# kungyao/vae-play

Measured on AMD Instinct MI355X. Metric: images/sec (train step, 128x128 VAE), higher is better.
Workload: dtype bf16x3; 1 GPU; networks VAE 128x128x3 latent=128 train step (fwd+BCE/KL+bwd+allreduce+Adam), 32 images/GPU, global batch 32; parallelism=dp1, per_gpu_batch=32, global_batch=32, graph=False, precision=bf16x3

## Files before the change

### include/vaeplay_hip.h

```cpp
#ifndef VAEPLAY_HIP_H
#define VAEPLAY_HIP_H
#include <stddef.h>
#include <stdint.h>

#ifdef __cplusplus
extern "C" {
#endif

typedef void* vp_stream;

enum vp_status { VP_OK = 0, VP_ERR_ARG = -1, VP_ERR_LAUNCH = -2, VP_ERR_WORKSPACE = -3, VP_ERR_STATE = -4 };
enum vp_act { VP_ACT_NONE = 0, VP_ACT_RELU = 1, VP_ACT_LRELU = 2, VP_ACT_TANH = 3, VP_ACT_SIGMOID = 4 };

int vp_abi_version(void);
const char* vp_last_error(void);

int vp_nchw_to_nhwc_f32(const float* in, float* out, int B, int C, int H, int W, vp_stream stream);
int vp_nhwc_to_nchw_f32(const float* in, float* out, int B, int C, int H, int W, vp_stream stream);

int vp_pack_w5_f32(const float* w_ref, float* p0, float* p1, int Csmall, int Cbig, vp_stream stream);

int vp_conv5_gather_f32(const float* big, const float* w_p0, const float* bias, float* small_out,
                        int B, int Hs, int Ws, int Cbig, int Csmall, int stride, int act, vp_stream stream);
int vp_conv5_scatter_f32(const float* small, const float* w_p1, float* big_out,
                         int B, int Hs, int Ws, int Csmall, int Cbig, int stride, vp_stream stream);
size_t vp_conv5_wgrad_workspace_bytes(int B, int Hs, int Ws, int Cbig, int Csmall, int stride);
int vp_conv5_wgrad_f32(const float* big, const float* small, float* dw_ref,
                       int B, int Hs, int Ws, int Cbig, int Csmall, int stride,
                       void* ws, size_t ws_bytes, vp_stream stream);
int vp_conv5_wgrad_f32_cus(const float* big, const float* small, float* dw_ref, int B, int Hs, int Ws, int Cbig, int Csmall,
                           int stride, int max_cus, void* ws, size_t ws_bytes, vp_stream stream);
size_t vp_conv5_stats_f32_workspace_bytes(int family, int B, int Hs, int Ws, int Cbig, int Csmall, int stride);
int vp_conv5_gather_stats_f32(const float* big, const float* w_p0, float* small_out, int B, int Hs, int Ws, int Cbig, int Csmall, int stride,
                              float eps, float momentum, float* mean, float* rstd, float* running_mean, float* running_var, void* ws,
                              size_t ws_bytes, vp_stream stream);
int vp_conv5_scatter_stats_f32(const float* small, const float* w_p1, float* big_out, int B, int Hs, int Ws, int Csmall, int Cbig, int stride,
                               float eps, float momentum, float* mean, float* rstd, float* running_mean, float* running_var, void* ws,
                               size_t ws_bytes, vp_stream stream);

int vp_pack_w_f32(const float* w_ref, float* p0, float* p1, int Csmall, int Cbig, int ks, vp_stream stream);
int vp_conv_gather_f32(const float* big, const float* w_p0, const float* bias, float* small_out,
                       int B, int Hs, int Ws, int Hb, int Wb, int Cbig, int Csmall, int ks, int stride, int act, vp_stream stream);
int vp_conv_scatter_f32(const float* small, const float* w_p1, float* big_out,
                        int B, int Hs, int Ws, int Hb, int Wb, int Csmall, int Cbig, int ks, int stride, vp_stream stream);
size_t vp_conv_wgrad_workspace_bytes(int B, int Hs, int Ws, int Hb, int Wb, int Cbig, int Csmall, int ks, int stride);
int vp_conv_wgrad_f32(const float* big, const float* small, float* dw_ref,
                      int B, int Hs, int Ws, int Hb, int Wb, int Cbig, int Csmall, int ks, int stride,
                      void* ws, size_t ws_bytes, vp_stream stream);

int vp_pack_w_split(const float* w_ref, void* p0_split, void* p1_split, int Csmall, int Cbig, int ks, vp_stream stream);
int vp_conv_gather_bf16x3(const void* big_split, const void* w_p0_split, const float* bias, float* small_out, int B, int Hs, int Ws,
                          int Hb, int Wb, int Cbig, int Csmall, int ks, int stride, int act, vp_stream stream);
int vp_conv_scatter_bf16x3(const void* small_split, const void* w_p1_split, float* big_out, int B, int Hs, int Ws, int Hb, int Wb,
                           int Csmall, int Cbig, int ks, int stride, vp_stream stream);
size_t vp_conv_wgrad_bf16x3_workspace_bytes(int B, int Hs, int Ws, int Hb, int Wb, int Cbig, int Csmall, int ks, int stride);
int vp_conv_wgrad_bf16x3(const void* big_split, const void* small_split, float* dw_ref, int B, int Hs, int Ws, int Hb, int Wb, int Cbig,
                         int Csmall, int ks, int stride, void* ws, size_t ws_bytes, vp_stream stream);
int vp_split_f32(const float* x, void* out_split, size_t n, vp_stream stream);
int vp_split_pad_f32(const float* x, void* out_split, size_t npix, int C, int Cpad, vp_stream stream);
int vp_pack_w5_split(const float* w_ref, void* p0_split, void* p1_split, int Csmall, int Cbig, vp_stream stream);
int vp_conv5_gather_bf16x3(const void* big_split, const void* w_p0_split, const float* bias, float* small_out,
                           int B, int Hs, int Ws, int Cbig, int Csmall, int stride, int act, vp_stream stream);
int vp_conv5_scatter_bf16x3(const void* small_split, const void* w_p1_split, float* big_out,
                            int B, int Hs, int Ws, int Csmall, int Cbig, int stride, vp_stream stream);
int vp_conv5_smallout_bf16x3(const float* big, const float* w_p0, const float* bias, float* small_out, int B, int H, int W,
                             int Cbig, int Csmall, int act, vp_stream stream);
size_t vp_conv5_smallout_wgrad_bf16x3_workspace_bytes(int B, int H, int W, int Cbig, int Csmall);
int vp_conv5_smallout_wgrad_bf16x3(const float* big, const float* small, float* dw_ref, int B, int H, int W, int Cbig, int Csmall,
                                   void* ws, size_t ws_bytes, vp_stream stream);
size_t vp_conv5_smallout_wgrad_f32_workspace_bytes(int B, int H, int W, int Cbig, int Csmall);
int vp_conv5_smallout_wgrad_f32(const float* big, const float* small, float* dw_ref, int B, int H, int W, int Cbig, int Csmall,
                                void* ws, size_t ws_bytes, vp_stream stream);
int vp_im2col5s2_cols(int C);
int vp_im2col5s2_split_f32(const float* x, void* out_split, int B, int C, int Hb, int Wb, int nchw, vp_stream stream);
int vp_pack_w_im2col5_split(const float* w_ref, void* out_split, int Cout, int C, vp_stream stream);
int vp_unpack_dw_im2col5_f32(const float* dw_cols, float* dw_ref, int Cout, int C, vp_stream stream);
int vp_im2col5s2_f32(const float* x, float* out, int B, int C, int Hb, int Wb, int nchw, vp_stream stream);
int vp_pack_w_im2col5_f32(const float* w_ref, float* out, int Cout, int C, vp_stream stream);
size_t vp_conv5_stats_workspace_bytes(int family, int B, int Hs, int Ws, int Cbig, int Csmall, int stride);
int vp_conv5_gather_stats_bf16x3(const void* big_split, const void* w_p0_split, float* small_out,
                                 int B, int Hs, int Ws, int Cbig, int Csmall, int stride, float eps, float momentum,
                                 float* mean, float* rstd, float* running_mean, float* running_var,
                                 void* ws, size_t ws_bytes, vp_stream stream);
int vp_conv5_scatter_stats_bf16x3(const void* small_split, const void* w_p1_split, float* big_out,
                                  int B, int Hs, int Ws, int Csmall, int Cbig, int stride, float eps, float momentum,
                                  float* mean, float* rstd, float* running_mean, float* running_var,
                                  void* ws, size_t ws_bytes, vp_stream stream);
int vp_conv5_smallin_dgrad_bf16x3(const float* small, const float* w_ref, float* big_out, int B, int H, int W, int Csmall, int Cbig,
                                  vp_stream stream);
int vp_conv5_smallin_dgrad_f32(const float* small, const float* w_ref, float* big_out, int B, int H, int W, int Csmall, int Cbig,
                               vp_stream stream);
int vp_conv5_smallin_fwd_bf16x3(const float* small, const float* w_ref, const float* bias, float* big_out, int B, int H, int W, int Csmall,
                                int Cbig, int act, vp_stream stream);
size_t vp_conv5_wgrad_bf16x3_workspace_bytes(int B, int Hs, int Ws, int Cbig, int Csmall, int stride);
int vp_conv5_wgrad_bf16x3(const void* big_split, const void* small_split, float* dw_ref,
                          int B, int Hs, int Ws, int Cbig, int Csmall, int stride,
                          void* ws, size_t ws_bytes, vp_stream stream);
int vp_conv5_wgrad_bf16x3_cus(const void* big_split, const void* small_split, float* dw_ref,
                              int B, int Hs, int Ws, int Cbig, int Csmall, int stride, int max_cus,
                              void* ws, size_t ws_bytes, vp_stream stream);
size_t vp_conv3_small_wgrad_workspace_bytes(int B, int H, int W, int Cin, int Cout);
int vp_conv3_small_wgrad_f32(const float* x, const float* dy, float* dw_ref, int B, int H, int W, int Cin, int Cout,
                             void* ws, size_t ws_bytes, vp_stream stream);
int vp_conv3_small_fwd_f32(const float* x, const float* w_ref, const float* bias, float* y, int B, int H, int W, int Cin, int Cout,
                           vp_stream stream);
int vp_conv3_small_dgrad_f32(const float* dy, const float* w_ref, float* dx, int B, int H, int W, int Cin, int Cout, vp_stream stream);
int vp_wgrad_slab_reduce_f32(const float* slab, float* dw_ref, int Csmall, int Cbig, int nsplit, int ntaps, int variant,
                             vp_stream stream);
int vp_bn_small_fwd_f32(const float* x, int R, int C, float eps, float momentum, const float* gamma, const float* beta, float* mean,
                        float* rstd, float* running_mean, float* running_var, float* y, int act, float slope, vp_stream stream);
int vp_bn_small_bwd_f32(const float* x, const float* dy, const float* mean, const float* rstd, const float* gamma, const float* beta,
                        float* dx, float* dgamma, float* dbeta, int R, int C, int act, float slope, int batch_stats, vp_stream stream);
int vp_bn_act_fwd_split_f32(const float* x, const float* mean, const float* rstd, const float* gamma, const float* beta,
                            float* y, void* y_split, int R, int C, int act, float slope, vp_stream stream);
int vp_bn_act_bwd_split_f32(const float* x, const float* dy, const float* mean, const float* rstd,
                            const float* gamma, const float* beta, float* dx, void* dx_split, float* dgamma, float* dbeta,
                            int R, int C, int act, float slope, int batch_stats,
                            void* ws, size_t ws_bytes, vp_stream stream);
int vp_nchw_to_nhwc_split_f32(const float* in, float* out, void* out_split, int B, int C, int H, int W, vp_stream stream);
typedef struct vp_pack_job {
  const float* w;
  void* p0;
  void* p1;
  int Csmall, Cbig, Csmall_pad, split;
} vp_pack_job;
int vp_pack_w5_batch(const vp_pack_job* jobs, int njobs, vp_stream stream);
int vp_pack_w5_p1_split_padded(const float* w_ref, void* p1_split, int Csmall, int Cbig, int Csmall_pad, vp_stream stream);
int vp_bce_sigmoid_bwd_pad_split_f32(const float* p, const float* t, float gscale, float* dlogit, void* dlogit_split,
                                     size_t npix, int C, int Cpad, vp_stream stream);

size_t vp_gemm_workspace_bytes(int M, int N, int K);
int vp_gemm_f32(const float* A, long sam, long sak, const float* B, long sbn, long sbk,
                float* C, int ldc, const float* bias, int M, int N, int K, int mode,
                void* ws, size_t ws_bytes, vp_stream stream);
size_t vp_colsum_workspace_bytes(int R, int C);
int vp_colsum_f32(const float* x, float* out, int R, int C, void* ws, size_t ws_bytes, vp_stream stream);

size_t vp_bn_workspace_bytes(int R, int C);
int vp_bn_stats_f32(const float* x, int R, int C, float eps, float momentum,
                    float* mean, float* rstd, float* running_mean, float* running_var,
                    void* ws, size_t ws_bytes, vp_stream stream);
int vp_bn_act_fwd_f32(const float* x, const float* mean, const float* rstd, const float* gamma, const float* beta,
                      float* y, int R, int C, int act, float slope, vp_stream stream);
int vp_bn_act_bwd_f32(const float* x, const float* dy, const float* mean, const float* rstd,
                      const float* gamma, const float* beta, float* dx, float* dgamma, float* dbeta,
                      int R, int C, int act, float slope, int batch_stats,
                      void* ws, size_t ws_bytes, vp_stream stream);
size_t vp_instnorm_workspace_bytes(int B, int R, int C);
int vp_instnorm_act_fwd_f32(const float* x, float* y, float* mean, float* rstd, int B, int R, int C, float eps, int act,
                            float slope, void* ws, size_t ws_bytes, vp_stream stream);
int vp_instnorm_act_bwd_f32(const float* x, const float* dy, const float* mean, const float* rstd, float* dx, int B, int R, int C,
                            int act, float slope, void* ws, size_t ws_bytes, vp_stream stream);
int vp_instnorm_act_fwd_split_f32(const float* x, float* y, void* y_split, float* mean, float* rstd, int B, int R, int C, float eps,
                                  int act, float slope, void* ws, size_t ws_bytes, vp_stream stream);
int vp_instnorm_act_bwd_split_f32(const float* x, const float* dy, const float* mean, const float* rstd, float* dx, void* dx_split, int B,
                                  int R, int C, int act, float slope, void* ws, size_t ws_bytes, vp_stream stream);
int vp_act_fwd_f32(const float* x, float* y, size_t n, int act, float slope, vp_stream stream);
int vp_act_bwd_from_y_f32(const float* y, const float* dy, float* dx, size_t n, int act, float slope, vp_stream stream);

int vp_upsample2x_bilinear_fwd_f32(const float* x, float* y, int B, int H, int W, int C, vp_stream stream);
int vp_upsample2x_bilinear_bwd_f32(const float* dy, float* dx, int B, int H, int W, int C, vp_stream stream);
int vp_add_coords_f32(const float* x, float* out, int B, int H, int W, int C, int normalize, vp_stream stream);
int vp_slice_channels_f32(const float* in, float* out, size_t npix, int Cin, int Cout, vp_stream stream);

int vp_latent_fwd_f32(const float* mu, const float* logvar, const float* eps, float* z, float* kl,
                      int B, int Z, vp_stream stream);
int vp_latent_bwd_f32(const float* mu, const float* logvar, const float* eps, const float* dz, const float* gkl,
                      float gkl_scalar, float* dmu, float* dlogvar, int B, int Z, vp_stream stream);

size_t vp_reduce_workspace_bytes(size_t n);
int vp_bce_sum_f32(const float* p, const float* t, size_t n, float* out, void* ws, size_t ws_bytes, vp_stream stream);
int vp_bce_bwd_f32(const float* p, const float* t, const float* gptr, float gscale, float* dp, size_t n, vp_stream stream);
int vp_bce_sigmoid_bwd_f32(const float* p, const float* t, float gscale, float* dlogit, size_t n, vp_stream stream);
int vp_global_avgpool_fwd_f32(const float* x_nhwc, float* out, int B, int HW, int C, vp_stream stream);
int vp_global_avgpool_bwd_f32(const float* dy, float* dx_nhwc, int B, int HW, int C, vp_stream stream);
int vp_softmax_rows_fwd_f32(const float* x, float* y, int R, int n, vp_stream stream);
int vp_softmax_rows_bwd_f32(const float* y, const float* dy, float* dx, int R, int n, vp_stream stream);
int vp_cross_entropy_fwd_f32(const float* logits, const long long* labels, float* loss, float* prob, int R, int n, vp_stream stream);
int vp_cross_entropy_bwd_f32(const float* prob, const long long* labels, const float* gptr, float* dlogits, int R, int n, vp_stream stream);
int vp_l1_mean_f32(const float* a, const float* b, size_t n, float* out, void* ws, size_t ws_bytes, vp_stream stream);
int vp_l1_mean_bwd_f32(const float* a, const float* b, const float* gptr, float* da, float* db, size_t n, vp_stream stream);

size_t vp_be_loss_workspace_bytes(int B, int n);
int vp_be_loss_fwd_f32(const float* logits, const float* targets, float* loss, float* sums, int B, int n, float bce_weight,
                       float smooth, void* ws, size_t ws_bytes, vp_stream stream);
int vp_be_loss_bwd_f32(const float* logits, const float* targets, const float* sums, const float* gptr, float* dlogits, int B,
                       int n, float bce_weight, float smooth, vp_stream stream);

int vp_dice_loss_fwd_f32(const float* probs, const float* targets, float* loss, float* sums, int B, int n, float smooth, void* ws,
                         size_t ws_bytes, vp_stream stream);
int vp_dice_loss_bwd_f32(const float* probs, const float* targets, const float* sums, const float* gptr, float* dprobs, int B, int n,
                         float smooth, vp_stream stream);

int vp_half_sqdiff_f32(const float* a, const float* b, float* out, size_t n, vp_stream stream);
int vp_half_sqdiff_rowsum_f32(const float* a, const float* b, float* out, int R, int n_per_row, vp_stream stream);
int vp_half_sqdiff_bwd_f32(const float* a, const float* b, const float* g, float* da, float* db, int R, int n_per_row,
                           int g_per_row, vp_stream stream);
int vp_gan_head_f32(const float* logit, int B, float coef, float* p_out, float* sums, float* dlogit, vp_stream stream);
int vp_smooth_l1_cat_f32(const float* targets, const float* a, const float* b, int B, int n1, int n2, float scale, float* loss,
                         float* da, float* db, vp_stream stream);
int vp_sum_f32(const float* x, size_t n, float* out, void* ws, size_t ws_bytes, vp_stream stream);
int vp_vae_loss_f32(const float* x_tilde, const float* x, size_t n, const float* kl, int B, float* recon, float* kl_sum,
                    float* loss, float loss_scale, void* ws, size_t ws_bytes, vp_stream stream);
int vp_add_f32(const float* a, const float* b, float* out, size_t n, vp_stream stream);

#define VP_SPLIT_BF16 0
#define VP_SPLIT_F16 1
int vp_split_fmt_f32(const float* x, void* out_split, size_t n, int fmt, float scale, vp_stream stream);
int vp_nchw_to_nhwc_split_fmt_f32(const float* in, float* out, void* out_split, int B, int C, int H, int W, int fmt, vp_stream stream);
int vp_bn_act_fwd_split_fmt_f32(const float* x, const float* mean, const float* rstd, const float* gamma, const float* beta,
                                float* y, void* y_split, int R, int C, int act, float slope, int fmt, vp_stream stream);
int vp_bn_act_bwd_split_fmt_f32(const float* x, const float* dy, const float* mean, const float* rstd,
                                const float* gamma, const float* beta, float* dx, void* dx_split, float* dgamma, float* dbeta,
                                int R, int C, int act, float slope, int batch_stats, int fmt, float scale,
                                void* ws, size_t ws_bytes, vp_stream stream);
int vp_bn_act_bwd_split_fmt_sat_f32(const float* x, const float* dy, const float* mean, const float* rstd,
                                    const float* gamma, const float* beta, float* dx, void* dx_split, float* dgamma, float* dbeta,
                                    int R, int C, int act, float slope, int batch_stats, int fmt, float scale, int* saturated,
                                    void* ws, size_t ws_bytes, vp_stream stream);
int vp_im2col5s2_split_fmt_f32(const float* x, void* out_split, int B, int C, int Hb, int Wb, int nchw, int fmt, vp_stream stream);
int vp_pack_w_im2col5_split_fmt(const float* w_ref, void* out_split, int Cout, int C, int fmt, vp_stream stream);
int vp_conv5_gather_f16(const void* big_split, const void* w_p0_split, const float* bias, float* small_out,
// ... 48 lines not shown
```

### vae_play_amd/_lib.py

```python
from __future__ import annotations

import ctypes
import os
from ctypes import c_char_p, c_float, c_int, c_long, c_size_t, c_void_p

_HERE = os.path.dirname(os.path.abspath(__file__))
LIB_PATH = os.environ.get("VAEPLAY_HIP_LIB", os.path.join(_HERE, "libvaeplay_hip.so"))

P = c_void_p


class PackJob(ctypes.Structure):
    _fields_ = [("w", c_void_p), ("p0", c_void_p), ("p1", c_void_p), ("Csmall", c_int), ("Cbig", c_int),
                ("Csmall_pad", c_int), ("split", c_int)]


SIGNATURES = {
    "vp_abi_version": (c_int, []),
    "vp_last_error": (c_char_p, []),
    "vp_nchw_to_nhwc_f32": (c_int, [P, P, c_int, c_int, c_int, c_int, P]),
    "vp_nhwc_to_nchw_f32": (c_int, [P, P, c_int, c_int, c_int, c_int, P]),
    "vp_pack_w5_f32": (c_int, [P, P, P, c_int, c_int, P]),
    "vp_conv5_gather_f32": (c_int, [P, P, P, P, c_int, c_int, c_int, c_int, c_int, c_int, c_int, P]),
    "vp_conv5_scatter_f32": (c_int, [P, P, P, c_int, c_int, c_int, c_int, c_int, c_int, P]),
    "vp_conv5_wgrad_workspace_bytes": (c_size_t, [c_int, c_int, c_int, c_int, c_int, c_int]),
    "vp_conv5_wgrad_f32": (c_int, [P, P, P, c_int, c_int, c_int, c_int, c_int, c_int, P, c_size_t, P]),
    "vp_conv5_wgrad_f32_cus": (c_int, [P, P, P, c_int, c_int, c_int, c_int, c_int, c_int, c_int, P, c_size_t, P]),
    "vp_pack_w_f32": (c_int, [P, P, P, c_int, c_int, c_int, P]),
    "vp_conv_gather_f32": (c_int, [P, P, P, P] + [c_int] * 10 + [P]),
    "vp_conv_scatter_f32": (c_int, [P, P, P] + [c_int] * 9 + [P]),
    "vp_conv_wgrad_workspace_bytes": (c_size_t, [c_int] * 9),
    "vp_conv_wgrad_f32": (c_int, [P, P, P] + [c_int] * 9 + [P, c_size_t, P]),
    "vp_split_f32": (c_int, [P, P, c_size_t, P]),
    "vp_split_pad_f32": (c_int, [P, P, c_size_t, c_int, c_int, P]),
    "vp_pack_w5_split": (c_int, [P, P, P, c_int, c_int, P]),
    "vp_pack_w_split": (c_int, [P, P, P, c_int, c_int, c_int, P]),
    "vp_conv_gather_bf16x3": (c_int, [P, P, P, P] + [c_int] * 10 + [P]),
    "vp_conv_scatter_bf16x3": (c_int, [P, P, P] + [c_int] * 9 + [P]),
    "vp_conv_wgrad_bf16x3_workspace_bytes": (c_size_t, [c_int] * 9),
    "vp_conv_wgrad_bf16x3": (c_int, [P, P, P] + [c_int] * 9 + [P, c_size_t, P]),
    "vp_conv5_gather_bf16x3": (c_int, [P, P, P, P, c_int, c_int, c_int, c_int, c_int, c_int, c_int, P]),
    "vp_conv5_scatter_bf16x3": (c_int, [P, P, P, c_int, c_int, c_int, c_int, c_int, c_int, P]),
    "vp_conv5_smallout_bf16x3": (c_int, [P, P, P, P] + [c_int] * 6 + [P]),
    "vp_conv5_smallout_wgrad_bf16x3_workspace_bytes": (c_size_t, [c_int] * 5),
    "vp_conv5_smallout_wgrad_bf16x3": (c_int, [P, P, P] + [c_int] * 5 + [P, c_size_t, P]),
    "vp_conv5_smallout_wgrad_f32_workspace_bytes": (c_size_t, [c_int] * 5),
    "vp_conv5_smallout_wgrad_f32": (c_int, [P, P, P] + [c_int] * 5 + [P, c_size_t, P]),
    "vp_im2col5s2_cols": (c_int, [c_int]),
    "vp_im2col5s2_split_f32": (c_int, [P, P, c_int, c_int, c_int, c_int, c_int, P]),
    "vp_pack_w_im2col5_split": (c_int, [P, P, c_int, c_int, P]),
    "vp_unpack_dw_im2col5_f32": (c_int, [P, P, c_int, c_int, P]),
    "vp_im2col5s2_f32": (c_int, [P, P, c_int, c_int, c_int, c_int, c_int, P]),
    "vp_pack_w_im2col5_f32": (c_int, [P, P, c_int, c_int, P]),
    "vp_conv5_stats_workspace_bytes": (c_size_t, [c_int] * 7),
    "vp_conv5_gather_stats_bf16x3": (c_int, [P, P, P] + [c_int] * 6 + [c_float, c_float, P, P, P, P, P, c_size_t, P]),
    "vp_conv5_gather_stats_f32": (c_int, [P, P, P] + [c_int] * 6 + [c_float, c_float, P, P, P, P, P, c_size_t, P]),
    "vp_conv5_scatter_stats_f32": (c_int, [P, P, P] + [c_int] * 6 + [c_float, c_float, P, P, P, P, P, c_size_t, P]),
    "vp_conv5_stats_f32_workspace_bytes": (c_size_t, [c_int] * 7),
    "vp_conv5_scatter_stats_bf16x3": (c_int, [P, P, P] + [c_int] * 6 + [c_float, c_float, P, P, P, P, P, c_size_t, P]),
    "vp_split_fmt_f32": (c_int, [P, P, c_size_t, c_int, c_float, P]),
    "vp_nchw_to_nhwc_split_fmt_f32": (c_int, [P, P, P, c_int, c_int, c_int, c_int, c_int, P]),
    "vp_bn_act_fwd_split_fmt_f32": (c_int, [P] * 7 + [c_int, c_int, c_int, c_float, c_int, P]),
    "vp_bn_act_bwd_split_fmt_f32": (c_int, [P] * 10 + [c_int, c_int, c_int, c_float, c_int, c_int, c_float, P, c_size_t, P]),
    "vp_bn_act_bwd_split_fmt_sat_f32": (c_int, [P] * 10 + [c_int, c_int, c_int, c_float, c_int, c_int, c_float, P, P, c_size_t, P]),
    "vp_im2col5s2_split_fmt_f32": (c_int, [P, P] + [c_int] * 6 + [P]),
    "vp_pack_w_im2col5_split_fmt": (c_int, [P, P, c_int, c_int, c_int, P]),
    "vp_conv5_gather_f16": (c_int, [P, P, P, P] + [c_int] * 8 + [c_float, P]),
    "vp_conv_gather_f16": (c_int, [P, P, P, P] + [c_int] * 11 + [c_float, P]),
    "vp_conv5_scatter_f16": (c_int, [P, P, P] + [c_int] * 7 + [c_float, P]),
    "vp_conv_scatter_f16": (c_int, [P, P, P] + [c_int] * 10 + [c_float, P]),
    "vp_conv5_wgrad_f16x2": (c_int, [P, P, P] + [c_int] * 6 + [c_float, P, c_size_t, P]),
    "vp_conv5_wgrad_f16x2_cus": (c_int, [P, P, P] + [c_int] * 6 + [c_float, c_int, P, c_size_t, P]),
    "vp_conv_wgrad_f16x2": (c_int, [P, P, P] + [c_int] * 9 + [c_float, P, c_size_t, P]),
    "vp_conv5_stats_f16_workspace_bytes": (c_size_t, [c_int] * 7),
    "vp_conv5_gather_stats_f16": (c_int, [P, P, P] + [c_int] * 7 + [c_float, c_float, P, P, P, P, P, c_size_t, P]),
    "vp_conv5_scatter_stats_f16": (c_int, [P, P, P] + [c_int] * 7 + [c_float, c_float, P, P, P, P, P, c_size_t, P]),
    "vp_conv5_smallin_fwd_bf16x3": (c_int, [P, P, P, P, c_int, c_int, c_int, c_int, c_int, c_int, P]),
    "vp_conv5_smallin_dgrad_bf16x3": (c_int, [P, P, P, c_int, c_int, c_int, c_int, c_int, P]),
    "vp_conv5_smallin_dgrad_f32": (c_int, [P, P, P, c_int, c_int, c_int, c_int, c_int, P]),
    "vp_conv5_wgrad_bf16x3_workspace_bytes": (c_size_t, [c_int, c_int, c_int, c_int, c_int, c_int]),
    "vp_conv5_wgrad_bf16x3": (c_int, [P, P, P, c_int, c_int, c_int, c_int, c_int, c_int, P, c_size_t, P]),
    "vp_conv5_wgrad_bf16x3_cus": (c_int, [P, P, P, c_int, c_int, c_int, c_int, c_int, c_int, c_int, P, c_size_t, P]),
    "vp_wgrad_slab_reduce_f32": (c_int, [P, P, c_int, c_int, c_int, c_int, c_int, P]),
    "vp_conv3_small_wgrad_workspace_bytes": (c_size_t, [c_int] * 5),
    "vp_conv3_small_wgrad_f32": (c_int, [P, P, P, c_int, c_int, c_int, c_int, c_int, P, c_size_t, P]),
    "vp_conv3_small_fwd_f32": (c_int, [P, P, P, P, c_int, c_int, c_int, c_int, c_int, P]),
    "vp_conv3_small_dgrad_f32": (c_int, [P, P, P, c_int, c_int, c_int, c_int, c_int, P]),
    "vp_bn_small_fwd_f32": (c_int, [P, c_int, c_int, c_float, c_float, P, P, P, P, P, P, P, c_int, c_float, P]),
    "vp_bn_small_bwd_f32": (c_int, [P] * 9 + [c_int, c_int, c_int, c_float, c_int, P]),
    "vp_bn_act_fwd_split_f32": (c_int, [P, P, P, P, P, P, P, c_int, c_int, c_int, c_float, P]),
    "vp_bn_act_bwd_split_f32": (c_int, [P, P, P, P, P, P, P, P, P, P, c_int, c_int, c_int, c_float, c_int, P, c_size_t, P]),
    "vp_nchw_to_nhwc_split_f32": (c_int, [P, P, P, c_int, c_int, c_int, c_int, P]),
    "vp_pack_w5_p1_split_padded": (c_int, [P, P, c_int, c_int, c_int, P]),
    "vp_pack_w5_batch": (c_int, [ctypes.POINTER(PackJob), c_int, P]),
    "vp_bce_sigmoid_bwd_pad_split_f32": (c_int, [P, P, c_float, P, P, c_size_t, c_int, c_int, P]),
    "vp_gemm_workspace_bytes": (c_size_t, [c_int, c_int, c_int]),
    "vp_gemm_f32": (c_int, [P, c_long, c_long, P, c_long, c_long, P, c_int, P, c_int, c_int, c_int, c_int, P, c_size_t, P]),
    "vp_colsum_workspace_bytes": (c_size_t, [c_int, c_int]),
    "vp_colsum_f32": (c_int, [P, P, c_int, c_int, P, c_size_t, P]),
    "vp_bn_workspace_bytes": (c_size_t, [c_int, c_int]),
    "vp_bn_stats_f32": (c_int, [P, c_int, c_int, c_float, c_float, P, P, P, P, P, c_size_t, P]),
    "vp_bn_act_fwd_f32": (c_int, [P, P, P, P, P, P, c_int, c_int, c_int, c_float, P]),
    "vp_bn_act_bwd_f32": (c_int, [P, P, P, P, P, P, P, P, P, c_int, c_int, c_int, c_float, c_int, P, c_size_t, P]),
    "vp_instnorm_workspace_bytes": (c_size_t, [c_int, c_int, c_int]),
    "vp_instnorm_act_fwd_f32": (c_int, [P, P, P, P, c_int, c_int, c_int, c_float, c_int, c_float, P, c_size_t, P]),
    "vp_instnorm_act_bwd_f32": (c_int, [P, P, P, P, P, c_int, c_int, c_int, c_int, c_float, P, c_size_t, P]),
    "vp_instnorm_act_fwd_split_f32": (c_int, [P, P, P, P, P, c_int, c_int, c_int, c_float, c_int, c_float, P, c_size_t, P]),
    "vp_instnorm_act_bwd_split_f32": (c_int, [P, P, P, P, P, P, c_int, c_int, c_int, c_int, c_float, P, c_size_t, P]),
    "vp_act_fwd_f32": (c_int, [P, P, c_size_t, c_int, c_float, P]),
    "vp_act_bwd_from_y_f32": (c_int, [P, P, P, c_size_t, c_int, c_float, P]),
    "vp_upsample2x_bilinear_fwd_f32": (c_int, [P, P, c_int, c_int, c_int, c_int, P]),
    "vp_upsample2x_bilinear_bwd_f32": (c_int, [P, P, c_int, c_int, c_int, c_int, P]),
    "vp_add_coords_f32": (c_int, [P, P, c_int, c_int, c_int, c_int, c_int, P]),
    "vp_slice_channels_f32": (c_int, [P, P, c_size_t, c_int, c_int, P]),
    "vp_latent_fwd_f32": (c_int, [P, P, P, P, P, c_int, c_int, P]),
    "vp_latent_bwd_f32": (c_int, [P, P, P, P, P, c_float, P, P, c_int, c_int, P]),
    "vp_reduce_workspace_bytes": (c_size_t, [c_size_t]),
    "vp_bce_sum_f32": (c_int, [P, P, c_size_t, P, P, c_size_t, P]),
    "vp_bce_bwd_f32": (c_int, [P, P, P, c_float, P, c_size_t, P]),
    "vp_bce_sigmoid_bwd_f32": (c_int, [P, P, c_float, P, c_size_t, P]),
    "vp_sum_f32": (c_int, [P, c_size_t, P, P, c_size_t, P]),
    "vp_vae_loss_f32": (c_int, [P, P, c_size_t, P, c_int, P, P, P, c_float, P, c_size_t, P]),
    "vp_add_f32": (c_int, [P, P, P, c_size_t, P]),
    "vp_global_avgpool_fwd_f32": (c_int, [P, P, c_int, c_int, c_int, P]),
    "vp_global_avgpool_bwd_f32": (c_int, [P, P, c_int, c_int, c_int, P]),
    "vp_softmax_rows_fwd_f32": (c_int, [P, P, c_int, c_int, P]),
    "vp_softmax_rows_bwd_f32": (c_int, [P, P, P, c_int, c_int, P]),
    "vp_cross_entropy_fwd_f32": (c_int, [P, P, P, P, c_int, c_int, P]),
    "vp_cross_entropy_bwd_f32": (c_int, [P, P, P, P, c_int, c_int, P]),
    "vp_l1_mean_f32": (c_int, [P, P, c_size_t, P, P, c_size_t, P]),
    "vp_l1_mean_bwd_f32": (c_int, [P, P, P, P, P, c_size_t, P]),
    "vp_be_loss_workspace_bytes": (c_size_t, [c_int, c_int]),
    "vp_be_loss_fwd_f32": (c_int, [P, P, P, P, c_int, c_int, c_float, c_float, P, c_size_t, P]),
    "vp_be_loss_bwd_f32": (c_int, [P, P, P, P, P, c_int, c_int, c_float, c_float, P]),
    "vp_dice_loss_fwd_f32": (c_int, [P, P, P, P, c_int, c_int, c_float, P, c_size_t, P]),
    "vp_dice_loss_bwd_f32": (c_int, [P, P, P, P, P, c_int, c_int, c_float, P]),
    "vp_half_sqdiff_f32": (c_int, [P, P, P, c_size_t, P]),
    "vp_half_sqdiff_rowsum_f32": (c_int, [P, P, P, c_int, c_int, P]),
    "vp_half_sqdiff_bwd_f32": (c_int, [P, P, P, P, P, c_int, c_int, c_int, P]),
    "vp_gan_head_f32": (c_int, [P, c_int, c_float, P, P, P, P]),
    "vp_smooth_l1_cat_f32": (c_int, [P, P, P, c_int, c_int, c_int, c_float, P, P, P, P]),
    "vp_bn_fold_f32": (c_int, [P, P, P, P, c_float, P, P, P, c_int, P]),
    "vp_conv5_affine_supported": (c_int, [c_int] * 8),
    "vp_conv5_gather_affine_bf16x3": (c_int, [P] * 6 + [c_int] * 7 + [P]),
    "vp_conv5_scatter_affine_bf16x3": (c_int, [P] * 6 + [c_int] * 7 + [P]),
    "vp_conv5_gather_affine_f32": (c_int, [P] * 6 + [c_int] * 7 + [P]),
    "vp_conv5_scatter_affine_f32": (c_int, [P] * 6 + [c_int] * 7 + [P]),
    "vp_adam_f32": (c_int, [P, P, P, P, c_size_t, c_float, c_float, c_float, c_float, c_int, c_float, P]),
    "vp_adam_outer_f32": (c_int, [P, P, P, P, P, c_int, c_int, c_int, c_float, c_float, c_float, c_float, c_int, c_float, P]),
    "vp_rmsprop_f32": (c_int, [P, P, P, c_size_t, c_float, c_float, c_float, c_float, P]),
}

_lib = None


class VaePlayHipError(RuntimeError):
    pass


def load() -> ctypes.CDLL:
    global _lib
    if _lib is not None:
        return _lib
    if not os.path.exists(LIB_PATH):
        raise VaePlayHipError(
            f"{LIB_PATH} not found: build it with `python -c 'import __graft_entry__ as g; g.build()'` "
            "or `make -C vae_play_amd/csrc`. There is no CPU fallback.")
    lib = ctypes.CDLL(LIB_PATH)
    for name, (res, args) in SIGNATURES.items():
        fn = getattr(lib, name)
        fn.restype = res
        fn.argtypes = args
    _lib = lib
    return lib


def check(rc: int, what: str = "") -> None:
    if rc != 0:
        msg = load().vp_last_error()
        raise VaePlayHipError(f"{what or 'vaeplay_hip'} failed (status {rc}): {msg.decode() if msg else ''}")


TRACE = None


def call(name: str, *args):
    tr = TRACE
    if tr is None:
        check(getattr(load(), name)(*args), name)
        return
    import torch
    e0, e1 = torch.cuda.Event(enable_timing=True), torch.cuda.Event(enable_timing=True)
    e0.record()
    rc = getattr(load(), name)(*args)
    e1.record()
    tr["events"].append((name, args, e0, e1))
    check(rc, name)
```

### vae_play_amd/csrc/bn.hip

```cpp
#include <stdlib.h>
#include "common.h"
#include "problems.h"
#include "split.h"

namespace vp {

constexpr int BN_TX = 16;
constexpr int BN_TY = 16;
constexpr int BN_CH = BN_TX * 4;

struct BnGrid { int chunks_r, chunks_c, rows_per_chunk; };

inline BnGrid bn_grid(int R, int C) {
  BnGrid g;
  g.chunks_c = (C + BN_CH - 1) / BN_CH;
  int total = 1024;
  int want = total / g.chunks_c;
  if (want < 1) want = 1;
  int maxr = (R + 63) / 64;
  if (maxr < 1) maxr = 1;
  g.chunks_r = want < maxr ? want : maxr;
  g.rows_per_chunk = (R + g.chunks_r - 1) / g.chunks_r;
  g.chunks_r = (R + g.rows_per_chunk - 1) / g.rows_per_chunk;
  return g;
}

__device__ __forceinline__ float act_apply(float v, int act, float slope) {
  switch (act) {
    case ACT_RELU: return v > 0.f ? v : 0.f;
    case ACT_LRELU: return v > 0.f ? v : v * slope;
    case ACT_TANH: return tanhf(v);
    case ACT_SIGMOID: return 1.f / (1.f + __expf(-v));
    default: return v;
  }
}
__device__ __forceinline__ float bn_pre(float x, float mu, float rs, float ga, float be) {
  return fmaf(ga, (x - mu) * rs, be);
}
__device__ __forceinline__ float act_grad_pre(float u, int act, float slope) {
  switch (act) {
    case ACT_RELU: return u > 0.f ? 1.f : 0.f;
    case ACT_LRELU: return u > 0.f ? 1.f : slope;
    case ACT_TANH: { float t = tanhf(u); return 1.f - t * t; }
    case ACT_SIGMOID: { float s = 1.f / (1.f + __expf(-u)); return s * (1.f - s); }
    default: return 1.f;
  }
}

template <int MODE>
__global__ void __launch_bounds__(256) bn_partial_kernel(const float* __restrict__ x, const float* __restrict__ dy,
                                                         const float* __restrict__ mean, const float* __restrict__ rstd,
                                                         const float* __restrict__ gamma, const float* __restrict__ beta,
                                                         float* __restrict__ part, int R, int C, int rows_per_chunk,
                                                         int act, float slope, size_t bxs = 0, size_t bps = 0) {
  x += blockIdx.z * bxs; part += blockIdx.z * bps;
  if (MODE == 1) { dy += blockIdx.z * bxs; mean += blockIdx.z * (size_t)C; rstd += blockIdx.z * (size_t)C; }
  __shared__ float sh[2][BN_TY][BN_CH + 4];
  const int tx = threadIdx.x % BN_TX, ty = threadIdx.x / BN_TX;
  const int c = blockIdx.y * BN_CH + tx * 4;
  const int r0 = blockIdx.x * rows_per_chunk;
  const int r1 = min(R, r0 + rows_per_chunk);
  float s0[4] = {0.f, 0.f, 0.f, 0.f}, s1[4] = {0.f, 0.f, 0.f, 0.f};
  const bool vec = (C % 4 == 0);
  float mu[4], rs[4], ga[4], be[4];
#pragma unroll
  for (int j = 0; j < 4; ++j) {
    const bool ok = c + j < C;
    mu[j] = (MODE == 1 && ok) ? mean[c + j] : 0.f;
    rs[j] = (MODE == 1 && ok) ? rstd[c + j] : 0.f;
    ga[j] = (MODE == 1 && ok && gamma) ? gamma[c + j] : 1.f;
    be[j] = (MODE == 1 && ok && beta) ? beta[c + j] : 0.f;
    if (MODE == 0) mu[j] = ok ? x[c + j] : 0.f;
  }
  if (c < C) {
    auto accum = [&](const float (&xv)[4], const float (&gv)[4]) {
#pragma unroll
      for (int j = 0; j < 4; ++j) {
        if (MODE == 0) {
          const float d = xv[j] - mu[j];
          s0[j] += d;
          s1[j] = fmaf(d, d, s1[j]);
        } else {
          const float xh = (xv[j] - mu[j]) * rs[j];
          const float g = gv[j] * act_grad_pre(fmaf(ga[j], xh, be[j]), act, slope);
          s0[j] += g;
          s1[j] = fmaf(g, xh, s1[j]);
        }
      }
    };
    int r = r0 + ty;
    if (vec) {
      for (; r + 3 * BN_TY < r1; r += 4 * BN_TY) {
        vp_f32x4 tx4[4], td4[4];
#pragma unroll
        for (int u = 0; u < 4; ++u) {
          const size_t off = (size_t)(r + u * BN_TY) * C + c;
          tx4[u] = *reinterpret_cast<const vp_f32x4*>(x + off);
          if (MODE == 1) td4[u] = *reinterpret_cast<const vp_f32x4*>(dy + off);
        }
#pragma unroll
        for (int u = 0; u < 4; ++u) {
          float xv[4] = {tx4[u][0], tx4[u][1], tx4[u][2], tx4[u][3]}, gv[4] = {0.f, 0.f, 0.f, 0.f};
          if (MODE == 1) { gv[0] = td4[u][0]; gv[1] = td4[u][1]; gv[2] = td4[u][2]; gv[3] = td4[u][3]; }
          accum(xv, gv);
        }
      }
    }
    for (; r < r1; r += BN_TY) {
      float xv[4], gv[4] = {0.f, 0.f, 0.f, 0.f};
      const size_t off = (size_t)r * C + c;
      if (vec) {
        vp_f32x4 t = *reinterpret_cast<const vp_f32x4*>(x + off);
        xv[0] = t[0]; xv[1] = t[1]; xv[2] = t[2]; xv[3] = t[3];
        if (MODE == 1) {
          vp_f32x4 d = *reinterpret_cast<const vp_f32x4*>(dy + off);
          gv[0] = d[0]; gv[1] = d[1]; gv[2] = d[2]; gv[3] = d[3];
        }
      } else {
#pragma unroll
        for (int j = 0; j < 4; ++j) {
          xv[j] = (c + j < C) ? x[off + j] : 0.f;
          if (MODE == 1) gv[j] = (c + j < C) ? dy[off + j] : 0.f;
        }
      }
      accum(xv, gv);
    }
  }
#pragma unroll
  for (int j = 0; j < 4; ++j) {
    sh[0][ty][tx * 4 + j] = s0[j];
    sh[1][ty][tx * 4 + j] = s1[j];
  }
  __syncthreads();
  if (threadIdx.x < 2 * BN_CH) {
    const int which = threadIdx.x / BN_CH, cc = threadIdx.x % BN_CH;
    float s = 0.f;
#pragma unroll
    for (int k = 0; k < BN_TY; ++k) s += sh[which][k][cc];
    const int cg = blockIdx.y * BN_CH + cc;
    if (cg < C) part[((size_t)which * gridDim.x + blockIdx.x) * C + cg] = s;
  }
}

constexpr int FIN_C = 4;

__device__ __forceinline__ void bn_final_reduce(const float* __restrict__ part, int nchunk, int C, int c, int lane,
                                                double& s, double& q) {
  double s0 = 0.0, s1 = 0.0, q0 = 0.0, q1 = 0.0;
  if (c < C) {
    int k = lane;
    for (; k + 64 < nchunk; k += 128) {
      s0 += (double)part[(size_t)k * C + c];
      s1 += (double)part[(size_t)(k + 64) * C + c];
      q0 += (double)part[((size_t)nchunk + k) * C + c];
      q1 += (double)part[((size_t)nchunk + k + 64) * C + c];
    }
    if (k < nchunk) {
      s0 += (double)part[(size_t)k * C + c];
      q0 += (double)part[((size_t)nchunk + k) * C + c];
    }
  }
  s = wave_sum_d(s0 + s1);
  q = wave_sum_d(q0 + q1);
}

__global__ void __launch_bounds__(256) bn_stats_final_kernel(const float* __restrict__ part, int nchunk, int R, int C, float eps,
                                                             float momentum, float* __restrict__ mean, float* __restrict__ rstd,
                                                             float* __restrict__ rm, float* __restrict__ rv, const float* __restrict__ x,
                                                             size_t bps = 0, size_t bxs = 0) {
  part += blockIdx.z * bps; mean += blockIdx.z * (size_t)C; rstd += blockIdx.z * (size_t)C; x += blockIdx.z * bxs;
  const int c = blockIdx.x * FIN_C + (threadIdx.x >> 6), lane = threadIdx.x & 63;
  double s, q;
  bn_final_reduce(part, nchunk, C, c, lane, s, q);
  if (lane != 0 || c >= C) return;
  const double ms = s / R;
  double var = q / R - ms * ms;
  if (var < 0.0) var = 0.0;
  const double m = (double)x[c] + ms;
  mean[c] = (float)m;
  rstd[c] = (float)(1.0 / sqrt(var + (double)eps));
  if (rm) rm[c] = (1.f - momentum) * rm[c] + momentum * (float)m;
  if (rv) {
    const double unb = R > 1 ? var * (double)R / (double)(R - 1) : var;
    rv[c] = (1.f - momentum) * rv[c] + momentum * (float)unb;
  }
}

__global__ void __launch_bounds__(256) bn_bwd_final_kernel(const float* __restrict__ part, int nchunk, int C,
                                                           float* __restrict__ sum_g, float* __restrict__ sum_gx,
                                                           float* __restrict__ dgamma, float* __restrict__ dbeta, size_t bps = 0) {
  part += blockIdx.z * bps; sum_g += blockIdx.z * (size_t)C; sum_gx += blockIdx.z * (size_t)C;
// ... 595 lines not shown
```

### vae_play_amd/csrc/conv16.hip

```cpp
#define VP_PCFG_LIBRARY 1
#define VP_IGEMM16_M16_ON 1
#include "conv16_impl.h"

namespace vp {

__global__ void split_kernel(const float* __restrict__ x, u16_t* __restrict__ out, size_t n, int fmt, float scale) {
  const size_t n4 = n / 4;
  for (size_t i = (size_t)blockIdx.x * blockDim.x + threadIdx.x; i < n4; i += (size_t)gridDim.x * blockDim.x) {
    const vp_f32x4 v = *reinterpret_cast<const vp_f32x4*>(x + i * 4);
    store_split4(out, n, i * 4, v[0] * scale, v[1] * scale, v[2] * scale, v[3] * scale, fmt);
  }
  if (blockIdx.x == 0 && threadIdx.x < (n & 3)) {
    const size_t i = n4 * 4 + threadIdx.x;
    u16_t h, l;
    split_f32(x[i] * scale, h, l, fmt);
    out[i] = h;
    out[n + i] = l;
  }
}

__global__ void split_pad_kernel(const float* __restrict__ x, u16_t* __restrict__ out, size_t npix, int C, int Cpad) {
  const size_t n = npix * (size_t)Cpad, n4 = n / 4;
  for (size_t i = (size_t)blockIdx.x * blockDim.x + threadIdx.x; i < n4; i += (size_t)gridDim.x * blockDim.x) {
    const size_t e = i * 4, pix = e / Cpad;
// ... 323 lines not shown
  const float* pv = slab + ((size_t)0 * C + c) * G;
  const float* sv = slab + ((size_t)1 * C + c) * G;
  const float* qv = slab + ((size_t)2 * C + c) * G;
  const double P = (double)pv[0];
  double S = 0.0, Q = 0.0;
  for (int g = threadIdx.x; g < G; g += 256) {
    const int tile = g % tiles_m;
    const long left = M - (long)tile * BM;
    const double n = (double)(left < BM ? left : BM);
    const double d = (double)pv[g] - P, s = (double)sv[g], q = (double)qv[g];
    S += s + n * d;
    Q += q + 2.0 * d * s + n * d * d;
  }
  S = wave_sum_d(S);
  Q = wave_sum_d(Q);
  if ((threadIdx.x & 63) == 0) { shs[threadIdx.x >> 6] = S; shq[threadIdx.x >> 6] = Q; }
  __syncthreads();
  if (threadIdx.x != 0) return;
  S = (shs[0] + shs[1]) + (shs[2] + shs[3]);
  Q = (shq[0] + shq[1]) + (shq[2] + shq[3]);
  const double ms = S / (double)R;
  double var = Q / (double)R - ms * ms;
  if (var < 0.0) var = 0.0;
  const double m = P + ms;
  mean[c] = (float)m;
  rstd[c] = (float)(1.0 / sqrt(var + (double)eps));
  if (rm) rm[c] = (1.f - momentum) * rm[c] + momentum * (float)m;
  if (rv) {
    const double unb = R > 1 ? var * (double)R / (double)(R - 1) : var;
    rv[c] = (1.f - momentum) * rv[c] + momentum * (float)unb;
  }
}
}

extern "C" {

size_t vp_conv5_stats_workspace_bytes(int family, int B, int Hs, int Ws, int Cbig, int Csmall, int stride) {
  const StatPlan sp = stat_plan(family, B, Hs, Ws, Cbig, Csmall, stride);
  return sp.ok ? (size_t)3 * sp.N * sp.tiles_m * sp.gz * sizeof(float) : 0;
}

}
namespace vp {
int stats_slab_finish(const float* slab, int groups, int tiles_m, int bm, long M, long R, int N, float eps, float momentum, float* mean,
                      float* rstd, float* rm, float* rv, hipStream_t stream) {
  hipLaunchKernelGGL(bn_stats_slab_final_kernel, dim3(N), dim3(256), 0, stream, slab, groups, tiles_m, bm, M, R, N, eps, momentum, mean, rstd, rm, rv);
  return check_launch("vp_conv5_*_stats_f32(final)");
}
}
int vp16_stats_finish(const StatPlan& sp, const float* slab, float eps, float momentum, float* mean, float* rstd, float* rm, float* rv,
                        vp_stream stream) {
  hipLaunchKernelGGL(bn_stats_slab_final_kernel, dim3(sp.N), dim3(256), 0, (hipStream_t)stream, slab, sp.tiles_m * sp.gz, sp.tiles_m, sp.bm,
                     sp.M, sp.R, sp.N, eps, momentum, mean, rstd, rm, rv);
  return check_launch("vp_conv5_*_stats_bf16x3(final)");
}
extern "C" {

int vp_conv5_gather_stats_bf16x3(const void* big_split, const void* w_p0_split, float* small_out, int B, int Hs, int Ws, int Cbig,
                                 int Csmall, int stride, float eps, float momentum, float* mean, float* rstd, float* running_mean,
                                 float* running_var, void* ws, size_t ws_bytes, vp_stream stream) {
  VP_REQUIRE(big_split && w_p0_split && small_out && mean && rstd && ws, "vp_conv5_gather_stats_bf16x3: null pointer");
  const StatPlan sp = stat_plan(0, B, Hs, Ws, Cbig, Csmall, stride);
  VP_REQUIRE(sp.ok, "vp_conv5_gather_stats_bf16x3: this shape cannot emit statistics (vp_conv5_stats_workspace_bytes() == 0)");
  if (ws_bytes < (size_t)3 * sp.N * sp.tiles_m * sp.gz * sizeof(float)) return fail(VP_ERR_WORKSPACE, "vp_conv5_gather_stats_bf16x3: workspace too small");
  int rc = gather16_t<ProbF16>(big_split, w_p0_split, nullptr, small_out, B, Hs, Ws, Hs * stride, Ws * stride, Cbig, Csmall, 5, stride,
                               VP_ACT_NONE, true, stream, (float*)ws);
  if (rc) return rc;
  return vp16_stats_finish(sp, (const float*)ws, eps, momentum, mean, rstd, running_mean, running_var, stream);
}

int vp_conv5_scatter_stats_bf16x3(const void* small_split, const void* w_p1_split, float* big_out, int B, int Hs, int Ws, int Csmall,
                                  int Cbig, int stride, float eps, float momentum, float* mean, float* rstd, float* running_mean,
                                  float* running_var, void* ws, size_t ws_bytes, vp_stream stream) {
  VP_REQUIRE(small_split && w_p1_split && big_out && mean && rstd && ws, "vp_conv5_scatter_stats_bf16x3: null pointer");
  const StatPlan sp = stat_plan(1, B, Hs, Ws, Cbig, Csmall, stride);
  VP_REQUIRE(sp.ok, "vp_conv5_scatter_stats_bf16x3: this shape cannot emit statistics (vp_conv5_stats_workspace_bytes() == 0)");
  if (ws_bytes < (size_t)3 * sp.N * sp.tiles_m * sp.gz * sizeof(float)) return fail(VP_ERR_WORKSPACE, "vp_conv5_scatter_stats_bf16x3: workspace too small");
  int rc = scatter16_t<ProbT16>(small_split, w_p1_split, big_out, B, Hs, Ws, Hs * stride, Ws * stride, Csmall, Cbig, 5, stride, true, stream,
                                (float*)ws);
  if (rc) return rc;
  return vp16_stats_finish(sp, (const float*)ws, eps, momentum, mean, rstd, running_mean, running_var, stream);
}


}

extern "C" {

int vp_im2col5s2_cols(int C) { return im2col5_kc(C); }

int vp_im2col5s2_split_fmt_f32(const float* x, void* out_split, int B, int C, int Hb, int Wb, int nchw, int fmt, vp_stream stream) {
  VP_REQUIRE(x && out_split && B > 0 && Hb > 0 && Wb > 0 && Hb % 2 == 0 && Wb % 2 == 0, "vp_im2col5s2_split_f32: bad arguments");
  VP_REQUIRE(C == 1 || C == 3, "vp_im2col5s2_split_f32: 1 or 3 image channels");
  VP_REQUIRE(split_fmt_ok(fmt, 1.f), "vp_im2col5s2_split_fmt_f32: format 0 (bf16 pair) or 1 (fp16 pair)");
  const dim3 grid((unsigned)(B * (Hb / 2)));
  if (C == 3) hipLaunchKernelGGL((im2col5s2_split_kernel<3>), grid, dim3(256), 0, (hipStream_t)stream, x, (u16_t*)out_split, B, Hb, Wb, Hb / 2, Wb / 2, nchw, fmt);
  else hipLaunchKernelGGL((im2col5s2_split_kernel<1>), grid, dim3(256), 0, (hipStream_t)stream, x, (u16_t*)out_split, B, Hb, Wb, Hb / 2, Wb / 2, nchw, fmt);
  return check_launch("vp_im2col5s2_split_f32");
}

int vp_im2col5s2_split_f32(const float* x, void* out_split, int B, int C, int Hb, int Wb, int nchw, vp_stream stream) {
  return vp_im2col5s2_split_fmt_f32(x, out_split, B, C, Hb, Wb, nchw, SPLIT_BF16, stream);
}

int vp_im2col5s2_f32(const float* x, float* out, int B, int C, int Hb, int Wb, int nchw, vp_stream stream) {
  VP_REQUIRE(x && out && B > 0 && Hb > 0 && Wb > 0 && Hb % 2 == 0 && Wb % 2 == 0, "vp_im2col5s2_f32: bad arguments");
  VP_REQUIRE(C == 1 || C == 3, "vp_im2col5s2_f32: 1 or 3 image channels");
  VP_REQUIRE(((uintptr_t)out & 15) == 0, "vp_im2col5s2_f32: the output must be 16-byte aligned");
  const dim3 grid((unsigned)(B * (Hb / 2)));
  if (C == 3) hipLaunchKernelGGL((im2col5s2_f32_kernel<3>), grid, dim3(256), 0, (hipStream_t)stream, x, out, B, Hb, Wb, Hb / 2, Wb / 2, nchw);
  else hipLaunchKernelGGL((im2col5s2_f32_kernel<1>), grid, dim3(256), 0, (hipStream_t)stream, x, out, B, Hb, Wb, Hb / 2, Wb / 2, nchw);
  return check_launch("vp_im2col5s2_f32");
}

int vp_pack_w_im2col5_f32(const float* w_ref, float* out, int Cout, int C, vp_stream stream) {
  VP_REQUIRE(w_ref && out && Cout > 0 && (C == 1 || C == 3), "vp_pack_w_im2col5_f32: bad arguments");
  const int KC = im2col5_kc(C), GW = im2col5_gw(C);
  hipLaunchKernelGGL(pack_w_im2col5_f32_kernel, dim3(grid_for((size_t)Cout * KC, 256)), dim3(256), 0, (hipStream_t)stream, w_ref, out, Cout, C,
                     GW, KC);
  return check_launch("vp_pack_w_im2col5_f32");
}

int vp_pack_w_im2col5_split_fmt(const float* w_ref, void* out_split, int Cout, int C, int fmt, vp_stream stream) {
  VP_REQUIRE(w_ref && out_split && Cout > 0 && (C == 1 || C == 3), "vp_pack_w_im2col5_split: bad arguments");
  VP_REQUIRE(split_fmt_ok(fmt, 1.f), "vp_pack_w_im2col5_split_fmt: format 0 (bf16 pair) or 1 (fp16 pair)");
  const int KC = im2col5_kc(C), GW = im2col5_gw(C);
  hipLaunchKernelGGL(pack_w_im2col5_split_kernel, dim3(grid_for((size_t)Cout * KC, 256)), dim3(256), 0, (hipStream_t)stream, w_ref,
                     (u16_t*)out_split, Cout, C, GW, KC, fmt);
  return check_launch("vp_pack_w_im2col5_split");
}

int vp_pack_w_im2col5_split(const float* w_ref, void* out_split, int Cout, int C, vp_stream stream) {
  return vp_pack_w_im2col5_split_fmt(w_ref, out_split, Cout, C, SPLIT_BF16, stream);
}

int vp_unpack_dw_im2col5_f32(const float* dw_cols, float* dw_ref, int Cout, int C, vp_stream stream) {
  VP_REQUIRE(dw_cols && dw_ref && Cout > 0 && (C == 1 || C == 3), "vp_unpack_dw_im2col5_f32: bad arguments");
  const int KC = im2col5_kc(C), GW = im2col5_gw(C);
  hipLaunchKernelGGL(unpack_dw_im2col5_kernel, dim3(grid_for((size_t)Cout * C * 25, 256)), dim3(256), 0, (hipStream_t)stream, dw_cols, dw_ref,
                     Cout, C, GW, KC);
  return check_launch("vp_unpack_dw_im2col5_f32");
}


int vp_conv5_smallout_bf16x3(const float* big, const float* w_p0, const float* bias, float* small_out, int B, int H, int W, int Cbig,
                             int Csmall, int act, vp_stream stream) {
  VP_REQUIRE(big && w_p0 && small_out && B > 0 && H > 0 && W > 0, "vp_conv5_smallout_bf16x3: bad arguments");
  VP_REQUIRE(((uintptr_t)big & 15) == 0 && ((uintptr_t)w_p0 & 15) == 0, "vp_conv5_smallout_bf16x3: operands must be 16-byte aligned");
  const ConvGeom g = make_geom(B, H, W, Csmall, Cbig, 1);
  VP_REQUIRE(tapn_gather_applicable(g, act), "vp_conv5_smallout_bf16x3: needs 64 or 32 input channels, 1 or 3 outputs, act none|sigmoid");
  return tapn_gather_launch(big, w_p0, bias, small_out, g, act, (hipStream_t)stream);
}

}
```

### vae_play_amd/csrc/edge.hip

```cpp
#include <stdlib.h>
#include <stdint.h>
#include "common.h"
#include "igemm16.h"
#include "narrow.h"
#include "split.h"

namespace vp {

template <int NOUT, int TH>
__global__ void __launch_bounds__(256, 2) wgrad_tapm_kernel(const float* __restrict__ u, const float* __restrict__ dlogit,
                                                            float* __restrict__ slab, int H, int W, int bands_per_img) {
  constexpr int C = 64, NCOL = 25 * NOUT, MT = (NCOL + 31) / 32;
  constexpr int SS = 64;
  constexpr int US = KmStride<64>::bytes;
  constexpr int UPLANE = ((SS * US + 127) / 128) * 128 + 64;
  constexpr int UBUF = 2 * UPLANE;
  extern __shared__ __attribute__((aligned(16))) unsigned char smem[];
  const int PC = ((W + 4 + 7) / 8) * 8;
  const int PLANE_E = (TH + 4) * PC;
  u16* const dhi = reinterpret_cast<u16*>(smem + 2 * UBUF);
  u16* const dlo = dhi + NOUT * PLANE_E;
  u16* const zeros = dlo + NOUT * PLANE_E;
  const int tid = threadIdx.x, lane = tid & 63;
  const int wave = __builtin_amdgcn_readfirstlane(tid >> 6);
  const int li = lane & 31, lh = lane >> 5;
  const int b = blockIdx.x / bands_per_img, h0 = (blockIdx.x - b * bands_per_img) * TH;

  for (int i = tid; i < NOUT * PLANE_E; i += 256) {
    const int n = i / PLANE_E, rem = i - n * PLANE_E;
    const int pr = rem / PC, pc = rem - pr * PC;
    const int h = h0 - 2 + pr, w = pc - 2;
    float v = 0.f;
    if (h >= 0 && h < H && w >= 0 && w < W) v = dlogit[((size_t)(b * H + h) * W + w) * NOUT + n];
    u16_t hh, ll;
    split_f32(v, hh, ll);
    dhi[i] = hh;
    dlo[i] = ll;
  }
  if (tid < 32) zeros[tid] = 0;

  const int m = 32 * wave + li;
  const bool mrow = wave < MT && m < NCOL;
  const int tap = mrow ? m / NOUT : 0, n_ = mrow ? m - tap * NOUT : 0;
  const int r_ = tap / 5, q_ = tap - 5 * r_;
  const int a_off = n_ * PLANE_E + (4 - r_) * PC + (4 - q_) + 8 * lh;

  const int spx = tid >> 2, sch = (tid & 3) * 16;
  vp_f32x4 st[4];
  const int nss = TH * W / SS;
  auto load_ss = [&](int ss) {
    const int p0 = ss * SS + spx;
    const int hr = p0 / W, w = p0 - hr * W;
    const float* src = u + ((size_t)(b * H + h0 + hr) * W + w) * C + sch;
#pragma unroll
    for (int v = 0; v < 4; ++v) st[v] = ld4(src + 4 * v);
  };
  auto write_ss = [&](int buf) {
    unsigned char* base = smem + buf * UBUF + spx * US + sch * 2;
#pragma unroll
    for (int v = 0; v < 4; ++v) {
      u16x4_t h, l;
#pragma unroll
      for (int j = 0; j < 4; ++j) { u16_t a, c; split_f32(st[v][j], a, c); h[j] = a; l[j] = c; }
      *reinterpret_cast<u16x4_t*>(base + 8 * v) = h;
      *reinterpret_cast<u16x4_t*>(base + UPLANE + 8 * v) = l;
    }
  };

  f32x16_t acc[2];
#pragma unroll
  for (int j = 0; j < 2; ++j)
#pragma unroll
    for (int r = 0; r < 16; ++r) acc[j][r] = 0.f;

  load_ss(0);
  write_ss(0);
  __syncthreads();
  for (int ss = 0; ss < nss; ++ss) {
    const bool more = ss + 1 < nss;
    if (more) load_ss(ss + 1);
    if (wave < MT) {
      const unsigned char* ub = smem + (ss & 1) * UBUF;
      const int pbase = ss * SS;
      const int hr = pbase / W, w0 = pbase - hr * W;
#pragma unroll
      for (int s = 0; s < 4; ++s) {
        const int e = mrow ? a_off + hr * PC + w0 + 16 * s : 0;
        const u16* ph = mrow ? dhi + e : zeros;
        const u16* pl = mrow ? dlo + e : zeros;
        bf16x8_t ah, al;
#pragma unroll
        for (int j = 0; j < 8; ++j) {
          ah[j] = __builtin_bit_cast(__bf16, ph[j]);
          al[j] = __builtin_bit_cast(__bf16, pl[j]);
        }
#pragma unroll
        for (int j = 0; j < 2; ++j) {
          const bf16x8_t bh = frag16<64, true, 64>(ub, 32 * j + li, s, li, lh, lane);
          const bf16x8_t bl = frag16<64, true, 64>(ub + UPLANE, 32 * j + li, s, li, lh, lane);
          acc[j] = __builtin_amdgcn_mfma_f32_32x32x16_bf16(al, bh, acc[j], 0, 0, 0);
          acc[j] = __builtin_amdgcn_mfma_f32_32x32x16_bf16(ah, bl, acc[j], 0, 0, 0);
          acc[j] = __builtin_amdgcn_mfma_f32_32x32x16_bf16(ah, bh, acc[j], 0, 0, 0);
        }
      }
    }
    if (more) write_ss((ss + 1) & 1);
    __syncthreads();
  }
  if (wave < MT) {
    float* out = slab + (size_t)blockIdx.x * NCOL * C;
#pragma unroll
    for (int j = 0; j < 2; ++j)
#pragma unroll
      for (int r = 0; r < 16; ++r) {
        const int row = 32 * wave + (r & 3) + 8 * (r >> 2) + 4 * lh;
        if (row < NCOL) out[(size_t)row * C + 32 * j + li] = acc[j][r];
      }
  }
}

template <int NOUT, int TH>
__global__ void __launch_bounds__(256, 2) wgrad_tapm_f32_kernel(const float* __restrict__ u, const float* __restrict__ dlogit,
                                                                float* __restrict__ slab, int H, int W, int bands_per_img) {
  constexpr int C = 64, NCOL = 25 * NOUT, MT = (NCOL + 31) / 32;
  constexpr int SS = 64, UP = 96;
  constexpr int UBUF = SS * UP;
  static_assert(MT <= 3, "row blocks");
  extern __shared__ __attribute__((aligned(16))) unsigned char smem[];
  float* const ubuf = reinterpret_cast<float*>(smem);
  float* const patch = ubuf + 2 * UBUF;
  const int PC = ((W + 4 + 7) / 8) * 8;
  const int PLANE_E = (TH + 4) * PC;
  const int tid = threadIdx.x, lane = tid & 63;
  const int wave = __builtin_amdgcn_readfirstlane(tid >> 6);
  const int li = lane & 31, lh = lane >> 5;
  const int b = blockIdx.x / bands_per_img, h0 = (blockIdx.x - b * bands_per_img) * TH;

  for (int i = tid; i < NOUT * PLANE_E; i += 256) {
    const int n = i / PLANE_E, rem = i - n * PLANE_E;
    const int pr = rem / PC, pc = rem - pr * PC;
    const int h = h0 - 2 + pr, w = pc - 2;
    patch[i] = (h >= 0 && h < H && w >= 0 && w < W) ? dlogit[((size_t)(b * H + h) * W + w) * NOUT + n] : 0.f;
  }

  int a_off[MT];
  bool mrow[MT];
#pragma unroll
  for (int rb = 0; rb < MT; ++rb) {
    const int m = 32 * rb + li;
    mrow[rb] = m < NCOL;
    const int tap = mrow[rb] ? m / NOUT : 0, n_ = mrow[rb] ? m - tap * NOUT : 0;
    const int r_ = tap / 5, q_ = tap - 5 * r_;
    a_off[rb] = n_ * PLANE_E + (4 - r_) * PC + (4 - q_) + 16 * wave + lh;
  }

  const int spx = tid >> 2, sch = (tid & 3) * 16;
  vp_f32x4 st[4];
  const int nss = TH * W / SS;
  auto load_ss = [&](int ss) {
    const int p0 = ss * SS + spx;
    const int hr = p0 / W, w = p0 - hr * W;
    const float* src = u + ((size_t)(b * H + h0 + hr) * W + w) * C + sch;
#pragma unroll
    for (int v = 0; v < 4; ++v) st[v] = ld4(src + 4 * v);
  };
  auto write_ss = [&](int buf) {
    float* base = ubuf + buf * UBUF + spx * UP + sch;
#pragma unroll
    for (int v = 0; v < 4; ++v) *reinterpret_cast<vp_f32x4*>(base + 4 * v) = st[v];
  };

  f32x16_t acc[MT][2];
#pragma unroll
  for (int rb = 0; rb < MT; ++rb)
#pragma unroll
    for (int j = 0; j < 2; ++j)
#pragma unroll
      for (int r = 0; r < 16; ++r) acc[rb][j][r] = 0.f;

  load_ss(0);
  write_ss(0);
  __syncthreads();
  for (int ss = 0; ss < nss; ++ss) {
    const bool more = ss + 1 < nss;
    if (more) load_ss(ss + 1);
    {
      const float* ub = ubuf + (ss & 1) * UBUF + (16 * wave + lh) * UP + li;
      const int pbase = ss * SS;
      const int hr = pbase / W, w0 = pbase - hr * W;
      const float* pa = patch + hr * PC + w0;
#pragma unroll
      for (int j = 0; j < 8; ++j) {
        const float b0 = ub[2 * j * UP], b1 = ub[2 * j * UP + 32];
#pragma unroll
        for (int rb = 0; rb < MT; ++rb) {
          float a = pa[a_off[rb] + 2 * j];
          a = mrow[rb] ? a : 0.f;
          acc[rb][0] = __builtin_amdgcn_mfma_f32_32x32x2f32(a, b0, acc[rb][0], 0, 0, 0);
          acc[rb][1] = __builtin_amdgcn_mfma_f32_32x32x2f32(a, b1, acc[rb][1], 0, 0, 0);
        }
      }
    }
    if (more) write_ss((ss + 1) & 1);
    __syncthreads();
  }
  constexpr int WREGS = MT * 2 * 16;
  float* const red = ubuf;
  static_assert(2 * WREGS * 64 <= 2 * UBUF, "reduction scratch");
  auto park = [&](int slot) {
#pragma unroll
    for (int rb = 0; rb < MT; ++rb)
#pragma unroll
      for (int j = 0; j < 2; ++j)
#pragma unroll
        for (int r = 0; r < 16; ++r) red[((slot * WREGS) + (rb * 2 + j) * 16 + r) * 64 + lane] = acc[rb][j][r];
  };
  auto take = [&](int slot) {
#pragma unroll
    for (int rb = 0; rb < MT; ++rb)
#pragma unroll
      for (int j = 0; j < 2; ++j)
#pragma unroll
        for (int r = 0; r < 16; ++r) acc[rb][j][r] += red[((slot * WREGS) + (rb * 2 + j) * 16 + r) * 64 + lane];
  };
  if (wave >= 2) park(wave - 2);
  __syncthreads();
  if (wave < 2) take(wave);
  __syncthreads();
  if (wave == 1) park(0);
  __syncthreads();
  if (wave == 0) {
    take(0);
    float* out = slab + (size_t)blockIdx.x * NCOL * C;
#pragma unroll
    for (int rb = 0; rb < MT; ++rb)
#pragma unroll
      for (int j = 0; j < 2; ++j)
#pragma unroll
        for (int r = 0; r < 16; ++r) {
          const int row = 32 * rb + (r & 3) + 8 * (r >> 2) + 4 * lh;
          if (row < NCOL) out[(size_t)row * C + 32 * j + li] = acc[rb][j][r];
        }
  }
}

constexpr int TAPM_TH = 8;

bool tapm_wgrad_applicable(const ConvGeom& g) {
  const bool on = true;
  return on && g.ks == 5 && g.stride == 1 && g.Hb == g.Hs && g.Wb == g.Ws && (g.Cs == 1 || g.Cs == 3) && g.Cb == 64 &&
         g.Ws % 64 == 0 && g.Hs % TAPM_TH == 0 && g.Ws <= 512;
}

size_t tapm_wgrad_ws_floats(const ConvGeom& g) { return (size_t)g.B * (g.Hs / TAPM_TH) * kTaps * g.Cs * g.Cb; }

static size_t tapm_lds_bytes(const ConvGeom& g) {
  constexpr int US = KmStride<64>::bytes, UPLANE = ((64 * US + 127) / 128) * 128 + 64;
  const int PC = ((g.Ws + 4 + 7) / 8) * 8;
  return (size_t)2 * 2 * UPLANE + (size_t)2 * g.Cs * (TAPM_TH + 4) * PC * 2 + 64;
}

int tapm_wgrad_launch(const float* big_f32, const float* small_f32, float* dw_ref, const ConvGeom& g, float* ws, hipStream_t s) {
  const int bands = g.Hs / TAPM_TH, nblk = g.B * bands;
  const size_t lds = tapm_lds_bytes(g);
  if (lds > 160 * 1024) return fail(VP_ERR_ARG, "wgrad_tapm: image too wide for the LDS patch");
  if (g.Cs == 3) {
    static bool attr3 = false;
    if (!attr3) { (void)hipFuncSetAttribute((const void*)wgrad_tapm_kernel<3, TAPM_TH>, hipFuncAttributeMaxDynamicSharedMemorySize, 160 * 1024); attr3 = true; }
    hipLaunchKernelGGL((wgrad_tapm_kernel<3, TAPM_TH>), dim3(nblk), dim3(256), lds, s, big_f32, small_f32, ws, g.Hs, g.Ws, bands);
  } else {
    static bool attr1 = false;
    if (!attr1) { (void)hipFuncSetAttribute((const void*)wgrad_tapm_kernel<1, TAPM_TH>, hipFuncAttributeMaxDynamicSharedMemorySize, 160 * 1024); attr1 = true; }
    hipLaunchKernelGGL((wgrad_tapm_kernel<1, TAPM_TH>), dim3(nblk), dim3(256), lds, s, big_f32, small_f32, ws, g.Hs, g.Ws, bands);
  }
  int rc = check_launch("wgrad_tapm");
  if (rc) return rc;
  return slab_reduce_launch(ws, dw_ref, g.Cs, g.Cb, nblk, s, kTaps);
}

static size_t tapm_f32_lds_bytes(const ConvGeom& g) {
  const int PC = ((g.Ws + 4 + 7) / 8) * 8;
  return (size_t)2 * 64 * 96 * 4 + (size_t)g.Cs * (TAPM_TH + 4) * PC * 4;
}

int tapm_wgrad_f32_launch(const float* big_f32, const float* small_f32, float* dw_ref, const ConvGeom& g, float* ws, hipStream_t s) {
  const int bands = g.Hs / TAPM_TH, nblk = g.B * bands;
  const size_t lds = tapm_f32_lds_bytes(g);
  if (lds > 160 * 1024) return fail(VP_ERR_ARG, "wgrad_tapm_f32: image too wide for the LDS patch");
  if (g.Cs == 3) {
    static bool attr3 = false;
    if (!attr3) { (void)hipFuncSetAttribute((const void*)wgrad_tapm_f32_kernel<3, TAPM_TH>, hipFuncAttributeMaxDynamicSharedMemorySize, 160 * 1024); attr3 = true; }
    hipLaunchKernelGGL((wgrad_tapm_f32_kernel<3, TAPM_TH>), dim3(nblk), dim3(256), lds, s, big_f32, small_f32, ws, g.Hs, g.Ws, bands);
  } else {
    static bool attr1 = false;
    if (!attr1) { (void)hipFuncSetAttribute((const void*)wgrad_tapm_f32_kernel<1, TAPM_TH>, hipFuncAttributeMaxDynamicSharedMemorySize, 160 * 1024); attr1 = true; }
    hipLaunchKernelGGL((wgrad_tapm_f32_kernel<1, TAPM_TH>), dim3(nblk), dim3(256), lds, s, big_f32, small_f32, ws, g.Hs, g.Ws, bands);
  }
  int rc = check_launch("wgrad_tapm_f32");
  if (rc) return rc;
  return slab_reduce_launch(ws, dw_ref, g.Cs, g.Cb, nblk, s, kTaps);
}


template <int NIN, int CF, bool FWD>
__global__ void __launch_bounds__(512, 2) dgrad_rowk_kernel(const float* __restrict__ dlogit, const float* __restrict__ w,
                                                            float* __restrict__ out, int H, int W, int tiles_x, int tiles_per_img,
                                                            int ntiles, const float* __restrict__ bias = nullptr, int act = ACT_NONE) {
  static_assert(CF == 64 || CF == 32, "wide channel count");
  constexpr int NJT = CF / 32;
  constexpr int TR = 8, TC = 32, PR = TR + 4, PC = (TC + 4) * NIN + 8;
  constexpr int KROW = 5 * NIN;
  __shared__ float patch[PR * PC];
  const int tid = threadIdx.x, lane = tid & 63, wave = tid >> 6;
  const int li = lane & 31, lh = lane >> 5;
  typedef __bf16 bf16x8_l __attribute__((ext_vector_type(8)));
  typedef float f32x16_l __attribute__((ext_vector_type(16)));
  __shared__ __attribute__((aligned(16))) bf16x8_l bfr[5 * NJT * 2 * 64];
  auto split8 = [](const float (&x)[8], bf16x8_l& h, bf16x8_l& l) {
#pragma unroll
    for (int j = 0; j < 8; ++j) {
      const __bf16 hh = (__bf16)x[j];
      h[j] = hh;
      l[j] = (__bf16)(x[j] - (float)hh);
    }
  };
  if (wave < 5) {
    const int r = wave;
#pragma unroll
    for (int jt = 0; jt < NJT; ++jt) {
      float x[8];
#pragma unroll
      for (int j = 0; j < 8; ++j) {
        const int k = 8 * lh + j, d = k / NIN, n = k - d * NIN, cf = 32 * jt + li;
        const size_t wi = FWD ? (((size_t)cf * NIN + n) * 5 + r) * 5 + d : (((size_t)n * CF + cf) * 5 + r) * 5 + (4 - d);
        x[j] = k < KROW ? w[wi] : 0.f;
      }
      bf16x8_l h8, l8;
      split8(x, h8, l8);
      bfr[((r * NJT + jt) * 2 + 0) * 64 + lane] = h8;
      bfr[((r * NJT + jt) * 2 + 1) * 64 + lane] = l8;
    }
  }
  constexpr int NPE = PR * (TC + 4) * NIN, NPV = (NPE + 511) / 512;
  float pv[NPV];
  auto load_patch = [&](int tile) {
    const int b = tile / tiles_per_img, rem = tile - b * tiles_per_img;
    const int h0 = (rem / tiles_x) * TR, w0 = (rem % tiles_x) * TC;
#pragma unroll
    for (int u = 0; u < NPV; ++u) {
      const int i = tid + 512 * u;
      const int pr = i / ((TC + 4) * NIN), e = i - pr * ((TC + 4) * NIN);
      const int px = e / NIN, n = e - px * NIN;
      const int h = h0 - 2 + pr, ww = w0 - 2 + px;
      pv[u] = (i < NPE && h >= 0 && h < H && ww >= 0 && ww < W) ? dlogit[((size_t)(b * H + h) * W + ww) * NIN + n] : 0.f;
    }
  };
  if ((int)blockIdx.x < ntiles) load_patch(blockIdx.x);
  for (int tile = blockIdx.x; tile < ntiles; tile += gridDim.x) {
    const int b = tile / tiles_per_img, rem = tile - b * tiles_per_img;
    const int h0 = (rem / tiles_x) * TR, w0 = (rem % tiles_x) * TC;
    __syncthreads();
#pragma unroll
    for (int u = 0; u < NPV; ++u) {
      const int i = tid + 512 * u;
      if (i < NPE) { const int pr = i / ((TC + 4) * NIN); patch[pr * PC + (i - pr * ((TC + 4) * NIN))] = pv[u]; }
    }
    if (tid < PR * 8) patch[(tid >> 3) * PC + (TC + 4) * NIN + (tid & 7)] = 0.f;
    __syncthreads();
    if (tile + (int)gridDim.x < ntiles) load_patch(tile + (int)gridDim.x);
    f32x16_l acc[NJT];
#pragma unroll
    for (int jt = 0; jt < NJT; ++jt)
#pragma unroll
      for (int e = 0; e < 16; ++e) acc[jt][e] = 0.f;
#pragma unroll
    for (int r = 0; r < 5; ++r) {
      const float* q = &patch[(FWD ? wave + r : wave + 4 - r) * PC + li * NIN + 8 * lh];
      float x[8];
#pragma unroll
      for (int j = 0; j < 8; ++j) x[j] = (8 * lh + j < KROW) ? q[j] : 0.f;
      bf16x8_l ah, al;
      split8(x, ah, al);
#pragma unroll
      for (int jt = 0; jt < NJT; ++jt) {
        const bf16x8_l bh = bfr[((r * NJT + jt) * 2 + 0) * 64 + lane], bl = bfr[((r * NJT + jt) * 2 + 1) * 64 + lane];
        acc[jt] = __builtin_amdgcn_mfma_f32_32x32x16_bf16(al, bh, acc[jt], 0, 0, 0);
        acc[jt] = __builtin_amdgcn_mfma_f32_32x32x16_bf16(ah, bl, acc[jt], 0, 0, 0);
        acc[jt] = __builtin_amdgcn_mfma_f32_32x32x16_bf16(ah, bh, acc[jt], 0, 0, 0);
      }
    }
    const int h = h0 + wave;
    if (h < H) {
#pragma unroll
      for (int jt = 0; jt < NJT; ++jt) {
        const float bv = (FWD && bias) ? bias[32 * jt + li] : 0.f;
#pragma unroll
        for (int e = 0; e < 16; ++e) {
          const int ww = w0 + (e & 3) + 8 * (e >> 2) + 4 * lh;
          float v = acc[jt][e] + bv;
          if (FWD && act == ACT_RELU) v = v > 0.f ? v : 0.f;
          if (ww < W) out[((size_t)(b * H + h) * W + ww) * CF + 32 * jt + li] = v;
        }
      }
    }
  }
}

template <int NIN, int CF>
__global__ void __launch_bounds__(512, 2) dgrad_rowk_f32_kernel(const float* __restrict__ dlogit, const float* __restrict__ w,
                                                                float* __restrict__ out, int H, int W, int tiles_x, int tiles_per_img,
                                                                int ntiles) {
  static_assert(CF == 64 || CF == 32, "wide channel count");
  constexpr int NJT = CF / 32;
  constexpr int TR = 8, TC = 32, PR = TR + 4, PC = (TC + 4) * NIN + 8;
  constexpr int KROW = 5 * NIN;
  __shared__ float patch[PR * PC];
  typedef float f32x4_l __attribute__((ext_vector_type(4)));
  typedef float f32x16_l __attribute__((ext_vector_type(16)));
  __shared__ __attribute__((aligned(16))) f32x4_l bfr[5 * NJT * 2 * 64];
  const int tid = threadIdx.x, lane = tid & 63, wave = tid >> 6;
  const int li = lane & 31, lh = lane >> 5;
  if (wave < 5) {
    const int r = wave;
#pragma unroll
    for (int jt = 0; jt < NJT; ++jt)
#pragma unroll
      for (int jh = 0; jh < 2; ++jh) {
        f32x4_l x;
#pragma unroll
        for (int jj = 0; jj < 4; ++jj) {
          const int k = 8 * lh + 4 * jh + jj, d = k / NIN, n = k - d * NIN, cf = 32 * jt + li;
          x[jj] = k < KROW ? w[(((size_t)n * CF + cf) * 5 + r) * 5 + (4 - d)] : 0.f;
        }
        bfr[((r * NJT + jt) * 2 + jh) * 64 + lane] = x;
      }
  }
  constexpr int NPE = PR * (TC + 4) * NIN, NPV = (NPE + 511) / 512;
  float pv[NPV];
  auto load_patch = [&](int tile) {
    const int b = tile / tiles_per_img, rem = tile - b * tiles_per_img;
    const int h0 = (rem / tiles_x) * TR, w0 = (rem % tiles_x) * TC;
#pragma unroll
    for (int u = 0; u < NPV; ++u) {
      const int i = tid + 512 * u;
      const int pr = i / ((TC + 4) * NIN), e = i - pr * ((TC + 4) * NIN);
      const int px = e / NIN, n = e - px * NIN;
      const int h = h0 - 2 + pr, ww = w0 - 2 + px;
      pv[u] = (i < NPE && h >= 0 && h < H && ww >= 0 && ww < W) ? dlogit[((size_t)(b * H + h) * W + ww) * NIN + n] : 0.f;
    }
  };
  if ((int)blockIdx.x < ntiles) load_patch(blockIdx.x);
  for (int tile = blockIdx.x; tile < ntiles; tile += gridDim.x) {
    const int b = tile / tiles_per_img, rem = tile - b * tiles_per_img;
    const int h0 = (rem / tiles_x) * TR, w0 = (rem % tiles_x) * TC;
    __syncthreads();
#pragma unroll
    for (int u = 0; u < NPV; ++u) {
      const int i = tid + 512 * u;
      if (i < NPE) { const int pr = i / ((TC + 4) * NIN); patch[pr * PC + (i - pr * ((TC + 4) * NIN))] = pv[u]; }
    }
    if (tid < PR * 8) patch[(tid >> 3) * PC + (TC + 4) * NIN + (tid & 7)] = 0.f;
    __syncthreads();
    if (tile + (int)gridDim.x < ntiles) load_patch(tile + (int)gridDim.x);
    f32x16_l acc[NJT];
#pragma unroll
    for (int jt = 0; jt < NJT; ++jt)
#pragma unroll
      for (int e = 0; e < 16; ++e) acc[jt][e] = 0.f;
#pragma unroll
    for (int r = 0; r < 5; ++r) {
      const float* q = &patch[(wave + 4 - r) * PC + li * NIN + 8 * lh];
      float x[8];
#pragma unroll
      for (int j = 0; j < 8; ++j) x[j] = (8 * lh + j < KROW) ? q[j] : 0.f;
#pragma unroll
      for (int jt = 0; jt < NJT; ++jt) {
        const f32x4_l b0 = bfr[((r * NJT + jt) * 2 + 0) * 64 + lane], b1 = bfr[((r * NJT + jt) * 2 + 1) * 64 + lane];
#pragma unroll
        for (int j = 0; j < 4; ++j) acc[jt] = __builtin_amdgcn_mfma_f32_32x32x2f32(x[j], b0[j], acc[jt], 0, 0, 0);
#pragma unroll
        for (int j = 0; j < 4; ++j) acc[jt] = __builtin_amdgcn_mfma_f32_32x32x2f32(x[4 + j], b1[j], acc[jt], 0, 0, 0);
      }
    }
    const int h = h0 + wave;
    if (h < H) {
#pragma unroll
      for (int jt = 0; jt < NJT; ++jt)
#pragma unroll
        for (int e = 0; e < 16; ++e) {
          const int ww = w0 + (e & 3) + 8 * (e >> 2) + 4 * lh;
          if (ww < W) out[((size_t)(b * H + h) * W + ww) * CF + 32 * jt + li] = acc[jt][e];
        }
    }
  }
}

bool rowk_dgrad_applicable(int B, int H, int W, int Cbig, int Csmall) {
  const bool on = true;
  return on && B > 0 && H > 0 && W > 0 && Cbig == 64 && (Csmall == 1 || Csmall == 3);
}

}

using namespace vp;

extern "C" {

size_t vp_conv5_smallout_wgrad_bf16x3_workspace_bytes(int B, int H, int W, int Cbig, int Csmall) {
  const ConvGeom g = make_geom(B, H, W, Csmall, Cbig, 1);
  return tapm_wgrad_applicable(g) ? tapm_wgrad_ws_floats(g) * sizeof(float) : 0;
}

int vp_conv5_smallout_wgrad_bf16x3(const float* big, const float* small, float* dw_ref, int B, int H, int W, int Cbig, int Csmall,
                                   void* ws, size_t ws_bytes, vp_stream stream) {
  VP_REQUIRE(big && small && dw_ref && ws && B > 0 && H > 0 && W > 0, "vp_conv5_smallout_wgrad_bf16x3: bad arguments");
  VP_REQUIRE(((uintptr_t)big & 15) == 0, "vp_conv5_smallout_wgrad_bf16x3: the activation must be 16-byte aligned");
  const ConvGeom g = make_geom(B, H, W, Csmall, Cbig, 1);
  VP_REQUIRE(tapm_wgrad_applicable(g), "vp_conv5_smallout_wgrad_bf16x3: needs 64 input channels, 1 or 3 outputs, width a multiple of 64, height of 8");
  if (ws_bytes < tapm_wgrad_ws_floats(g) * sizeof(float)) return fail(VP_ERR_WORKSPACE, "vp_conv5_smallout_wgrad_bf16x3: workspace too small");
  return tapm_wgrad_launch(big, small, dw_ref, g, (float*)ws, (hipStream_t)stream);
}

size_t vp_conv5_smallout_wgrad_f32_workspace_bytes(int B, int H, int W, int Cbig, int Csmall) {
  return vp_conv5_smallout_wgrad_bf16x3_workspace_bytes(B, H, W, Cbig, Csmall);
}

int vp_conv5_smallout_wgrad_f32(const float* big, const float* small, float* dw_ref, int B, int H, int W, int Cbig, int Csmall,
                                void* ws, size_t ws_bytes, vp_stream stream) {
  VP_REQUIRE(big && small && dw_ref && ws && B > 0 && H > 0 && W > 0, "vp_conv5_smallout_wgrad_f32: bad arguments");
  VP_REQUIRE(((uintptr_t)big & 15) == 0, "vp_conv5_smallout_wgrad_f32: the activation must be 16-byte aligned");
  const ConvGeom g = make_geom(B, H, W, Csmall, Cbig, 1);
  VP_REQUIRE(tapm_wgrad_applicable(g), "vp_conv5_smallout_wgrad_f32: needs 64 input channels, 1 or 3 outputs, width a multiple of 64, height of 8");
  if (ws_bytes < tapm_wgrad_ws_floats(g) * sizeof(float)) return fail(VP_ERR_WORKSPACE, "vp_conv5_smallout_wgrad_f32: workspace too small");
  return tapm_wgrad_f32_launch(big, small, dw_ref, g, (float*)ws, (hipStream_t)stream);
}

int vp_conv5_smallin_dgrad_bf16x3(const float* small, const float* w_ref, float* big_out, int B, int H, int W, int Csmall, int Cbig,
                                  vp_stream stream) {
  VP_REQUIRE(small && w_ref && big_out, "vp_conv5_smallin_dgrad_bf16x3: null pointer");
  VP_REQUIRE(rowk_dgrad_applicable(B, H, W, Cbig, Csmall), "vp_conv5_smallin_dgrad_bf16x3: needs 64 big channels and 1 or 3 small channels");
  const int tiles_x = (W + 31) / 32, tiles_y = (H + 7) / 8, ntiles = B * tiles_x * tiles_y;
  const int grid = ntiles < 512 ? ntiles : 512;
  if (Csmall == 3)
    hipLaunchKernelGGL((dgrad_rowk_kernel<3, 64, false>), dim3(grid), dim3(512), 0, (hipStream_t)stream, small, w_ref, big_out, H, W, tiles_x,
                       tiles_x * tiles_y, ntiles, (const float*)nullptr, 0);
  else
    hipLaunchKernelGGL((dgrad_rowk_kernel<1, 64, false>), dim3(grid), dim3(512), 0, (hipStream_t)stream, small, w_ref, big_out, H, W, tiles_x,
                       tiles_x * tiles_y, ntiles, (const float*)nullptr, 0);
  return check_launch("vp_conv5_smallin_dgrad_bf16x3");
}

int vp_conv5_smallin_dgrad_f32(const float* small, const float* w_ref, float* big_out, int B, int H, int W, int Csmall, int Cbig,
                               vp_stream stream) {
  VP_REQUIRE(small && w_ref && big_out, "vp_conv5_smallin_dgrad_f32: null pointer");
  VP_REQUIRE(rowk_dgrad_applicable(B, H, W, Cbig, Csmall), "vp_conv5_smallin_dgrad_f32: needs 64 big channels and 1 or 3 small channels");
  const int tiles_x = (W + 31) / 32, tiles_y = (H + 7) / 8, ntiles = B * tiles_x * tiles_y;
  const int grid = ntiles < 512 ? ntiles : 512;
  if (Csmall == 3)
    hipLaunchKernelGGL((dgrad_rowk_f32_kernel<3, 64>), dim3(grid), dim3(512), 0, (hipStream_t)stream, small, w_ref, big_out, H, W, tiles_x,
                       tiles_x * tiles_y, ntiles);
  else
    hipLaunchKernelGGL((dgrad_rowk_f32_kernel<1, 64>), dim3(grid), dim3(512), 0, (hipStream_t)stream, small, w_ref, big_out, H, W, tiles_x,
                       tiles_x * tiles_y, ntiles);
  return check_launch("vp_conv5_smallin_dgrad_f32");
}

int vp_conv5_smallin_fwd_bf16x3(const float* small, const float* w_ref, const float* bias, float* big_out, int B, int H, int W, int Csmall,
                                int Cbig, int act, vp_stream stream) {
  VP_REQUIRE(small && w_ref && big_out && B > 0 && H > 0 && W > 0, "vp_conv5_smallin_fwd_bf16x3: bad arguments");
  VP_REQUIRE((Cbig == 32 || Cbig == 64) && (Csmall == 1 || Csmall == 3), "vp_conv5_smallin_fwd_bf16x3: needs 1 or 3 input and 32 or 64 output channels");
  VP_REQUIRE(act == VP_ACT_NONE || act == VP_ACT_RELU, "vp_conv5_smallin_fwd_bf16x3: activation none|relu");
  const int tiles_x = (W + 31) / 32, tiles_y = (H + 7) / 8, ntiles = B * tiles_x * tiles_y;
  const int grid = ntiles < 512 ? ntiles : 512;
#define VP_ROWK_FWD(NI, CFF) hipLaunchKernelGGL((dgrad_rowk_kernel<NI, CFF, true>), dim3(grid), dim3(512), 0, (hipStream_t)stream, small, w_ref, big_out, \
                                                H, W, tiles_x, tiles_x * tiles_y, ntiles, bias, act)
  if (Cbig == 64) { if (Csmall == 3) VP_ROWK_FWD(3, 64); else VP_ROWK_FWD(1, 64); }
  else { if (Csmall == 3) VP_ROWK_FWD(3, 32); else VP_ROWK_FWD(1, 32); }
#undef VP_ROWK_FWD
  return check_launch("vp_conv5_smallin_fwd_bf16x3");
}

}
```

### vae_play_amd/csrc/narrow.h

```cpp
#pragma once
#include <hip/hip_runtime.h>
#include "problems.h"

namespace vp {
bool narrow_gather_applicable(const ConvGeom& g, int act);
int narrow_gather_launch(const float* big, const float* w_p0, const float* bias, float* out, const ConvGeom& g, int act, hipStream_t s);
bool tapn_gather_applicable(const ConvGeom& g, int act);
int tapn_gather_launch(const float* big, const float* w_p0, const float* bias, float* out, const ConvGeom& g, int act, hipStream_t s);
int narrow_wgrad_kind(const ConvGeom& g);
size_t narrow_wgrad_ws_floats(const ConvGeom& g);
int narrow_wgrad_launch(const float* big, const float* small, float* dw_ref, const ConvGeom& g, float* ws, hipStream_t s);
int pack_w5_f32_launch(const float* w, float* p0, float* p1, int Cs, int Cb, hipStream_t s, int nt = kTaps);
int slab_reduce_launch(const float* slab, float* dw_ref, int Cs, int Cb, int nsplit, hipStream_t s, int nt = kTaps);
}
```

### vae_play_amd/csrc/narrow.hip

```cpp
#include <stdlib.h>
#include <stdint.h>
#include "common.h"
#include "problems.h"
#include "narrow.h"

namespace vp {

template <int NOUT>
__global__ void __launch_bounds__(256) conv5s1_smallout_kernel(const float* __restrict__ in, const float* __restrict__ w,
                                                               const float* __restrict__ bias, float* __restrict__ out,
                                                               int H, int W, int C, int act) {
  constexpr int T = 16, HALO = T + 4, CC = 16, PS = 20, ROW = 448;
  typedef float f32x2 __attribute__((ext_vector_type(2)));
  __shared__ __attribute__((aligned(16))) float tile[HALO * ROW];
  const int b = blockIdx.z, h0 = blockIdx.y * T, w0 = blockIdx.x * T;
  const int tx = threadIdx.x % T, ty = threadIdx.x / T;
  f32x2 acc[NOUT];
#pragma unroll
  for (int n = 0; n < NOUT; ++n) acc[n] = f32x2{0.f, 0.f};
  for (int c0 = 0; c0 < C; c0 += CC) {
    __syncthreads();
    for (int i = threadIdx.x; i < HALO * HALO * 4; i += 256) {
      const int pix = i >> 2, v = i & 3;
      const int py = pix / HALO, px = pix - py * HALO;
      const int h = h0 + py - 2, ww = w0 + px - 2;
      vp_f32x4 val = zero4();
      if (h >= 0 && h < H && ww >= 0 && ww < W) val = ld4(in + ((size_t)(b * H + h) * W + ww) * C + c0 + v * 4);
      *reinterpret_cast<vp_f32x4*>(&tile[py * ROW + px * PS + v * 4]) = val;
    }
    __syncthreads();
#pragma unroll 1
    for (int r = 0; r < 5; ++r) {
#pragma unroll
      for (int q = 0; q < 5; ++q) {
        const float* tp = &tile[(ty + r) * ROW + (tx + q) * PS];
        const float* wp = w + (size_t)(r * 5 + q) * C + c0;
#pragma unroll
        for (int v = 0; v < 4; ++v) {
          const vp_f32x4 xv = *reinterpret_cast<const vp_f32x4*>(tp + v * 4);
          const f32x2 x01 = {xv[0], xv[1]}, x23 = {xv[2], xv[3]};
#pragma unroll
          for (int n = 0; n < NOUT; ++n) {
            const float* wn = wp + (size_t)n * kTaps * C + v * 4;
            const f32x2 w01 = {wn[0], wn[1]}, w23 = {wn[2], wn[3]};
            acc[n] = __builtin_elementwise_fma(x01, w01, acc[n]);
            acc[n] = __builtin_elementwise_fma(x23, w23, acc[n]);
          }
        }
      }
    }
  }
  const int h = h0 + ty, ww = w0 + tx;
  if (h < H && ww < W) {
    float* o = out + ((size_t)(b * H + h) * W + ww) * NOUT;
#pragma unroll
    for (int n = 0; n < NOUT; ++n) {
      float v = (acc[n][0] + acc[n][1]) + (bias ? bias[n] : 0.f);
      if (act == ACT_SIGMOID) v = 1.f / (1.f + __builtin_expf(-v));
      o[n] = v;
    }
  }
}

constexpr int NS_ROWS = 4;

template <int NS>
__global__ void __launch_bounds__(256) wgrad_narrow_small_kernel(const float* __restrict__ big, const float* __restrict__ small,
                                                                 float* __restrict__ slab, int B, int H, int W, int Cb,
                                                                 int nunits) {
  __shared__ float red[4][5 * NS][64];
  const int lane = threadIdx.x & 63;
  const int g = __builtin_amdgcn_readfirstlane(threadIdx.x >> 6);
  const int c = blockIdx.y * 64 + lane;
  typedef float f32x2 __attribute__((ext_vector_type(2)));
  f32x2 accp[5][2][NS];
  float acc4[5][NS];
#pragma unroll
  for (int r = 0; r < 5; ++r)
#pragma unroll
    for (int n = 0; n < NS; ++n) { accp[r][0][n] = f32x2{0.f, 0.f}; accp[r][1][n] = f32x2{0.f, 0.f}; acc4[r][n] = 0.f; }
  const int unit = blockIdx.x * 4 + g;
  if (unit < nunits) {
    const int strips = (H + NS_ROWS - 1) / NS_ROWS;
    const int half = unit & 1, su = unit >> 1;
    const int b = su / strips, h0 = (su - b * strips) * NS_ROWS;
    const int h1 = min(H, h0 + NS_ROWS);
    const int wh = (W + 1) / 2;
    const int xa = half * wh, xb = min(W, xa + wh);
    for (int hb = max(0, h0 - 2); hb < min(H, h1 + 2) && xa < xb; ++hb) {
      const float* bp = big + ((size_t)(b * H + hb) * W) * Cb + c;
      const float* sp[5];
      bool on[5];
#pragma unroll
      for (int r = 0; r < 5; ++r) {
        const int h = hb + 2 - r;
        on[r] = h >= h0 && h < h1;
        sp[r] = small + ((size_t)(b * H + (on[r] ? h : h0)) * W) * NS;
      }
      float win[8], nxt[4];
      win[0] = xa - 2 >= 0 ? bp[(size_t)(xa - 2) * Cb] : 0.f;
      win[1] = xa - 1 >= 0 ? bp[(size_t)(xa - 1) * Cb] : 0.f;
      win[2] = bp[(size_t)xa * Cb];
      win[3] = xa + 1 < W ? bp[(size_t)(xa + 1) * Cb] : 0.f;
#pragma unroll
      for (int j = 0; j < 4; ++j) nxt[j] = (xa + 2 + j < W) ? bp[(size_t)(xa + 2 + j) * Cb] : 0.f;
      for (int x0 = xa; x0 < xb; x0 += 4) {
#pragma unroll
        for (int j = 0; j < 4; ++j) win[4 + j] = nxt[j];
        if (x0 + 4 < xb) {
#pragma unroll
          for (int j = 0; j < 4; ++j) nxt[j] = (x0 + 6 + j < W) ? bp[(size_t)(x0 + 6 + j) * Cb] : 0.f;
        }
        const bool full = x0 + 4 <= xb;
#pragma unroll
        for (int r = 0; r < 5; ++r) {
          if (!on[r]) continue;
          if (full) {
            float sv[4 * NS];
            const float* s4 = sp[r] + (size_t)x0 * NS;
#pragma unroll
            for (int i = 0; i < 4 * NS; ++i) sv[i] = s4[i];
#pragma unroll
            for (int j = 0; j < 4; ++j)
#pragma unroll
              for (int n = 0; n < NS; ++n) {
                const f32x2 s2 = {sv[j * NS + n], sv[j * NS + n]};
                accp[r][0][n] = __builtin_elementwise_fma(f32x2{win[j + 0], win[j + 1]}, s2, accp[r][0][n]);
                accp[r][1][n] = __builtin_elementwise_fma(f32x2{win[j + 2], win[j + 3]}, s2, accp[r][1][n]);
                acc4[r][n] = fmaf(win[j + 4], sv[j * NS + n], acc4[r][n]);
              }
          } else {
#pragma unroll
            for (int j = 0; j < 4; ++j) {
              if (x0 + j < xb) {
#pragma unroll
                for (int n = 0; n < NS; ++n) {
                  const float v = sp[r][(x0 + j) * NS + n];
                  const f32x2 s2 = {v, v};
                  accp[r][0][n] = __builtin_elementwise_fma(f32x2{win[j + 0], win[j + 1]}, s2, accp[r][0][n]);
                  accp[r][1][n] = __builtin_elementwise_fma(f32x2{win[j + 2], win[j + 3]}, s2, accp[r][1][n]);
                  acc4[r][n] = fmaf(win[j + 4], v, acc4[r][n]);
                }
              }
            }
          }
        }
#pragma unroll
        for (int j = 0; j < 4; ++j) win[j] = win[4 + j];
      }
    }
  }
  float* dst = slab + (size_t)blockIdx.x * kTaps * NS * Cb;
#pragma unroll
  for (int r = 0; r < 5; ++r) {
    __syncthreads();
#pragma unroll
    for (int q = 0; q < 5; ++q)
// ... 32 lines not shown
  const int nrows = B * H;
  const int row0 = blockIdx.x * rows_per_block;
  const int row1 = min(nrows, row0 + rows_per_block);
  for (int row = row0 + g; row < row1; row += 4) {
    const int b = row / H, h = row - b * H;
    const float* sp = small + (size_t)row * W * Cs + (c_ok ? c : 0);
    const int hb0 = stride * h - 2 + r0, hb1 = stride * h - 2 + r1;
    const bool rok0 = has0 && hb0 >= 0 && hb0 < Hb, rok1 = has1 && hb1 >= 0 && hb1 < Hb;
    const float* base0 = big + ((size_t)(b * Hb + (rok0 ? hb0 : 0)) * Wb) * NB;
    const float* base1 = big + ((size_t)(b * Hb + (rok1 ? hb1 : 0)) * Wb) * NB;
    auto win = [&](int x, float& v0, float& v1, float& dyv) {
      const int col0 = stride * x - 2 + e0 / NB, col1 = stride * x - 2 + e1 / NB;
      v0 = (rok0 && col0 >= 0 && col0 < Wb) ? base0[(size_t)col0 * NB + e0 % NB] : 0.f;
      v1 = (rok1 && col1 >= 0 && col1 < Wb) ? base1[(size_t)col1 * NB + e1 % NB] : 0.f;
      dyv = c_ok ? sp[(size_t)x * Cs] : 0.f;
    };
    float v0, v1, dyv;
    win(0, v0, v1, dyv);
    for (int x = 0; x < W; ++x) {
      float n0 = 0.f, n1 = 0.f, ndy = 0.f;
      if (x + 1 < W) win(x + 1, n0, n1, ndy);
#pragma unroll
      for (int t = 0; t < kTaps; ++t)
#pragma unroll
        for (int n = 0; n < NB; ++n) {
          const int idx = (t / 5) * NE + (t % 5) * NB + n;
          const float src = idx < 64 ? v0 : v1;
          const float sv = __builtin_bit_cast(float, __builtin_amdgcn_readlane(__builtin_bit_cast(int, src), idx & 63));
          acc[t][n] = fmaf(dyv, sv, acc[t][n]);
        }
      v0 = n0; v1 = n1; dyv = ndy;
    }
  }
  float* dst = slab + (size_t)blockIdx.x * kTaps * Cs * NB;
#pragma unroll
  for (int r = 0; r < 5; ++r) {
    __syncthreads();
#pragma unroll
    for (int q = 0; q < 5; ++q)
#pragma unroll
      for (int n = 0; n < NB; ++n) red[g][q * NB + n][lane] = acc[r * 5 + q][n];
    __syncthreads();
    for (int i = g; i < 5 * NB; i += 4) {
      const float v = (red[0][i][lane] + red[1][i][lane]) + (red[2][i][lane] + red[3][i][lane]);
      const int q = i / NB, n = i - q * NB;
      if (c_ok) dst[((size_t)(r * 5 + q) * Cs + c) * NB + n] = v;
    }
  }
}

__global__ void __launch_bounds__(256) slab_reduce_kernel(const float* __restrict__ slab, float* __restrict__ dw, int Cs, int Cb,
                                                          int nsplit, int nt) {
  __shared__ float tile[64 * 25];
  const size_t cc = (size_t)Cs * Cb, per = cc * nt;
  const size_t j0 = (size_t)blockIdx.x * 64;
  const int lane = threadIdx.x & 63, tg = threadIdx.x >> 6;
  const bool ok = j0 + lane < cc;
  for (int t = tg; t < nt; t += 4) {
    const float* src = slab + (size_t)t * cc + j0 + lane;
    float s0 = 0.f, s1 = 0.f;
    int sp = 0;
    if (ok) {
      for (; sp + 1 < nsplit; sp += 2) {
        s0 += src[(size_t)sp * per];
        s1 += src[(size_t)(sp + 1) * per];
      }
      if (sp < nsplit) s0 += src[(size_t)sp * per];
    }
    tile[lane * nt + t] = s0 + s1;
  }
  __syncthreads();
  const size_t base = j0 * nt;
  for (int i = threadIdx.x; i < 64 * nt; i += 256)
    if (base + i < per) dw[base + i] = tile[i];
}

__global__ void __launch_bounds__(256) slab_reduce_v4_kernel(const float* __restrict__ slab, float* __restrict__ dw, int Cs, int Cb,
                                                             int nsplit, int nt) {
  __shared__ __attribute__((aligned(16))) float tile[64 * 25];
  const size_t cc = (size_t)Cs * Cb, per = cc * nt;
  const size_t j0 = (size_t)blockIdx.x * 64;
  const int q = threadIdx.x & 15, tg = threadIdx.x >> 4;
  for (int t = tg; t < nt; t += 16) {
    const float* src = slab + (size_t)t * cc + j0 + 4 * q;
    vp_f32x4 s0 = {0.f, 0.f, 0.f, 0.f}, s1 = {0.f, 0.f, 0.f, 0.f};
    int sp = 0;
    for (; sp + 3 < nsplit; sp += 4) {
      const vp_f32x4 a = *reinterpret_cast<const vp_f32x4*>(src + (size_t)sp * per);
      const vp_f32x4 b = *reinterpret_cast<const vp_f32x4*>(src + (size_t)(sp + 1) * per);
      const vp_f32x4 c = *reinterpret_cast<const vp_f32x4*>(src + (size_t)(sp + 2) * per);
      const vp_f32x4 d = *reinterpret_cast<const vp_f32x4*>(src + (size_t)(sp + 3) * per);
      s0 += a; s1 += b; s0 += c; s1 += d;
    }
    for (; sp + 1 < nsplit; sp += 2) {
      const vp_f32x4 a = *reinterpret_cast<const vp_f32x4*>(src + (size_t)sp * per);
      const vp_f32x4 b = *reinterpret_cast<const vp_f32x4*>(src + (size_t)(sp + 1) * per);
      s0 += a; s1 += b;
    }
    if (sp < nsplit) s0 += *reinterpret_cast<const vp_f32x4*>(src + (size_t)sp * per);
    const vp_f32x4 v = s0 + s1;
#pragma unroll
    for (int e = 0; e < 4; ++e) tile[(4 * q + e) * nt + t] = v[e];
  }
  __syncthreads();
  const size_t base = j0 * nt;
  for (int i = threadIdx.x * 4; i < 64 * nt; i += 1024)
    *reinterpret_cast<vp_f32x4*>(dw + base + i) = *reinterpret_cast<const vp_f32x4*>(tile + i);
}

__global__ void __launch_bounds__(256) slab_reduce_deep_kernel(const float* __restrict__ slab, float* __restrict__ dw, int Cs, int Cb,
                                                               int nsplit, int nt) {
  __shared__ float red[16][17];
  const size_t per = (size_t)nt * Cs * Cb;
  const int o = threadIdx.x & 15, sl = threadIdx.x >> 4;
  const size_t i = (size_t)blockIdx.x * 16 + o;
  float s0 = 0.f, s1 = 0.f, s2 = 0.f, s3 = 0.f;
  if (i < per) {
    int sp = sl;
    for (; sp + 48 < nsplit; sp += 64) {
      s0 += slab[(size_t)sp * per + i];
      s1 += slab[(size_t)(sp + 16) * per + i];
      s2 += slab[(size_t)(sp + 32) * per + i];
      s3 += slab[(size_t)(sp + 48) * per + i];
    }
    for (; sp < nsplit; sp += 16) s0 += slab[(size_t)sp * per + i];
  }
  red[sl][o] = (s0 + s1) + (s2 + s3);
  __syncthreads();
  if (sl == 0 && i < per) {
    float v = 0.f;
#pragma unroll
    for (int k = 0; k < 16; ++k) v += red[k][o];
    const int cb = (int)(i % Cb);
    const size_t r = i / Cb;
    const int cs = (int)(r % Cs), t = (int)(r / Cs);
    dw[((size_t)cs * Cb + cb) * nt + t] = v;
  }
}


typedef float f32x16_e __attribute__((ext_vector_type(16)));
typedef __bf16 bf16x8_e __attribute__((ext_vector_type(8)));

__device__ __forceinline__ void split8(const vp_f32x4& a, const vp_f32x4& b, bf16x8_e& h, bf16x8_e& l) {
#pragma unroll
  for (int j = 0; j < 8; ++j) {
    const float x = j < 4 ? a[j] : b[j - 4];
    const __bf16 hh = (__bf16)x;
    h[j] = hh;
    l[j] = (__bf16)(x - (float)hh);
  }
}

template <int NOUT, int C>
__global__ void __launch_bounds__(512, 2) conv5s1_tapn_kernel(const float* __restrict__ in, const float* __restrict__ w,
                                                              const float* __restrict__ bias, float* __restrict__ out,
                                                              int H, int W, int tiles_x, int tiles_per_img, int ntiles, int act) {
  static_assert(C == 64 || C == 32, "64 input channels (the VAE's final conv) or 32 (input gradient of a 1|3 -> 32 first conv)");
  constexpr int T = 16, HALO = T + 4, NPIX = HALO * HALO;
  constexpr int NS = C / 16, NRAW = C / 8, HC = C / 2;
  constexpr int NCOL = 25 * NOUT, NT = (NCOL + 31) / 32;
  constexpr int PITCH = 32 * NT + 1;
  constexpr int MT = (NPIX + 31) / 32;
  constexpr int NWAVE = 8;
  __shared__ float P[NPIX * PITCH];
  const int tid = threadIdx.x, lane = tid & 63, wave = tid >> 6;
  const int li = lane & 31, lh = lane >> 5;

  bf16x8_e bh[NT][NS], bl[NT][NS];
#pragma unroll
  for (int jt = 0; jt < NT; ++jt) {
    const int row = 32 * jt + li;
#pragma unroll
    for (int s = 0; s < NS; ++s) {
      vp_f32x4 a = zero4(), c = zero4();
      if (row < NCOL) {
        const float* q = w + (size_t)row * C + HC * lh + 8 * s;
        a = ld4(q);
        c = ld4(q + 4);
      }
      split8(a, c, bh[jt][s], bl[jt][s]);
    }
  }

  auto load_tile = [&](int tile, int t, vp_f32x4 (&raw)[NRAW]) {
    const int b = tile / tiles_per_img, rem = tile - b * tiles_per_img;
    const int h0 = (rem / tiles_x) * T, w0 = (rem % tiles_x) * T;
    const int pi = 32 * t + li;
    const int py = pi / HALO, px = pi - py * HALO;
    const int gh = h0 + py - 2, gw = w0 + px - 2;
    const bool ok = pi < NPIX && gh >= 0 && gh < H && gw >= 0 && gw < W;
    const float* q = in + ((size_t)(b * H + (ok ? gh : 0)) * W + (ok ? gw : 0)) * C + HC * lh;
#pragma unroll
    for (int v = 0; v < NRAW; ++v) raw[v] = ok ? ld4(q + 4 * v) : zero4();
  };
  vp_f32x4 cur[NRAW], nxt[NRAW];
  if ((int)blockIdx.x < ntiles && wave < MT) load_tile(blockIdx.x, wave, cur);
  for (int tile = blockIdx.x; tile < ntiles; tile += gridDim.x) {
    const int b = tile / tiles_per_img, rem = tile - b * tiles_per_img;
    const int h0 = (rem / tiles_x) * T, w0 = (rem % tiles_x) * T;
    for (int t = wave; t < MT; t += NWAVE) {
      const bool more = t + NWAVE < MT;
      if (more) load_tile(tile, t + NWAVE, nxt);
      f32x16_e acc[NT];
#pragma unroll
      for (int jt = 0; jt < NT; ++jt)
#pragma unroll
        for (int r = 0; r < 16; ++r) acc[jt][r] = 0.f;
#pragma unroll
      for (int s = 0; s < NS; ++s) {
        bf16x8_e ah, al;
        split8(cur[2 * s], cur[2 * s + 1], ah, al);
#pragma unroll
        for (int jt = 0; jt < NT; ++jt) {
          acc[jt] = __builtin_amdgcn_mfma_f32_32x32x16_bf16(al, bh[jt][s], acc[jt], 0, 0, 0);
          acc[jt] = __builtin_amdgcn_mfma_f32_32x32x16_bf16(ah, bl[jt][s], acc[jt], 0, 0, 0);
          acc[jt] = __builtin_amdgcn_mfma_f32_32x32x16_bf16(ah, bh[jt][s], acc[jt], 0, 0, 0);
        }
      }
#pragma unroll
      for (int jt = 0; jt < NT; ++jt)
#pragma unroll
        for (int r = 0; r < 16; ++r) {
          const int row = 32 * t + (r & 3) + 8 * (r >> 2) + 4 * lh;
          if (row < NPIX) P[row * PITCH + 32 * jt + li] = acc[jt][r];
        }
      if (more) {
#pragma unroll
        for (int v = 0; v < NRAW; ++v) cur[v] = nxt[v];
      }
    }
    const int ntile = tile + (int)gridDim.x;
    if (ntile < ntiles && wave < MT) load_tile(ntile, wave, cur);
    __syncthreads();
    if (tid < T * T) {
      const int tx = tid % T, ty = tid / T;
      const int h = h0 + ty, ww = w0 + tx;
      float sum[NOUT];
#pragma unroll
      for (int n = 0; n < NOUT; ++n) sum[n] = bias ? bias[n] : 0.f;
#pragma unroll
      for (int r = 0; r < 5; ++r)
#pragma unroll
        for (int q = 0; q < 5; ++q) {
          const float* pp = &P[((ty + r) * HALO + tx + q) * PITCH + r * 5 + q];
#pragma unroll
          for (int n = 0; n < NOUT; ++n) sum[n] += pp[n * 25];
        }
      if (h < H && ww < W) {
        float* o = out + ((size_t)(b * H + h) * W + ww) * NOUT;
#pragma unroll
        for (int n = 0; n < NOUT; ++n) {
          float v = sum[n];
          if (act == ACT_SIGMOID) v = 1.f / (1.f + __builtin_expf(-v));
          o[n] = v;
        }
      }
    }
    __syncthreads();
  }
}

bool narrow_gather_applicable(const ConvGeom& g, int act) {
  return g.ks == 5 && g.Hb == g.Hs && g.Wb == g.Ws && g.stride == 1 && (g.Cs == 1 || g.Cs == 3) && g.Cb % 16 == 0 && (act == ACT_NONE || act == ACT_SIGMOID);
}

bool tapn_gather_applicable(const ConvGeom& g, int act) {
  return narrow_gather_applicable(g, act) && (g.Cb == 64 || g.Cb == 32);
}
int tapn_gather_launch(const float* big, const float* w_p0, const float* bias, float* out, const ConvGeom& g, int act, hipStream_t s) {
  const int tiles_x = (g.Ws + 15) / 16, tiles_per_img = tiles_x * ((g.Hs + 15) / 16), ntiles = tiles_per_img * g.B;
  const dim3 pgrid((unsigned)(ntiles < 256 ? ntiles : 256));
#define VP_TAPN(NO, CC) hipLaunchKernelGGL((conv5s1_tapn_kernel<NO, CC>), pgrid, dim3(512), 0, s, big, w_p0, bias, out, g.Hs, g.Ws, tiles_x, tiles_per_img, ntiles, act)
  if (g.Cb == 64) { if (g.Cs == 3) VP_TAPN(3, 64); else VP_TAPN(1, 64); }
  else { if (g.Cs == 3) VP_TAPN(3, 32); else VP_TAPN(1, 32); }
#undef VP_TAPN
  return check_launch("conv5s1_tapn");
}

int narrow_gather_launch(const float* big, const float* w_p0, const float* bias, float* out, const ConvGeom& g, int act,
                         hipStream_t s) {
  dim3 grid((g.Ws + 15) / 16, (g.Hs + 15) / 16, g.B);
  if (g.Cs == 3)
    hipLaunchKernelGGL((conv5s1_smallout_kernel<3>), grid, dim3(256), 0, s, big, w_p0, bias, out, g.Hs, g.Ws, g.Cb, act);
  else
    hipLaunchKernelGGL((conv5s1_smallout_kernel<1>), grid, dim3(256), 0, s, big, w_p0, bias, out, g.Hs, g.Ws, g.Cb, act);
  return check_launch("conv5s1_smallout");
}

static int narrow_rows_per_block(const ConvGeom& g) {
  const int rows = g.B * g.Hs;
  int blocks = 1024;
  int rpb = (rows + blocks - 1) / blocks;
  if (rpb < 4) rpb = 4;
  return rpb;
}

int narrow_wgrad_kind(const ConvGeom& g) {
  if (g.ks != 5 || g.Hb != g.Hs * g.stride || g.Wb != g.Ws * g.stride) return 0;
  if (g.stride == 1 && (g.Cs == 1 || g.Cs == 3) && g.Cb % 64 == 0) return 1;
  if ((g.Cb == 1 || g.Cb == 3) && g.Cs % 32 == 0) return 2;
  return 0;
}

static int narrow_small_units(const ConvGeom& g) { return g.B * ((g.Hs + NS_ROWS - 1) / NS_ROWS) * 2; }

static int narrow_wgrad_nblk(const ConvGeom& g) {
  if (narrow_wgrad_kind(g) == 1) return (narrow_small_units(g) + 3) / 4;
  const int rpb = narrow_rows_per_block(g);
  return (g.B * g.Hs + rpb - 1) / rpb;
}

size_t narrow_wgrad_ws_floats(const ConvGeom& g) { return (size_t)narrow_wgrad_nblk(g) * kTaps * g.Cs * g.Cb; }

int narrow_wgrad_launch(const float* big, const float* small, float* dw_ref, const ConvGeom& g, float* ws, hipStream_t s) {
  const int kind = narrow_wgrad_kind(g);
  const int rpb = narrow_rows_per_block(g);
  const int nblk = narrow_wgrad_nblk(g);
  if (kind == 1) {
    dim3 grid(nblk, g.Cb / 64);
    const int nunits = narrow_small_units(g);
    if (g.Cs == 3)
      hipLaunchKernelGGL((wgrad_narrow_small_kernel<3>), grid, dim3(256), 0, s, big, small, ws, g.B, g.Hs, g.Ws, g.Cb, nunits);
    else
      hipLaunchKernelGGL((wgrad_narrow_small_kernel<1>), grid, dim3(256), 0, s, big, small, ws, g.B, g.Hs, g.Ws, g.Cb, nunits);
  } else {
    dim3 grid(nblk, (g.Cs + 63) / 64);
    if (g.Cb == 3)
      hipLaunchKernelGGL((wgrad_narrow_big_kernel<3>), grid, dim3(256), 0, s, big, small, ws, g.B, g.Hs, g.Ws, g.Cs, g.stride, rpb);
    else
      hipLaunchKernelGGL((wgrad_narrow_big_kernel<1>), grid, dim3(256), 0, s, big, small, ws, g.B, g.Hs, g.Ws, g.Cs, g.stride, rpb);
  }
  int rc = check_launch("wgrad_narrow");
  if (rc) return rc;
  const size_t per = (size_t)kTaps * g.Cs * g.Cb;
  hipLaunchKernelGGL(slab_reduce_deep_kernel, dim3((unsigned)((per + 15) / 16)), dim3(256), 0, s, (const float*)ws, dw_ref, g.Cs, g.Cb, nblk, kTaps);
  return check_launch("slab_reduce");
}

static bool slab_v4_ok(const float* slab, const float* dw_ref, size_t cc, int nsplit, int nt) {
  return cc >= 4096 && nt <= 25 && !(nt == 1 && nsplit > 16) && cc % 64 == 0 && ((uintptr_t)slab & 15) == 0 && ((uintptr_t)dw_ref & 15) == 0;
}

int slab_reduce_variant_launch(const float* slab, float* dw_ref, int Cs, int Cb, int nsplit, hipStream_t s, int nt, int variant) {
  const size_t cc = (size_t)Cs * Cb, per = cc * nt;
  const bool v4_default = true;
  const bool v4 = variant < 0 ? v4_default : variant == 1;
  if (v4 && slab_v4_ok(slab, dw_ref, cc, nsplit, nt))
    hipLaunchKernelGGL(slab_reduce_v4_kernel, dim3((unsigned)(cc / 64)), dim3(256), 0, s, slab, dw_ref, Cs, Cb, nsplit, nt);
  else if (cc >= 4096 && nt <= 25 && !(nt == 1 && nsplit > 16))
    hipLaunchKernelGGL(slab_reduce_kernel, dim3((unsigned)((cc + 63) / 64)), dim3(256), 0, s, slab, dw_ref, Cs, Cb, nsplit, nt);
  else
    hipLaunchKernelGGL(slab_reduce_deep_kernel, dim3((unsigned)((per + 15) / 16)), dim3(256), 0, s, slab, dw_ref, Cs, Cb, nsplit, nt);
  return check_launch("slab_reduce");
}

int slab_reduce_launch(const float* slab, float* dw_ref, int Cs, int Cb, int nsplit, hipStream_t s, int nt) {
  return slab_reduce_variant_launch(slab, dw_ref, Cs, Cb, nsplit, s, nt, -1);
}

}

extern "C" int vp_wgrad_slab_reduce_f32(const float* slab, float* dw_ref, int Csmall, int Cbig, int nsplit, int ntaps, int variant,
                                        vp_stream stream) {
  using namespace vp;
  VP_REQUIRE(slab && dw_ref && Csmall > 0 && Cbig > 0 && nsplit > 0 && ntaps > 0, "vp_wgrad_slab_reduce_f32: bad arguments");
  VP_REQUIRE(variant >= -1 && variant <= 1, "vp_wgrad_slab_reduce_f32: variant must be -1, 0 or 1");
  return slab_reduce_variant_launch(slab, dw_ref, Csmall, Cbig, nsplit, (hipStream_t)stream, ntaps, variant);
}
```

### vae_play_amd/engine.py

```python
from __future__ import annotations

import math
import os
from ctypes import c_void_p
from typing import Dict, Optional

import torch

from . import _lib, ops, parallel
from .networks import VAE
from .plan import FWD_PRODUCTS, PlanBuilder, _Plan, _ptr, grad_of, plan_device, side_ctx, sync_counters_on_state_dict

_ACT_NONE, _ACT_SIGMOID = ops.ACT_NONE, ops.ACT_SIGMOID


class FusedVAEStep:

    def __init__(self, vae: VAE, optimizer, batch_size: int, img_size: int, channels: int, group=None,
                 precision: str = "bf16x3", grad_scale16: float = 4096.0, _plan_only: bool = False):
        if precision not in ("f32", "bf16x3", "f16x2"):
            raise ValueError("precision must be 'f32', 'bf16x3' or 'f16x2'")
        if precision == "f16x2" and not (grad_scale16 > 0 and math.log2(grad_scale16).is_integer()):
            raise ValueError("grad_scale16 must be a positive power of two")
        self.precision = precision
        self.grad_scale16 = float(grad_scale16)
        self.vae, self.opt, self.B, self.S, self.C = vae, optimizer, batch_size, img_size, channels
        self.Z, self.L = vae.z_size, vae.iter_level
        self.group = group
        self.world = torch.distributed.get_world_size(group) if torch.distributed.is_initialized() else 1
        self.opt.grad_scale = 1.0 / self.world
        self.dev = plan_device(vae, "FusedVAEStep", _plan_only)
        self._bufs: Dict[str, torch.Tensor] = {}
        self._graph = None
        self.reload_switches()
        self._build()
        self._sd_hook = sync_counters_on_state_dict(self, vae)

    def reload_switches(self) -> None:
        env = os.environ.get
        self._side_wgrad = env("VP_SIDE_WGRAD", "1") != "0"
        self._adam_outer = env("VP_ADAM_OUTER", "1") != "0"
        self._adam_outer_early = int(env("VP_ADAM_OUTER_EARLY", "2"))
        self._dp_factored = env("VP_DP_FACTORED", "1") != "0"
        self._dp_enc_tail = env("VP_DP_ENC_TAIL", "1") != "0"

    def _build(self):
        B, S, C, Z, L = self.B, self.S, self.C, self.Z, self.L
        enc, dec = self.vae.encoder, self.vae.decoder
        env = os.environ.get
        fwd, bwd = _Plan(), _Plan()
        P = _ptr
        self._f16_sat = torch.zeros(1, dtype=torch.int32, device=self.dev)
        x3 = self.precision in ("bf16x3", "f16x2")
        b = PlanBuilder(self, self.dev, self.precision, side_on=x3,
                        wgrad_cus=(int(env("VP_WGRAD_MAIN_CUS", "0")), int(env("VP_WGRAD_SIDE_CUS", "160"))),
                        grad_scale16=self.grad_scale16, sat=self._f16_sat, fuse_stats=env("VP_FUSE_BN_STATS", "1") != "0")
        lib = b.lib
        x2 = b.x2
        FMT = 1 if x2 else 0
        GS = b.GS
        a16 = self.precision if x3 else "f32"

        def use16(cin, cout):
            return x3 and cin % 8 == 0 and cout % 8 == 0

        self.x_nchw = b.buf("x_nchw", B, C, S, S)
        self.eps = b.buf("eps", B, Z)
        x_nhwc = b.buf("x_nhwc", B * S * S * C)
        if C > 1:
            fwd.add("vp_nchw_to_nhwc_f32", P(self.x_nchw), P(x_nhwc), B, C, S, S)
        else:
            x_nhwc = self.x_nchw

        enc_ch = [C] + [blk.conv.weight.shape[0] for blk in enc.conv]
        sp = [S // (2 ** i) for i in range(L + 1)]
        enc16 = [use16(enc_ch[i], enc_ch[i + 1]) for i in range(L)]
        enc0_cols = x3 and C in (1, 3) and enc_ch[1] % 8 == 0
        enc0_cols32 = (not x3) and C in (1, 3) and enc_ch[1] % 16 == 0
        enc_in = [x_nhwc]
        enc_in_s = [None]
        enc_rec = []
        for i, blk in enumerate(enc.conv):
            if i == 1 and b.k_pack is not None:
                fwd.wait_side(b.k_pack)
            Cin, Cout, Hs = enc_ch[i], enc_ch[i + 1], sp[i + 1]
            n_out = B * Hs * Hs * Cout
            c = b.buf(f"enc{i}.c", n_out)
            fl = 50.0 * B * Hs * Hs * Cin * Cout
            geom = (B, Hs, Hs, Cin, Cout, 2)
            conv = None
            if i == 0 and enc0_cols:
                KC = lib.vp_im2col5s2_cols(Cin)
                xcol = b.sbuf("enc0.xcol", B * Hs * Hs * KC)
                w0s = b.sbuf("enc0.w0s", Cout * KC)
                if x2:
                    fwd.add("vp_im2col5s2_split_fmt_f32", P(self.x_nchw), P(xcol), B, Cin, S, S, 1, FMT)
                    fwd.add("vp_pack_w_im2col5_split_fmt", P(blk.conv.weight), P(w0s), Cout, Cin, FMT)
                    fwd.add("vp_conv_gather_f16", P(xcol), P(w0s), None, P(c), B, Hs, Hs, Hs, Hs, KC, Cout, 1, 1, _ACT_NONE, FWD_PRODUCTS, 1.0,
                            flops=fl, tag="enc0.fwd")
                else:
                    fwd.add("vp_im2col5s2_split_f32", P(self.x_nchw), P(xcol), B, Cin, S, S, 1)
                    fwd.add("vp_pack_w_im2col5_split", P(blk.conv.weight), P(w0s), Cout, Cin)
                    fwd.add("vp_conv_gather_bf16x3", P(xcol), P(w0s), None, P(c), B, Hs, Hs, Hs, Hs, KC, Cout, 1, 1, _ACT_NONE,
                            flops=fl, tag="enc0.fwd")
                p1, enc0 = None, (xcol, KC)
            elif i == 0 and enc0_cols32:
                KC = lib.vp_im2col5s2_cols(Cin)
                xcol = b.buf("enc0.xcol32", B * Hs * Hs * KC)
                w0 = b.buf("enc0.w0", Cout * KC)
                fwd.add("vp_im2col5s2_f32", P(self.x_nchw), P(xcol), B, Cin, S, S, 1)
                fwd.add("vp_pack_w_im2col5_f32", P(blk.conv.weight), P(w0), Cout, Cin)
                fwd.add("vp_conv_gather_f32", P(xcol), P(w0), None, P(c), B, Hs, Hs, Hs, Hs, KC, Cout, 1, 1, _ACT_NONE, flops=fl, tag="enc0.fwd")
                p1, enc0 = None, (xcol, KC)
            elif enc16[i]:
                p0 = b.sbuf(f"enc{i}.p0s", Cout * 25 * Cin)
                p1 = b.sbuf(f"enc{i}.p1s", Cin * 25 * Cout)
                b.pack(blk.conv.weight, p0, p1, Cout, Cin, True, first=(i == 0))
                conv = (0, a16, enc_in_s[-1], p0, geom, fl)
            else:
                p0 = b.buf(f"enc{i}.p0", Cout * 25 * Cin)
                p1 = b.buf(f"enc{i}.p1", Cin * 25 * Cout) if i > 0 else None
                b.pack(blk.conv.weight, p0, p1, Cout, Cin, False, first=(i == 0))
                conv = (0, "f32", enc_in[-1], p0, geom, fl)
            nxt16 = i + 1 < L and enc16[i + 1]
            a = None if nxt16 else b.buf(f"enc{i}.a", n_out)
            a_s = b.sbuf(f"enc{i}.as", n_out) if nxt16 else None
            saved = b.bn_fwd(fwd, f"enc{i}", c, B * Hs * Hs, Cout, blk.bn, a, a_s, conv=conv)
            enc_rec.append((blk, Cin, Cout, Hs, p1, c, saved))
            enc_in.append(a)
            enc_in_s.append(a_s)
        if L == 1 and b.k_pack is not None:
            fwd.wait_side(b.k_pack)
        size = enc_ch[-1]
        F0 = 64 * size
        flat = b.buf("enc.flat", B * F0)
        fwd.add("vp_nhwc_to_nchw_f32", P(enc_in[-1]), P(flat), B, size, 8, 8)
        fc_lin, fc_bn = enc.fc[0], enc.fc[1]
        h = b.buf("enc.h", B * 1024)
        hb = b.buf("enc.hb", B * 1024)
        b.lin_fwd(fwd, flat, fc_lin.weight, None, h, B, 1024, F0)
        h_saved = b.bn_fwd(fwd, "enc.fc", h, B, 1024, fc_bn, hb)
        self.mu, self.logvar = b.buf("mu", B, Z), b.buf("logvar", B, Z)
        for lin, out in ((enc.l_mu, self.mu), (enc.l_var, self.logvar)):
            b.lin_fwd(fwd, hb, lin.weight, lin.bias, out, B, Z, 1024)
        self.z, self.kl = b.buf("z", B, Z), b.buf("kl", B)
        fwd.add("vp_latent_fwd_f32", P(self.mu), P(self.logvar), P(self.eps), P(self.z), P(self.kl), B, Z)

        dfc_lin, dfc_bn = dec.fc[0], dec.fc[1]
        dsize = dec._c0
        F1 = 64 * dsize
        d = b.buf("dec.d", B * F1)
        db = b.buf("dec.db", B * F1)
        b.lin_fwd(fwd, self.z, dfc_lin.weight, None, d, B, F1, Z)
        d_saved = b.bn_fwd(fwd, "dec.fc", d, B, F1, dfc_bn, db)
        dec_ch = [dsize] + [blk.conv.weight.shape[1] for blk in list(dec.conv)[:L]]
        dec16 = [use16(dec_ch[i], dec_ch[i + 1]) for i in range(L)]
        dn = None if dec16[0] else b.buf("dec.in", B * F1)
        dn_s = b.sbuf("dec.in_s", B * F1) if dec16[0] else None
        if x2:
            fwd.add("vp_nchw_to_nhwc_split_fmt_f32", P(db), P(dn), P(dn_s), B, dsize, 8, 8, FMT)
        else:
            fwd.add("vp_nchw_to_nhwc_split_f32", P(db), P(dn), P(dn_s), B, dsize, 8, 8)

        dec_in = [dn]
        dec_in_s = [dn_s]
        dec_rec = []
        for i in range(L):
            blk = dec.conv[i]
            Cin, Cout, Hs = dec_ch[i], dec_ch[i + 1], 8 * (2 ** i)
            n_out = B * 4 * Hs * Hs * Cout
            tbuf = b.buf(f"dec{i}.t", n_out)
            fl = 50.0 * B * Hs * Hs * Cin * Cout
            geom = (B, Hs, Hs, Cin, Cout, 2)
            if dec16[i]:
                p1 = b.sbuf(f"dec{i}.p1s", Cout * 25 * Cin)
                p0 = b.sbuf(f"dec{i}.p0s", Cin * 25 * Cout)
                b.pack(blk.conv.weight, p0, p1, Cin, Cout, True)
                conv = (1, a16, dec_in_s[-1], p1, geom, fl)
            else:
                p1 = b.buf(f"dec{i}.p1", Cout * 25 * Cin)
                p0 = b.buf(f"dec{i}.p0", Cin * 25 * Cout)
                b.pack(blk.conv.weight, p0, p1, Cin, Cout, False)
                conv = (1, "f32", dec_in[-1], p1, geom, fl)
            nxt16 = i + 1 < L and dec16[i + 1]
            u = None if nxt16 else b.buf(f"dec{i}.u", n_out)
            u_s = b.sbuf(f"dec{i}.us", n_out) if nxt16 else None
            saved = b.bn_fwd(fwd, f"dec{i}", tbuf, B * 4 * Hs * Hs, Cout, blk.bn, u, u_s, conv=conv)
            dec_rec.append((blk, Cin, Cout, Hs, p0, tbuf, saved))
            dec_in.append(u)
            dec_in_s.append(u_s)
        fin = dec.conv[L][0]
        Cf = dec_ch[-1]
        fl_fin = 50.0 * B * S * S * Cf * C
        fp0 = b.buf("fin.p0", C * 25 * Cf)
        fp1 = b.buf("fin.p1", Cf * 25 * C)
        b.pack(fin.weight, fp0, fp1, C, Cf, False)
        xt_nhwc = b.buf("xt_nhwc", B * S * S * C)
        if x3 and Cf == 64 and C in (1, 3):
            fwd.add("vp_conv5_smallout_bf16x3", P(dec_in[-1]), P(fp0), P(fin.bias), P(xt_nhwc), B, S, S, Cf, C, _ACT_SIGMOID,
                    flops=fl_fin, tag="fin.fwd")
        else:
            b.conv5(fwd, 0, "f32", dec_in[-1], fp0, xt_nhwc, (B, S, S, Cf, C, 1), bias=fin.bias, act=_ACT_SIGMOID,
                    flops=fl_fin, tag="fin.fwd")
        self.recon = b.buf("recon", 1)
        self.kl_sum = b.buf("kl_sum", 1)
        n_pix = B * S * S * C
        ws_red = b.ws("red.ws", lib.vp_reduce_workspace_bytes(n_pix))
        self._loss_num = b.buf("loss_num", 1)
        fwd.add("vp_vae_loss_f32", P(xt_nhwc), P(x_nhwc), n_pix, P(self.kl), B, P(self.recon), P(self.kl_sum), P(self._loss_num),
                1.0 / B, P(ws_red), ws_red.numel() * 4)
        self.xt_nhwc = xt_nhwc
        self.x_tilde = xt_nhwc.view(B, S, S, C).permute(0, 3, 1, 2)
        fwd.hook("fwd_done")

        inv_b = 1.0 / B
        dlogit = b.buf("g.dlogit", n_pix)
        fin_rowk = x3 and Cf == 64 and C in (1, 3)
        fin16 = x3 and Cf % 8 == 0 and C < 8 and not fin_rowk
        if fin16:
            dlogit_s = b.sbuf("g.dlogit_s", B * S * S * 8)
            fp1s = b.sbuf("fin.p1s", Cf * 25 * 8)
            b.pack(fin.weight, None, fp1s, C, Cf, True, 8, bf16=True)
            bwd.add("vp_bce_sigmoid_bwd_pad_split_f32", P(xt_nhwc), P(x_nhwc), inv_b, P(dlogit), P(dlogit_s), B * S * S, C, 8)
        else:
            bwd.add("vp_bce_sigmoid_bwd_f32", P(xt_nhwc), P(x_nhwc), inv_b, P(dlogit), n_pix)
        b.colsum(bwd, "g.fin", dlogit, grad_of(fin.bias), B * S * S, C, side=b.side_slot())
        ws_wg = b.wgrad_workspace([(B, r[3], r[1], r[2]) for r in enc_rec] + [(B, r[3], r[2], r[1]) for r in dec_rec],
                                  at_least=lib.vp_conv5_wgrad_workspace_bytes(B, S, S, Cf, C, 1))
        n_tapm = lib.vp_conv5_smallout_wgrad_bf16x3_workspace_bytes(B, S, S, Cf, C)
        if n_tapm:
            ws_fw = b.ws("g.finwgrad.ws", n_tapm)
            bwd.add("vp_conv5_smallout_wgrad_bf16x3" if x3 else "vp_conv5_smallout_wgrad_f32", P(dec_in[-1]), P(dlogit), P(grad_of(fin.weight)),
                    B, S, S, Cf, C, P(ws_fw), ws_fw.numel() * 4, flops=fl_fin, tag="fin.wgrad", side=b.side_slot())
        else:
            bwd.add("vp_conv5_wgrad_f32", P(dec_in[-1]), P(dlogit), P(grad_of(fin.weight)), B, S, S, Cf, C, 1, P(ws_wg), ws_wg.numel() * 4,
                    flops=fl_fin, tag="fin.wgrad", side=b.side_slot())
        big = max([B * F0, B * F1, n_pix] + [B * 4 * r[3] * r[3] * r[2] for r in dec_rec] + [B * r[3] * r[3] * r[2] for r in enc_rec]
                  + [B * S * S * Cf])
        gA, gB = b.buf("g.A", big), b.buf("g.B", big)
        if fin_rowk:
            bwd.add("vp_conv5_smallin_dgrad_bf16x3", P(dlogit), P(fin.weight), P(gA), B, S, S, C, Cf, flops=fl_fin, tag="fin.dgrad")
        elif fin16:
            b.conv5(bwd, 1, "bf16x3", dlogit_s, fp1s, gA, (B, S, S, 8, Cf, 1), flops=fl_fin, tag="fin.dgrad")
        elif Cf == 64 and C in (1, 3):
            bwd.add("vp_conv5_smallin_dgrad_f32", P(dlogit), P(fin.weight), P(gA), B, S, S, C, Cf, flops=fl_fin, tag="fin.dgrad")
        else:
            b.conv5(bwd, 1, "f32", dlogit, fp1, gA, (B, S, S, C, Cf, 1), flops=fl_fin, tag="fin.dgrad")
        cur, other = gA, gB
        gS2 = b.grad_planes(big)
        self._grad_planes = gS2 if x2 else []
        for i in range(L - 1, -1, -1):
            blk, Cin, Cout, Hs, p0, tbuf, saved = dec_rec[i]
            R = B * 4 * Hs * Hs
            fl = 50.0 * B * Hs * Hs * Cin * Cout
            geom = (B, Hs, Hs, Cout, Cin, 2)
            if dec16[i]:
                k, gS = b.next_plane(bwd)
                b.bn_bwd(bwd, tbuf, cur, None, R, Cout, blk.bn, saved, gS)
                b.wgrad5(bwd, gS, dec_in_s[i], grad_of(blk.conv.weight), geom, k, flops=fl, tag=f"dec{i}.wgrad")
                b.conv5(bwd, 0, a16, gS, p0, cur, geom, products=2, alpha=1.0 / GS, flops=fl, tag=f"dec{i}.dgrad")
            else:
                b.bn_bwd(bwd, tbuf, cur, other, R, Cout, blk.bn, saved)
                bwd.add("vp_conv5_wgrad_f32", P(other), P(dec_in[i]), P(grad_of(blk.conv.weight)), *geom,
                        P(ws_wg), ws_wg.numel() * 4, flops=fl, tag=f"dec{i}.wgrad")
                b.conv5(bwd, 0, "f32", other, p0, cur, geom, flops=fl, tag=f"dec{i}.dgrad")
        bwd.add("vp_nhwc_to_nchw_f32", P(cur), P(other), B, dsize, 8, 8)
        b.bn_bwd(bwd, d, other, cur, B, F1, dfc_bn, d_saved)
        b.lin_wgrad(bwd, cur, self.z, grad_of(dfc_lin.weight), B, F1, Z)
        dz = b.buf("g.dz", B, Z)
        b.lin_dgrad(bwd, cur, dfc_lin.weight, dz, B, F1, Z)
        bwd.hook("dec_done")
        dmu, dlv = b.buf("g.dmu", B, Z), b.buf("g.dlv", B, Z)
        bwd.add("vp_latent_bwd_f32", P(self.mu), P(self.logvar), P(self.eps), P(dz), None, inv_b, P(dmu), P(dlv), B, Z)
        dhb_a, dhb_b = b.buf("g.dhb_a", B * 1024), b.buf("g.dhb_b", B * 1024)
        for lin, dsrc, dst in ((enc.l_mu, dmu, dhb_a), (enc.l_var, dlv, dhb_b)):
            b.lin_wgrad(bwd, dsrc, hb, grad_of(lin.weight), B, Z, 1024)
            b.colsum(bwd, "g.heads", dsrc, grad_of(lin.bias), B, Z)
            b.lin_dgrad(bwd, dsrc, lin.weight, dst, B, Z, 1024)
        bwd.add("vp_add_f32", P(dhb_a), P(dhb_b), P(dhb_a), B * 1024)
        dh = b.buf("g.dh", B * 1024)
        b.bn_bwd(bwd, h, dhb_a, dh, B, 1024, fc_bn, h_saved)
        bwd.hook("fc_wgrad", replaces_next=True)
        b.lin_wgrad(bwd, dh, flat, grad_of(fc_lin.weight), B, 1024, F0)
        self._fc_factors = (dh, flat, fc_lin.weight, F0)
        b.lin_dgrad(bwd, dh, fc_lin.weight, gA, B, 1024, F0)
        bwd.hook("enc_dense_done")
        bwd.add("vp_nchw_to_nhwc_f32", P(gA), P(gB), B, size, 8, 8)
        cur, other = gB, gA
        self._bwd_b_enc_tail = self._enc_tail_first = None
        for i in range(L - 1, -1, -1):
            blk, Cin, Cout, Hs, p1, c, saved = enc_rec[i]
            R = B * Hs * Hs
            fl = 50.0 * B * Hs * Hs * Cin * Cout
            geom = (B, Hs, Hs, Cin, Cout, 2)
            if i == 0 and enc0_cols:
                xcol, KC = enc0
                k, gS = b.next_plane(bwd)
                b.bn_bwd(bwd, c, cur, None, R, Cout, blk.bn, saved, gS)
                dwc = b.buf("enc0.dwc", Cout * KC)
                ws0 = b.ws("enc0.wgws", lib.vp_conv_wgrad_bf16x3_workspace_bytes(B, Hs, Hs, Hs, Hs, KC, Cout, 1, 1))
                if x2:
                    bwd.add("vp_conv_wgrad_f16x2", P(xcol), P(gS), P(dwc), B, Hs, Hs, Hs, Hs, KC, Cout, 1, 1, 1.0 / GS, P(ws0), ws0.numel() * 4,
                            flops=fl, tag="enc0.wgrad")
                else:
                    bwd.add("vp_conv_wgrad_bf16x3", P(xcol), P(gS), P(dwc), B, Hs, Hs, Hs, Hs, KC, Cout, 1, 1, P(ws0), ws0.numel() * 4,
                            flops=fl, tag="enc0.wgrad")
                bwd.add("vp_unpack_dw_im2col5_f32", P(dwc), P(grad_of(blk.conv.weight)), Cout, Cin)
            elif enc16[i]:
                k, gS = b.next_plane(bwd)
                b.bn_bwd(bwd, c, cur, None, R, Cout, blk.bn, saved, gS)
                b.wgrad5(bwd, enc_in_s[i], gS, grad_of(blk.conv.weight), geom, k, flops=fl, tag=f"enc{i}.wgrad")
                if i > 0:
                    b.conv5(bwd, 1, a16, gS, p1, cur, (B, Hs, Hs, Cout, Cin, 2), products=2, alpha=1.0 / GS,
                            flops=fl, tag=f"enc{i}.dgrad")
                if i == max(L - 2, 1):
                    self._bwd_b_enc_tail, self._enc_tail_first = len(bwd.calls), i
                    bwd.hook("enc_tail")
            elif i == 0 and enc0_cols32:
                xcol, KC = enc0
                b.bn_bwd(bwd, c, cur, other, R, Cout, blk.bn, saved)
                dwc = b.buf("enc0.dwc", Cout * KC)
                ws0 = b.ws("enc0.wgws", lib.vp_conv_wgrad_workspace_bytes(B, Hs, Hs, Hs, Hs, KC, Cout, 1, 1))
                bwd.add("vp_conv_wgrad_f32", P(xcol), P(other), P(dwc), B, Hs, Hs, Hs, Hs, KC, Cout, 1, 1, P(ws0), ws0.numel() * 4,
                        flops=fl, tag="enc0.wgrad")
                bwd.add("vp_unpack_dw_im2col5_f32", P(dwc), P(grad_of(blk.conv.weight)), Cout, Cin)
            else:
                b.bn_bwd(bwd, c, cur, other, R, Cout, blk.bn, saved)
                bwd.add("vp_conv5_wgrad_f32", P(enc_in[i]), P(other), P(grad_of(blk.conv.weight)), *geom,
                        P(ws_wg), ws_wg.numel() * 4, flops=fl, tag=f"enc{i}.wgrad", side=(b.side_slot() if i == 0 else None))
                if i > 0:
                    b.conv5(bwd, 1, "f32", other, p1, cur, (B, Hs, Hs, Cout, Cin, 2), flops=fl, tag=f"enc{i}.dgrad")
        b.finish(fwd)
        self._fwd, self._bwd = fwd, bwd
        self._bn_momentum_eps = {id(bn): (float(bn.momentum), float(bn.eps)) for bn, _ in b.bn_counts}
        self._bn_mods = [m for m in self.vae.modules() if hasattr(m, "num_batches_tracked")]

    def _launch_all(self, timers: Optional[dict] = None, hooks: Optional[dict] = None):
        s = torch.cuda.current_stream().cuda_stream
        side = self._side_ctx() if timers is None else None
        self._fwd.run(s, timers, side=side, hooks=hooks)
        self._bwd.run(s, timers, side=side, hooks=hooks)
        if side is not None:
            side.join()

    def _side_ctx(self):
        return side_ctx(self, self._side_wgrad)

    def forward_backward(self, x: torch.Tensor, eps: torch.Tensor, timers: Optional[dict] = None, hooks: Optional[dict] = None):
        self._bind_inputs(x, eps)
        if self._graph is not None and timers is None and not hooks:
            self._graph.replay()
        else:
            self._launch_all(timers, hooks)
        self.opt.arena.adopt_views()
        self._steps_since_sync = getattr(self, "_steps_since_sync", 0) + 1
        return self._loss_num, self.recon, self.kl_sum

    def _bind_inputs(self, x: torch.Tensor, eps: torch.Tensor) -> None:
        if not hasattr(self, "_in_slots"):
            self._in_slots = {"x": [], "eps": []}
            statics = {"x": self.x_nchw.data_ptr(), "eps": self.eps.data_ptr()}
            if self.C != 1:
                for plan in (self._fwd, self._bwd):
                    for call in plan.calls:
                        for i, a in enumerate(call[2]):
                            if isinstance(a, c_void_p):
                                for k, v in statics.items():
                                    if a.value == v:
                                        self._in_slots[k].append((call[2], i))
        for key, t, static in (("x", x, self.x_nchw), ("eps", eps, self.eps)):
            if tuple(t.shape) != tuple(static.shape):
                raise _lib.VaePlayHipError(
                    f"FusedVAEStep: {key} has shape {tuple(t.shape)}, this plan was built for {tuple(static.shape)} "
                    f"(batch {self.B}; build a second FusedVAEStep over the same optimiser for another batch size)")
            slots = self._in_slots[key]
            direct = (bool(slots) and self._graph is None and t.device == static.device and t.dtype == torch.float32
                      and t.is_contiguous() and t.shape == static.shape)
            if not direct:
                static.copy_(t, non_blocking=True)
                t = static
            for args, i in slots:
                args[i] = c_void_p(t.data_ptr())

    def f16_saturated(self) -> int:
        n = 0
        for t in getattr(self, "_grad_planes", []):
            hi = t[0].view(torch.float16)
            n += int((hi.abs() >= 65504.0).sum().item())
        return n

    def sync_counters(self):
        n = getattr(self, "_steps_since_sync", 0)
        if n:
            for m in self._bn_mods:
                m.num_batches_tracked.add_(n)
            self._steps_since_sync = 0
        if self.precision == "f16x2" and int(self._f16_sat.item()):
            self._f16_sat.zero_()
            raise _lib.VaePlayHipError(
                f"precision='f16x2': gradient planes saturated fp16's range since the last sync_counters() (|g| * grad_scale16 > 65504 "
                f"with grad_scale16 = {self.grad_scale16:g}); build the step with a smaller power of two")

    def _decoder_slice_start(self) -> int:
        dec_ids = {id(p) for p in self.vae.decoder.parameters()}
        offs = [o for p, o in zip(self.opt.arena.params, self.opt.arena.offsets) if id(p) in dec_ids]
        first = min(offs)
        assert all(o >= first for o in offs) and all(
            (id(p) in dec_ids) == (o >= first) for p, o in zip(self.opt.arena.params, self.opt.arena.offsets)), \
            "decoder parameters must form the tail of the flat arena"
        return first

    def _encoder_dense_start(self) -> int:
        a = self.opt.arena
        off = {id(p): o for p, o in zip(a.params, a.offsets)}
        first = off[id(self.vae.encoder.fc[0].weight)]
        conv_ids = {id(p) for p in self.vae.encoder.conv.parameters()}
        assert all((id(p) in conv_ids) == (o < first) for p, o in zip(a.params, a.offsets) if o < self._decoder_slice_start()), \
            "encoder conv parameters must form the head of the flat arena"
        return first

    def step(self, x: torch.Tensor, eps: torch.Tensor, timers: Optional[dict] = None, overlap: bool = True, comm_trace=None):
        tr = comm_trace

        def reduce(name, t):
            if tr is not None:
                return tr.issue(name, "all_reduce", t.numel() * 4, lambda: parallel.allreduce_flat_grads(t, self.group, async_op=True))
            return parallel.allreduce_flat_grads(t, self.group, async_op=True)

        def gather(name, out_all, local):
            if tr is not None:
                return tr.issue(name, "all_gather", out_all.numel() * 4,
                                lambda: parallel.allgather_rows(out_all, local, self.group, async_op=True))
            return parallel.allgather_rows(out_all, local, self.group, async_op=True)

        def wait_all(works):
            if tr is not None:
                tr.wait()
                return
            for w in works:
                if w is not None:
                    w.wait()

        if parallel.dp_active(self.group) and overlap:
            g = self.opt.flat_grad
            cut = self._decoder_slice_start()
            dense = self._encoder_dense_start()
            works = []
            factored = self._dp_factored

            def dec_bucket(side):
                if side is not None:
                    side.join()
                works.append(reduce("decoder", g[cut:]))
            hooks = {"dec_done": dec_bucket}
            tail_lo = dense
            if self._enc_tail_first is not None and self._dp_enc_tail:
                off = {id(p): o for p, o in zip(self.opt.arena.params, self.opt.arena.offsets)}
                tail_lo = off[id(self.vae.encoder.conv[self._enc_tail_first].conv.weight)]
            if tail_lo < dense:
                def enc_tail(side):
                    def issue():
                        works.append(reduce("encoder.conv[deep]", g[tail_lo:dense]))
                    if side is not None:
                        side.run(issue)
                    else:
                        issue()
                hooks["enc_tail"] = enc_tail
            if factored:
                dh, flat, fcw, F0 = self._fc_factors
                W, B = self.world, self.B
                if not hasattr(self, "_fc_all"):
                    self._fc_all = (torch.empty((W * B, 1024), device=self.dev), torch.empty((W * B, F0), device=self.dev))
                dh_all, flat_all = self._fc_all
                gathers = []
                fc_lo = self.opt.arena.offsets[[id(p) for p in self.opt.arena.params].index(id(fcw))]
                fc_hi = fc_lo + (fcw.numel() + 63) // 64 * 64

                def after_fwd(side):
                    gathers.append(gather("fc.0 factor: flat", flat_all, flat.view(B, F0)))

                def fc_wgrad(side):
                    gathers.append(gather("fc.0 factor: dh", dh_all, dh.view(B, 1024)))
                    wait_all(gathers)
                    ops.gemm(dh_all, 1, 1024, flat_all, 1, F0, 1024, F0, W * B, 2, out=self.opt.arena.grad_view(fcw).view(1024, F0))

                def dense_bucket(side):
                    assert fc_lo == dense, "fc.0.weight must open the encoder's dense slice"
                    works.append(reduce("encoder dense (without fc.0)", g[fc_hi:cut]))
                hooks.update(fwd_done=after_fwd, fc_wgrad=fc_wgrad, enc_dense_done=dense_bucket)
            else:
                hooks["enc_dense_done"] = lambda side: works.append(reduce("encoder dense", g[dense:cut]))
            out = self.forward_backward(x, eps, timers, hooks=hooks)
            works.append(reduce("encoder.conv[shallow]" if tail_lo < dense else "encoder.conv", g[:tail_lo]))
            wait_all(works)
        elif self.world == 1 and self._graph is None and self._outer_adam():
            hooks = {"fc_wgrad": lambda side: None}
            if timers is None and self._adam_outer_early:
                def early(side):
                    if side is not None:
                        side.run(lambda: self.opt.step_outer_early(
                            with_tail=(self._adam_outer_early == 2 and getattr(self, "_early_tail_ok", False))))
                hooks["enc_dense_done"] = early
# ... 48 lines not shown
```

### vae_play_amd/plan.py

```python
from __future__ import annotations

import weakref
from ctypes import c_void_p
from typing import Dict, List, Optional

import torch

from . import _lib, ops

_ACT_RELU, _ACT_NONE = ops.ACT_RELU, ops.ACT_NONE


class _Plan:

    def __init__(self):
        self.calls: List[list] = []

    def add(self, name: str, *args, flops: float = 0.0, tag: str = "", side: Optional[int] = None, side_args: Optional[dict] = None):
        fn = getattr(_lib.load(), name)
        a = list(args) + [None]
        self.calls.append([name, fn, a, len(a) - 1, flops, tag, side, side_args])

    def add_first(self, name: str, *args, side: Optional[int] = None):
        fn = getattr(_lib.load(), name)
        a = list(args) + [None]
        self.calls.insert(0, [name, fn, a, len(a) - 1, 0.0, "", side, None])

    def wait_side(self, k: int):
        self.calls.append(["__wait_side__", None, [k], 0, 0.0, "", None, None])

    def hook(self, key: str, replaces_next: bool = False):
        self.calls.append(["__hook__", None, [key, replaces_next], 0, 0.0, "", None, None])

    def run(self, stream_ptr: int, timers: Optional[dict] = None, side: Optional["_SideCtx"] = None, hooks: Optional[dict] = None):
        s = c_void_p(stream_ptr)
        it = iter(enumerate(self.calls))
        for ci, (name, fn, a, slot, flops, tag, sev, sargs) in it:
            if fn is None:
                if name == "__hook__":
                    if hooks is not None and a[0] in hooks:
                        hooks[a[0]](side)
                        if a[1]:
                            next(it)
                elif side is not None:
                    torch.cuda.current_stream().wait_event(side.events[a[0]])
                continue
            on_side = side is not None and sev is not None
            if sargs is not None:
                for idx, (v_main, v_side) in sargs.items():
                    a[idx] = v_side if on_side else v_main
            if on_side:
                a[slot] = c_void_p(side.stream.cuda_stream)
                side.launch(name, fn, a, sev)
                continue
            a[slot] = s
            timed = timers is not None and name in timers["names"]
            if timed:
                pool = timers.get("pool")
                if pool is not None:
                    key = (id(self), ci, timers.get("slot", 0))
                    if key not in pool:
                        pool[key] = (torch.cuda.Event(enable_timing=True), torch.cuda.Event(enable_timing=True))
                    e0, e1 = pool[key]
                else:
                    e0, e1 = torch.cuda.Event(enable_timing=True), torch.cuda.Event(enable_timing=True)
                e0.record()
            rc = fn(*a)
            if timed:
                e1.record()
                timers["events"].append((name, tag, flops, e0, e1))
            if rc != 0:
                _lib.check(rc, name)


class _SideCtx:

    def __init__(self, n_events: int):
        self.stream = torch.cuda.Stream()
        self.events = [torch.cuda.Event() for _ in range(n_events)]
        self.fork = torch.cuda.Event()

    def launch(self, name, fn, args, k: int):
        self.fork.record()
        self.stream.wait_event(self.fork)
        rc = fn(*args)
        self.events[k].record(self.stream)
        if rc != 0:
            _lib.check(rc, name)

    def run(self, fn):
        self.fork.record()
        self.stream.wait_event(self.fork)
        with torch.cuda.stream(self.stream):
            fn()

    def join(self):
        torch.cuda.current_stream().wait_stream(self.stream)


def _ptr(t: Optional[torch.Tensor]):
    return None if t is None else c_void_p(t.data_ptr())


def side_ctx(step, enabled: bool = True) -> Optional[_SideCtx]:
    if not step._n_side_events or not enabled:
        return None
    if getattr(step, "_side", None) is None:
        step._side = _SideCtx(step._n_side_events)
    return step._side


def plan_device(module: torch.nn.Module, what: str, plan_only: bool) -> torch.device:
    dev = next(module.parameters()).device
    if dev.type != "cuda" and not plan_only:
        raise _lib.VaePlayHipError(f"{what} needs the model on the HIP device")
    return dev


def sync_counters_on_state_dict(step, module: torch.nn.Module):
    me = weakref.ref(step)

    def _sync(mod, prefix, keep_vars):
        o = me()
        if o is not None:
            o.sync_counters()
    return module.register_state_dict_pre_hook(_sync)


def grad_of(p: torch.nn.Parameter) -> torch.Tensor:
    arena = getattr(p, "_vp_arena", None)
    if arena is None:
        raise _lib.VaePlayHipError("parameter has no arena gradient; build the optimiser first")
    return arena.grad_view(p)


_CONV5 = {
    ("f32", False): ("vp_conv5_gather_f32", "vp_conv5_scatter_f32"),
    ("f32", True): ("vp_conv5_gather_stats_f32", "vp_conv5_scatter_stats_f32"),
    ("bf16x3", False): ("vp_conv5_gather_bf16x3", "vp_conv5_scatter_bf16x3"),
    ("bf16x3", True): ("vp_conv5_gather_stats_bf16x3", "vp_conv5_scatter_stats_bf16x3"),
    ("f16x2", False): ("vp_conv5_gather_f16", "vp_conv5_scatter_f16"),
    ("f16x2", True): ("vp_conv5_gather_stats_f16", "vp_conv5_scatter_stats_f16"),
}
_CONV5_STATS_WS = {"f32": "vp_conv5_stats_f32_workspace_bytes", "bf16x3": "vp_conv5_stats_workspace_bytes",
                   "f16x2": "vp_conv5_stats_f16_workspace_bytes"}
FWD_PRODUCTS = 3


class PlanBuilder:

    def __init__(self, step, dev, precision: str, side_on: bool, wgrad_cus, grad_scale16: float = 1.0, sat=None,
                 fuse_stats: bool = True):
        self.lib = _lib.load()
        self.step, self.dev, self.precision = step, dev, precision
        self.x3 = precision in ("bf16x3", "f16x2")
        self.x2 = precision == "f16x2"
        self.GS = grad_scale16 if self.x2 else 1.0
        self.sat = sat
        self.side_on, self.wgrad_cus, self.fuse_stats = side_on, tuple(wgrad_cus), fuse_stats
        self.bufs: Dict[str, torch.Tensor] = step._bufs
        self.n_side = 0
        self.bn_counts: List[tuple] = []
        self._gemm_calls, self._gemm_need = [], 0
        self._pack_jobs, self._first_pack_jobs = [], []
        self.k_pack = self.side_slot()

    def buf(self, name: str, *shape) -> torch.Tensor:
        t = torch.empty(shape, dtype=torch.float32, device=self.dev)
        assert name not in self.bufs, name
        self.bufs[name] = t
        return t

    def ws(self, name: str, nbytes: int) -> torch.Tensor:
        return self.buf(name, max(4, (int(nbytes) + 3) // 4))

    def sbuf(self, name: str, n: int) -> torch.Tensor:
        t = torch.empty((2, n), dtype=torch.int16, device=self.dev)
        assert name not in self.bufs, name
        self.bufs[name] = t
        return t

    def side_slot(self) -> Optional[int]:
        if not self.side_on:
            return None
        self.n_side += 1
        return self.n_side - 1

    def grad_planes(self, n: int, depth: int = 2):
        self.planes = [self.sbuf(f"g.S{j}", n) for j in range(depth)] if self.x3 else [None] * depth
        self._plane_reader = [None] * depth
        self._plane_turn = 0
        return self.planes

    def next_plane(self, plan: _Plan):
        k = self._plane_turn % len(self.planes)
        self._plane_turn += 1
        if self._plane_reader[k] is not None:
            plan.wait_side(self._plane_reader[k])
            self._plane_reader[k] = None
        return k, self.planes[k]

    def pack(self, weight, p0, p1, Cs, Cb, split, Cs_pad=0, first=False, bf16=False):
        fmt = (2 if (self.x2 and not bf16) else 1) if split else 0
        (self._first_pack_jobs if (first and self.k_pack is not None) else self._pack_jobs).append(
            _lib.PackJob(weight.data_ptr(), p0.data_ptr() if p0 is not None else None, p1.data_ptr() if p1 is not None else None,
                         Cs, Cb, Cs_pad, fmt))

    def _gemm(self, plan, A, sam, sak, Bm, sbn, sbk, C, ldc, bias, M, N, K, mode):
        self._gemm_need = max(self._gemm_need, self.lib.vp_gemm_workspace_bytes(M, N, K))
        plan.add("vp_gemm_f32", A, sam, sak, Bm, sbn, sbk, C, ldc, bias, M, N, K, mode, None, 0)
        self._gemm_calls.append(plan.calls[-1][2])

    def lin_fwd(self, plan, x, W, bias, y, M, N, K):
        self._gemm(plan, _ptr(x), K, 1, _ptr(W), K, 1, _ptr(y), N, _ptr(bias), M, N, K, 0)

    def lin_dgrad(self, plan, dy, W, dx, M, N, K):
        self._gemm(plan, _ptr(dy), N, 1, _ptr(W), 1, K, _ptr(dx), K, None, M, K, N, 1)

    def lin_wgrad(self, plan, dy, x, dW, M, N, K):
        self._gemm(plan, _ptr(dy), 1, N, _ptr(x), 1, K, _ptr(dW), K, None, N, K, M, 2)

    def colsum(self, plan, tag, x, out, R, C, side=None):
        nbytes = self.lib.vp_colsum_workspace_bytes(R, C)
        ws = self.bufs.get(f"{tag}.csws")
        if ws is None:
            ws = self.ws(f"{tag}.csws", nbytes)
        assert ws.numel() * 4 >= nbytes, tag
        plan.add("vp_colsum_f32", _ptr(x), _ptr(out), R, C, _ptr(ws), ws.numel() * 4, side=side)

    def bn_fwd(self, plan, tag, x, R, Cn, bn, y, y_s=None, count=1, conv=None):
        P = _ptr
        mean, rstd = self.buf(f"{tag}.mean", Cn), self.buf(f"{tag}.rstd", Cn)
        mom, eps = float(bn.momentum), float(bn.eps)
        self.bn_counts.append((bn, count))
        if conv is None and y_s is None and R <= 64 and Cn % 4 == 0:
            plan.add("vp_bn_small_fwd_f32", P(x), R, Cn, eps, mom, P(bn.weight), P(bn.bias), P(mean), P(rstd), P(bn.running_mean),
                     P(bn.running_var), P(y), _ACT_RELU, 0.0)
            return mean, rstd, None
        ws = self.ws(f"{tag}.bnws", self.lib.vp_bn_workspace_bytes(R, Cn))
        fused = conv is not None and self._conv5_fwd(plan, tag, conv, x, bn, eps, mom, mean, rstd)
        if not fused:
            plan.add("vp_bn_stats_f32", P(x), R, Cn, eps, mom, P(mean), P(rstd), P(bn.running_mean), P(bn.running_var),
                     P(ws), ws.numel() * 4)
        if self.x2 and y_s is not None:
            plan.add("vp_bn_act_fwd_split_fmt_f32", P(x), P(mean), P(rstd), P(bn.weight), P(bn.bias), P(y), P(y_s), R, Cn,
                     _ACT_RELU, 0.0, 1)
        else:
            plan.add("vp_bn_act_fwd_split_f32", P(x), P(mean), P(rstd), P(bn.weight), P(bn.bias), P(y), P(y_s), R, Cn, _ACT_RELU, 0.0)
        return mean, rstd, ws

    def _conv5_fwd(self, plan, tag, conv, x, bn, eps, mom, mean, rstd) -> bool:
        P = _ptr
        family, arith, a, w, geom, fl = conv
        qgeom = geom if family == 0 else (geom[0], geom[1], geom[2], geom[4], geom[3], geom[5])
        nst = getattr(self.lib, _CONV5_STATS_WS[arith])(family, *qgeom) if self.fuse_stats else 0
        products = (FWD_PRODUCTS,) if arith == "f16x2" else ()
        name = _CONV5[(arith, bool(nst))][family]
        if nst:
            st = self.ws(f"{tag}.statws", nst)
            plan.add(name, P(a), P(w), P(x), *geom, *products, eps, mom, P(mean), P(rstd), P(bn.running_mean), P(bn.running_var),
                     P(st), st.numel() * 4, flops=fl, tag=f"{tag}.fwd")
            return True
        self.conv5(plan, family, arith, a, w, x, geom, flops=fl, tag=f"{tag}.fwd")
        return False

    def conv5(self, plan, family, arith, a, w, out, geom, products=FWD_PRODUCTS, alpha=1.0, bias=None, act=_ACT_NONE, **kw):
        P = _ptr
        name = _CONV5[(arith, False)][family]
        tail = (products, alpha) if arith == "f16x2" else ()
        if family == 0:
            plan.add(name, P(a), P(w), P(bias), P(out), *geom, act, *tail, **kw)
        else:
            plan.add(name, P(a), P(w), P(out), *geom, *tail, **kw)

    def bn_fold(self, plan, tag, bn):
        P = _ptr
        Cn = bn.running_mean.numel()
        scale, shift, rstd = self.buf(f"{tag}.scale", Cn), self.buf(f"{tag}.shift", Cn), self.buf(f"{tag}.rstd", Cn)
        plan.add("vp_bn_fold_f32", P(bn.weight), P(bn.bias), P(bn.running_mean), P(bn.running_var), float(bn.eps), P(scale), P(shift),
                 P(rstd), Cn, tag=f"{tag}.fold")
        return scale, shift, rstd

    def conv5_bn_eval(self, plan, tag, family, arith, a, w, geom, bn, folded, y, y_s=None, flops=0.0) -> bool:
        P = _ptr
        scale, shift, rstd = folded
        qgeom = geom if family == 0 else (geom[0], geom[1], geom[2], geom[4], geom[3], geom[5])
        if self.lib.vp_conv5_affine_supported(family, 1 if arith == "f32" else 0, *qgeom):
            name = ("vp_conv5_gather_affine_", "vp_conv5_scatter_affine_")[family] + arith
            plan.add(name, P(a), P(w), P(scale), P(shift), P(y), P(y_s), *geom, _ACT_RELU, flops=flops, tag=f"{tag}.fwd")
            return True
        Bn, Hs, Ws, stride = geom[0], geom[1], geom[2], geom[5]
        Cout = geom[4]
        R = Bn * Hs * Ws * (stride * stride if family == 1 else 1)
        c = self.buf(f"{tag}.c", R * Cout)
        self.conv5(plan, family, arith, a, w, c, geom, flops=flops, tag=f"{tag}.fwd")
        self.bn_eval(plan, tag, c, R, Cout, bn, rstd, y, y_s)
        return False

    def bn_eval(self, plan, tag, x, R, Cn, bn, rstd, y, y_s=None):
        P = _ptr
        if y_s is None:
            plan.add("vp_bn_act_fwd_f32", P(x), P(bn.running_mean), P(rstd), P(bn.weight), P(bn.bias), P(y), R, Cn, _ACT_RELU, 0.0,
                     tag=f"{tag}.bn")
        else:
            plan.add("vp_bn_act_fwd_split_f32", P(x), P(bn.running_mean), P(rstd), P(bn.weight), P(bn.bias), P(y), P(y_s), R, Cn,
                     _ACT_RELU, 0.0, tag=f"{tag}.bn")

    def bn_bwd(self, plan, x, dy, dx, R, Cn, bn, saved, dx_s=None, gfn=grad_of):
        P = _ptr
        mean, rstd, ws = saved
        if dx_s is None and R <= 64 and Cn % 4 == 0:
            plan.add("vp_bn_small_bwd_f32", P(x), P(dy), P(mean), P(rstd), P(bn.weight), P(bn.bias), P(dx), P(gfn(bn.weight)),
                     P(gfn(bn.bias)), R, Cn, _ACT_RELU, 0.0, 1)
        elif self.x2 and dx_s is not None:
            plan.add("vp_bn_act_bwd_split_fmt_sat_f32", P(x), P(dy), P(mean), P(rstd), P(bn.weight), P(bn.bias), P(dx), P(dx_s),
                     P(gfn(bn.weight)), P(gfn(bn.bias)), R, Cn, _ACT_RELU, 0.0, 1, 1, self.GS, P(self.sat), P(ws), ws.numel() * 4)
        else:
            plan.add("vp_bn_act_bwd_split_f32", P(x), P(dy), P(mean), P(rstd), P(bn.weight), P(bn.bias), P(dx), P(dx_s),
                     P(gfn(bn.weight)), P(gfn(bn.bias)), R, Cn, _ACT_RELU, 0.0, 1, P(ws), ws.numel() * 4)

    def wgrad_workspace(self, layers, at_least: int = 0) -> torch.Tensor:
        n = at_least
        for Bn, Hs, Cbig, Csmall in layers:
            n = max(n, self.lib.vp_conv5_wgrad_workspace_bytes(Bn, Hs, Hs, Cbig, Csmall, 2),
                    self.lib.vp_conv5_wgrad_bf16x3_workspace_bytes(Bn, Hs, Hs, Cbig, Csmall, 2))
        self.ws_wg = self.ws("g.wgrad.ws", n)
        return self.ws_wg

    def wgrad5(self, plan, big_s, small_s, dw, geom, plane: int, **kw):
        P, ws = _ptr, self.ws_wg
        k = self.side_slot()
        self._plane_reader[plane] = k
        if self.x2:
            plan.add("vp_conv5_wgrad_f16x2_cus", P(big_s), P(small_s), P(dw), *geom, 1.0 / self.GS, 0, P(ws), ws.numel() * 4,
                     side=k, side_args={4 + len(geom): self.wgrad_cus}, **kw)
        else:
            plan.add("vp_conv5_wgrad_bf16x3_cus", P(big_s), P(small_s), P(dw), *geom, 0, P(ws), ws.numel() * 4,
                     side=k, side_args={3 + len(geom): self.wgrad_cus}, **kw)

    def finish(self, fwd: _Plan):
        step = self.step
        step._pack_jobs = (_lib.PackJob * len(self._pack_jobs))(*self._pack_jobs)
        fwd.add_first("vp_pack_w5_batch", step._pack_jobs, len(self._pack_jobs), side=self.k_pack)
        if self._first_pack_jobs:
            step._pack_jobs0 = (_lib.PackJob * len(self._first_pack_jobs))(*self._first_pack_jobs)
            fwd.add_first("vp_pack_w5_batch", step._pack_jobs0, len(self._first_pack_jobs))
        wsg = self.ws("gemm.ws", self._gemm_need)
        for a in self._gemm_calls:
            a[13], a[14] = _ptr(wsg), wsg.numel() * 4
        step._n_side_events = self.n_side
```

Before: 9340 images/sec.

## Fuse last decoder BatchNorm+ReLU into final conv forward and weight-grad loads

The final decoder BatchNorm+ReLU is no longer applied as a separate pass that writes an activation buffer. The final 5x5 conv forward kernel and its weight-gradient kernel now read the pre-activation and apply the normalisation and ReLU in registers as they load each tile, using per-channel constants held in LDS or registers. This removes one full-resolution 64-channel write and re-read per step. In exchange the conv kernels do extra arithmetic on every load, and the activation is only rebuilt on demand through a lazily computed buffer for debugging or inspection.

```diff
diff --git a/include/vaeplay_hip.h b/include/vaeplay_hip.h
--- a/include/vaeplay_hip.h
+++ b/include/vaeplay_hip.h
@@ -68,6 +68,12 @@
 size_t vp_conv5_smallout_wgrad_bf16x3_workspace_bytes(int B, int H, int W, int Cbig, int Csmall);
 int vp_conv5_smallout_wgrad_bf16x3(const float* big, const float* small, float* dw_ref, int B, int H, int W, int Cbig, int Csmall,
                                    void* ws, size_t ws_bytes, vp_stream stream);
+int vp_conv5_smallout_bn_bf16x3(const float* pre, const float* mean, const float* rstd, const float* gamma, const float* beta, int act_in,
+                                const float* w_p0, const float* bias, float* small_out, int B, int H, int W, int Cbig, int Csmall, int act,
+                                vp_stream stream);
+int vp_conv5_smallout_bn_wgrad_bf16x3(const float* pre, const float* mean, const float* rstd, const float* gamma, const float* beta,
+                                      int act_in, const float* small, float* dw_ref, int B, int H, int W, int Cbig, int Csmall, void* ws,
+                                      size_t ws_bytes, vp_stream stream);
 size_t vp_conv5_smallout_wgrad_f32_workspace_bytes(int B, int H, int W, int Cbig, int Csmall);
 int vp_conv5_smallout_wgrad_f32(const float* big, const float* small, float* dw_ref, int B, int H, int W, int Cbig, int Csmall,
                                 void* ws, size_t ws_bytes, vp_stream stream);
diff --git a/vae_play_amd/_lib.py b/vae_play_amd/_lib.py
--- a/vae_play_amd/_lib.py
+++ b/vae_play_amd/_lib.py
@@ -44,6 +44,8 @@
     "vp_conv5_smallout_bf16x3": (c_int, [P, P, P, P] + [c_int] * 6 + [P]),
     "vp_conv5_smallout_wgrad_bf16x3_workspace_bytes": (c_size_t, [c_int] * 5),
     "vp_conv5_smallout_wgrad_bf16x3": (c_int, [P, P, P] + [c_int] * 5 + [P, c_size_t, P]),
+    "vp_conv5_smallout_bn_bf16x3": (c_int, [P] * 5 + [c_int, P, P, P] + [c_int] * 6 + [P]),
+    "vp_conv5_smallout_bn_wgrad_bf16x3": (c_int, [P] * 5 + [c_int, P, P] + [c_int] * 5 + [P, c_size_t, P]),
     "vp_conv5_smallout_wgrad_f32_workspace_bytes": (c_size_t, [c_int] * 5),
     "vp_conv5_smallout_wgrad_f32": (c_int, [P, P, P] + [c_int] * 5 + [P, c_size_t, P]),
     "vp_im2col5s2_cols": (c_int, [c_int]),
diff --git a/vae_play_amd/csrc/bn.hip b/vae_play_amd/csrc/bn.hip
--- a/vae_play_amd/csrc/bn.hip
+++ b/vae_play_amd/csrc/bn.hip
@@ -2,6 +2,7 @@
 #include "common.h"
 #include "problems.h"
 #include "split.h"
+#include "bn_apply.h"
 
 namespace vp {
 
@@ -25,18 +26,6 @@
   return g;
 }
 
-__device__ __forceinline__ float act_apply(float v, int act, float slope) {
-  switch (act) {
-    case ACT_RELU: return v > 0.f ? v : 0.f;
-    case ACT_LRELU: return v > 0.f ? v : v * slope;
-    case ACT_TANH: return tanhf(v);
-    case ACT_SIGMOID: return 1.f / (1.f + __expf(-v));
-    default: return v;
-  }
-}
-__device__ __forceinline__ float bn_pre(float x, float mu, float rs, float ga, float be) {
-  return fmaf(ga, (x - mu) * rs, be);
-}
 __device__ __forceinline__ float act_grad_pre(float u, int act, float slope) {
   switch (act) {
     case ACT_RELU: return u > 0.f ? 1.f : 0.f;
diff --git a/vae_play_amd/csrc/bn_apply.h b/vae_play_amd/csrc/bn_apply.h
--- /dev/null
+++ b/vae_play_amd/csrc/bn_apply.h
@@ -0,0 +1,20 @@
+#pragma once
+#include <hip/hip_runtime.h>
+#include "problems.h"
+
+namespace vp {
+
+__device__ __forceinline__ float act_apply(float v, int act, float slope) {
+  switch (act) {
+    case ACT_RELU: return v > 0.f ? v : 0.f;
+    case ACT_LRELU: return v > 0.f ? v : v * slope;
+    case ACT_TANH: return tanhf(v);
+    case ACT_SIGMOID: return 1.f / (1.f + __expf(-v));
+    default: return v;
+  }
+}
+__device__ __forceinline__ float bn_pre(float x, float mu, float rs, float ga, float be) {
+  return fmaf(ga, (x - mu) * rs, be);
+}
+
+}
diff --git a/vae_play_amd/csrc/conv16.hip b/vae_play_amd/csrc/conv16.hip
--- a/vae_play_amd/csrc/conv16.hip
+++ b/vae_play_amd/csrc/conv16.hip
@@ -499,4 +499,16 @@
   return tapn_gather_launch(big, w_p0, bias, small_out, g, act, (hipStream_t)stream);
 }
 
-}
+int vp_conv5_smallout_bn_bf16x3(const float* pre, const float* mean, const float* rstd, const float* gamma, const float* beta, int act_in,
+                                const float* w_p0, const float* bias, float* small_out, int B, int H, int W, int Cbig, int Csmall, int act,
+                                vp_stream stream) {
+  VP_REQUIRE(pre && mean && rstd && w_p0 && small_out && B > 0 && H > 0 && W > 0, "vp_conv5_smallout_bn_bf16x3: bad arguments");
+  VP_REQUIRE(((uintptr_t)pre & 15) == 0 && ((uintptr_t)w_p0 & 15) == 0, "vp_conv5_smallout_bn_bf16x3: operands must be 16-byte aligned");
+  VP_REQUIRE(act_in == VP_ACT_NONE || act_in == VP_ACT_RELU, "vp_conv5_smallout_bn_bf16x3: input activation none|relu");
+  const ConvGeom g = make_geom(B, H, W, Csmall, Cbig, 1);
+  VP_REQUIRE(tapn_gather_applicable(g, act) && Cbig == 64, "vp_conv5_smallout_bn_bf16x3: needs 64 input channels, 1 or 3 outputs, act none|sigmoid");
+  const TapnBn bn = {mean, rstd, gamma, beta, act_in};
+  return tapn_gather_launch(pre, w_p0, bias, small_out, g, act, (hipStream_t)stream, &bn);
+}
+
+}
diff --git a/vae_play_amd/csrc/edge.hip b/vae_play_amd/csrc/edge.hip
--- a/vae_play_amd/csrc/edge.hip
+++ b/vae_play_amd/csrc/edge.hip
@@ -4,12 +4,16 @@
 #include "igemm16.h"
 #include "narrow.h"
 #include "split.h"
+#include "bn_apply.h"
 
 namespace vp {
 
-template <int NOUT, int TH>
+template <int NOUT, int TH, bool BN = false>
 __global__ void __launch_bounds__(256, 2) wgrad_tapm_kernel(const float* __restrict__ u, const float* __restrict__ dlogit,
-                                                            float* __restrict__ slab, int H, int W, int bands_per_img) {
+                                                            float* __restrict__ slab, int H, int W, int bands_per_img,
+                                                            const float* __restrict__ mean = nullptr, const float* __restrict__ rstd = nullptr,
+                                                            const float* __restrict__ gamma = nullptr, const float* __restrict__ beta = nullptr,
+                                                            int act_in = ACT_NONE) {
   constexpr int C = 64, NCOL = 25 * NOUT, MT = (NCOL + 31) / 32;
   constexpr int SS = 64;
   constexpr int US = KmStride<64>::bytes;
@@ -47,6 +51,21 @@
 
   const int spx = tid >> 2, sch = (tid & 3) * 16;
   vp_f32x4 st[4];
+  const bool relu_in = act_in == ACT_RELU;
+  vp_f32x4 cmu[BN ? 4 : 1], crs[BN ? 4 : 1], cga[BN ? 4 : 1], cbe[BN ? 4 : 1];
+  if (BN) {
+#pragma unroll
+    for (int v = 0; v < (BN ? 4 : 1); ++v) {
+#pragma unroll
+      for (int j = 0; j < 4; ++j) {
+        const int c = sch + 4 * v + j;
+        cmu[v][j] = mean[c];
+        crs[v][j] = rstd[c];
+        cga[v][j] = gamma ? gamma[c] : 1.f;
+        cbe[v][j] = beta ? beta[c] : 0.f;
+      }
+    }
+  }
   const int nss = TH * W / SS;
   auto load_ss = [&](int ss) {
     const int p0 = ss * SS + spx;
@@ -61,7 +80,17 @@
     for (int v = 0; v < 4; ++v) {
       u16x4_t h, l;
 #pragma unroll
-      for (int j = 0; j < 4; ++j) { u16_t a, c; split_f32(st[v][j], a, c); h[j] = a; l[j] = c; }
+      for (int j = 0; j < 4; ++j) {
+        float x = st[v][j];
+        if (BN) {
+          x = bn_pre(x, cmu[BN ? v : 0][j], crs[BN ? v : 0][j], cga[BN ? v : 0][j], cbe[BN ? v : 0][j]);
+          if (relu_in) x = act_apply(x, ACT_RELU, 0.f);
+        }
+        u16_t a, c;
+        split_f32(x, a, c);
+        h[j] = a;
+        l[j] = c;
+      }
       *reinterpret_cast<u16x4_t*>(base + 8 * v) = h;
       *reinterpret_cast<u16x4_t*>(base + UPLANE + 8 * v) = l;
     }
@@ -260,11 +289,22 @@
   return (size_t)2 * 2 * UPLANE + (size_t)2 * g.Cs * (TAPM_TH + 4) * PC * 2 + 64;
 }
 
-int tapm_wgrad_launch(const float* big_f32, const float* small_f32, float* dw_ref, const ConvGeom& g, float* ws, hipStream_t s) {
+int tapm_wgrad_launch(const float* big_f32, const float* small_f32, float* dw_ref, const ConvGeom& g, float* ws, hipStream_t s,
+                      const TapnBn* bn = nullptr) {
   const int bands = g.Hs / TAPM_TH, nblk = g.B * bands;
   const size_t lds = tapm_lds_bytes(g);
   if (lds > 160 * 1024) return fail(VP_ERR_ARG, "wgrad_tapm: image too wide for the LDS patch");
-  if (g.Cs == 3) {
+  if (bn && g.Cs == 3) {
+    static bool attr3b = false;
+    if (!attr3b) { (void)hipFuncSetAttribute((const void*)wgrad_tapm_kernel<3, TAPM_TH, true>, hipFuncAttributeMaxDynamicSharedMemorySize, 160 * 1024); attr3b = true; }
+    hipLaunchKernelGGL((wgrad_tapm_kernel<3, TAPM_TH, true>), dim3(nblk), dim3(256), lds, s, big_f32, small_f32, ws, g.Hs, g.Ws, bands,
+                       bn->mean, bn->rstd, bn->gamma, bn->beta, bn->act);
+  } else if (bn) {
+    static bool attr1b = false;
+    if (!attr1b) { (void)hipFuncSetAttribute((const void*)wgrad_tapm_kernel<1, TAPM_TH, true>, hipFuncAttributeMaxDynamicSharedMemorySize, 160 * 1024); attr1b = true; }
+    hipLaunchKernelGGL((wgrad_tapm_kernel<1, TAPM_TH, true>), dim3(nblk), dim3(256), lds, s, big_f32, small_f32, ws, g.Hs, g.Ws, bands,
+                       bn->mean, bn->rstd, bn->gamma, bn->beta, bn->act);
+  } else if (g.Cs == 3) {
     static bool attr3 = false;
     if (!attr3) { (void)hipFuncSetAttribute((const void*)wgrad_tapm_kernel<3, TAPM_TH>, hipFuncAttributeMaxDynamicSharedMemorySize, 160 * 1024); attr3 = true; }
     hipLaunchKernelGGL((wgrad_tapm_kernel<3, TAPM_TH>), dim3(nblk), dim3(256), lds, s, big_f32, small_f32, ws, g.Hs, g.Ws, bands);
@@ -521,6 +561,19 @@
   return tapm_wgrad_launch(big, small, dw_ref, g, (float*)ws, (hipStream_t)stream);
 }
 
+int vp_conv5_smallout_bn_wgrad_bf16x3(const float* pre, const float* mean, const float* rstd, const float* gamma, const float* beta,
+                                      int act_in, const float* small, float* dw_ref, int B, int H, int W, int Cbig, int Csmall, void* ws,
+                                      size_t ws_bytes, vp_stream stream) {
+  VP_REQUIRE(pre && mean && rstd && small && dw_ref && ws && B > 0 && H > 0 && W > 0, "vp_conv5_smallout_bn_wgrad_bf16x3: bad arguments");
+  VP_REQUIRE(((uintptr_t)pre & 15) == 0, "vp_conv5_smallout_bn_wgrad_bf16x3: the pre-activation must be 16-byte aligned");
+  VP_REQUIRE(act_in == VP_ACT_NONE || act_in == VP_ACT_RELU, "vp_conv5_smallout_bn_wgrad_bf16x3: input activation none|relu");
+  const ConvGeom g = make_geom(B, H, W, Csmall, Cbig, 1);
+  VP_REQUIRE(tapm_wgrad_applicable(g), "vp_conv5_smallout_bn_wgrad_bf16x3: needs 64 input channels, 1 or 3 outputs, width a multiple of 64, height of 8");
+  if (ws_bytes < tapm_wgrad_ws_floats(g) * sizeof(float)) return fail(VP_ERR_WORKSPACE, "vp_conv5_smallout_bn_wgrad_bf16x3: workspace too small");
+  const TapnBn bn = {mean, rstd, gamma, beta, act_in};
+  return tapm_wgrad_launch(pre, small, dw_ref, g, (float*)ws, (hipStream_t)stream, &bn);
+}
+
 size_t vp_conv5_smallout_wgrad_f32_workspace_bytes(int B, int H, int W, int Cbig, int Csmall) {
   return vp_conv5_smallout_wgrad_bf16x3_workspace_bytes(B, H, W, Cbig, Csmall);
 }
diff --git a/vae_play_amd/csrc/narrow.h b/vae_play_amd/csrc/narrow.h
--- a/vae_play_amd/csrc/narrow.h
+++ b/vae_play_amd/csrc/narrow.h
@@ -6,7 +6,9 @@
 bool narrow_gather_applicable(const ConvGeom& g, int act);
 int narrow_gather_launch(const float* big, const float* w_p0, const float* bias, float* out, const ConvGeom& g, int act, hipStream_t s);
 bool tapn_gather_applicable(const ConvGeom& g, int act);
-int tapn_gather_launch(const float* big, const float* w_p0, const float* bias, float* out, const ConvGeom& g, int act, hipStream_t s);
+struct TapnBn { const float *mean, *rstd, *gamma, *beta; int act; };
+int tapn_gather_launch(const float* big, const float* w_p0, const float* bias, float* out, const ConvGeom& g, int act, hipStream_t s,
+                       const TapnBn* bn = nullptr);
 int narrow_wgrad_kind(const ConvGeom& g);
 size_t narrow_wgrad_ws_floats(const ConvGeom& g);
 int narrow_wgrad_launch(const float* big, const float* small, float* dw_ref, const ConvGeom& g, float* ws, hipStream_t s);
diff --git a/vae_play_amd/csrc/narrow.hip b/vae_play_amd/csrc/narrow.hip
--- a/vae_play_amd/csrc/narrow.hip
+++ b/vae_play_amd/csrc/narrow.hip
@@ -3,6 +3,7 @@
 #include "common.h"
 #include "problems.h"
 #include "narrow.h"
+#include "bn_apply.h"
 
 namespace vp {
 
@@ -341,10 +342,14 @@
   }
 }
 
-template <int NOUT, int C>
+template <int NOUT, int C, bool BN = false>
 __global__ void __launch_bounds__(512, 2) conv5s1_tapn_kernel(const float* __restrict__ in, const float* __restrict__ w,
                                                               const float* __restrict__ bias, float* __restrict__ out,
-                                                              int H, int W, int tiles_x, int tiles_per_img, int ntiles, int act) {
+                                                              int H, int W, int tiles_x, int tiles_per_img, int ntiles, int act,
+                                                              const float* __restrict__ mean = nullptr,
+                                                              const float* __restrict__ rstd = nullptr,
+                                                              const float* __restrict__ gamma = nullptr,
+                                                              const float* __restrict__ beta = nullptr, int act_in = ACT_NONE) {
   static_assert(C == 64 || C == 32, "64 input channels (the VAE's final conv) or 32 (input gradient of a 1|3 -> 32 first conv)");
   constexpr int T = 16, HALO = T + 4, NPIX = HALO * HALO;
   constexpr int NS = C / 16, NRAW = C / 8, HC = C / 2;
@@ -353,8 +358,18 @@
   constexpr int MT = (NPIX + 31) / 32;
   constexpr int NWAVE = 8;
   __shared__ float P[NPIX * PITCH];
+  __shared__ __attribute__((aligned(16))) float bnc[BN ? 4 : 1][BN ? C : 4];
   const int tid = threadIdx.x, lane = tid & 63, wave = tid >> 6;
   const int li = lane & 31, lh = lane >> 5;
+  if (BN) {
+    if (tid < C) {
+      bnc[0][tid] = mean[tid];
+      bnc[1][tid] = rstd[tid];
+      bnc[2][tid] = gamma ? gamma[tid] : 1.f;
+      bnc[3][tid] = beta ? beta[tid] : 0.f;
+    }
+    __syncthreads();
+  }
 
   bf16x8_e bh[NT][NS], bl[NT][NS];
 #pragma unroll
@@ -372,7 +387,7 @@
     }
   }
 
-  auto load_tile = [&](int tile, int t, vp_f32x4 (&raw)[NRAW]) {
+  auto load_tile = [&](int tile, int t, vp_f32x4 (&raw)[NRAW]) -> bool {
     const int b = tile / tiles_per_img, rem = tile - b * tiles_per_img;
     const int h0 = (rem / tiles_x) * T, w0 = (rem % tiles_x) * T;
     const int pi = 32 * t + li;
@@ -382,15 +397,34 @@
     const float* q = in + ((size_t)(b * H + (ok ? gh : 0)) * W + (ok ? gw : 0)) * C + HC * lh;
 #pragma unroll
     for (int v = 0; v < NRAW; ++v) raw[v] = ok ? ld4(q + 4 * v) : zero4();
+    return ok;
+  };
+  const bool relu_in = act_in == ACT_RELU;
+  auto bn_apply4 = [&](vp_f32x4& x, int v, bool ok) {
+    int c0 = HC * lh + 4 * v;
+    asm volatile("" : "+v"(c0));
+    const vp_f32x4 mu = *reinterpret_cast<const vp_f32x4*>(&bnc[0][c0]), rs = *reinterpret_cast<const vp_f32x4*>(&bnc[BN ? 1 : 0][c0]);
+    const vp_f32x4 ga = *reinterpret_cast<const vp_f32x4*>(&bnc[BN ? 2 : 0][c0]), be = *reinterpret_cast<const vp_f32x4*>(&bnc[BN ? 3 : 0][c0]);
+#pragma unroll
+    for (int j = 0; j < 4; ++j) {
+      float y = bn_pre(x[j], mu[j], rs[j], ga[j], be[j]);
+      if (relu_in) y = act_apply(y, ACT_RELU, 0.f);
+      x[j] = ok ? y : 0.f;
+    }
   };
   vp_f32x4 cur[NRAW], nxt[NRAW];
-  if ((int)blockIdx.x < ntiles && wave < MT) load_tile(blockIdx.x, wave, cur);
+  bool cur_ok = false, nxt_ok = false;
+  if ((int)blockIdx.x < ntiles && wave < MT) cur_ok = load_tile(blockIdx.x, wave, cur);
   for (int tile = blockIdx.x; tile < ntiles; tile += gridDim.x) {
     const int b = tile / tiles_per_img, rem = tile - b * tiles_per_img;
     const int h0 = (rem / tiles_x) * T, w0 = (rem % tiles_x) * T;
     for (int t = wave; t < MT; t += NWAVE) {
       const bool more = t + NWAVE < MT;
-      if (more) load_tile(tile, t + NWAVE, nxt);
+      if (more) nxt_ok = load_tile(tile, t + NWAVE, nxt);
+      if (BN) {
+#pragma unroll
+        for (int v = 0; v < NRAW; ++v) bn_apply4(cur[v], v, cur_ok);
+      }
       f32x16_e acc[NT];
 #pragma unroll
       for (int jt = 0; jt < NT; ++jt)
@@ -417,13 +451,16 @@
       if (more) {
 #pragma unroll
         for (int v = 0; v < NRAW; ++v) cur[v] = nxt[v];
+        cur_ok = nxt_ok;
       }
     }
     const int ntile = tile + (int)gridDim.x;
-    if (ntile < ntiles && wave < MT) load_tile(ntile, wave, cur);
-    __syncthreads();
-    if (tid < T * T) {
-      const int tx = tid % T, ty = tid / T;
+    if (ntile < ntiles && wave < MT) cur_ok = load_tile(ntile, wave, cur);
+    __syncthreads();
+    int tid_s = tid;
+    if (BN) asm volatile("" : "+v"(tid_s));
+    if (tid_s < T * T) {
+      const int tx = tid_s % T, ty = tid_s / T;
       const int h = h0 + ty, ww = w0 + tx;
       float sum[NOUT];
 #pragma unroll
@@ -457,9 +494,18 @@
 bool tapn_gather_applicable(const ConvGeom& g, int act) {
   return narrow_gather_applicable(g, act) && (g.Cb == 64 || g.Cb == 32);
 }
-int tapn_gather_launch(const float* big, const float* w_p0, const float* bias, float* out, const ConvGeom& g, int act, hipStream_t s) {
+int tapn_gather_launch(const float* big, const float* w_p0, const float* bias, float* out, const ConvGeom& g, int act, hipStream_t s,
+                       const TapnBn* bn) {
   const int tiles_x = (g.Ws + 15) / 16, tiles_per_img = tiles_x * ((g.Hs + 15) / 16), ntiles = tiles_per_img * g.B;
   const dim3 pgrid((unsigned)(ntiles < 256 ? ntiles : 256));
+  if (bn) {
+#define VP_TAPN_BN(NO) hipLaunchKernelGGL((conv5s1_tapn_kernel<NO, 64, true>), pgrid, dim3(512), 0, s, big, w_p0, bias, out, g.Hs, g.Ws, tiles_x, \
+                                          tiles_per_img, ntiles, act, bn->mean, bn->rstd, bn->gamma, bn->beta, bn->act)
+    if (g.Cb != 64) return fail(VP_ERR_ARG, "conv5s1_tapn: BatchNorm on load needs 64 input channels");
+    if (g.Cs == 3) VP_TAPN_BN(3); else VP_TAPN_BN(1);
+#undef VP_TAPN_BN
+    return check_launch("conv5s1_tapn(bn)");
+  }
 #define VP_TAPN(NO, CC) hipLaunchKernelGGL((conv5s1_tapn_kernel<NO, CC>), pgrid, dim3(512), 0, s, big, w_p0, bias, out, g.Hs, g.Ws, tiles_x, tiles_per_img, ntiles, act)
   if (g.Cb == 64) { if (g.Cs == 3) VP_TAPN(3, 64); else VP_TAPN(1, 64); }
   else { if (g.Cs == 3) VP_TAPN(3, 32); else VP_TAPN(1, 32); }
diff --git a/vae_play_amd/engine.py b/vae_play_amd/engine.py
--- a/vae_play_amd/engine.py
+++ b/vae_play_amd/engine.py
@@ -9,9 +9,9 @@
 
 from . import _lib, ops, parallel
 from .networks import VAE
-from .plan import FWD_PRODUCTS, PlanBuilder, _Plan, _ptr, grad_of, plan_device, side_ctx, sync_counters_on_state_dict
-
-_ACT_NONE, _ACT_SIGMOID = ops.ACT_NONE, ops.ACT_SIGMOID
+from .plan import FWD_PRODUCTS, DerivedBufs, PlanBuilder, _Plan, _ptr, grad_of, plan_device, side_ctx, sync_counters_on_state_dict
+
+_ACT_NONE, _ACT_RELU, _ACT_SIGMOID = ops.ACT_NONE, ops.ACT_RELU, ops.ACT_SIGMOID
 
 
 class FusedVAEStep:
@@ -30,7 +30,7 @@
         self.world = torch.distributed.get_world_size(group) if torch.distributed.is_initialized() else 1
         self.opt.grad_scale = 1.0 / self.world
         self.dev = plan_device(vae, "FusedVAEStep", _plan_only)
-        self._bufs: Dict[str, torch.Tensor] = {}
+        self._bufs: Dict[str, torch.Tensor] = DerivedBufs()
         self._graph = None
         self.reload_switches()
         self._build()
@@ -43,6 +43,7 @@
         self._adam_outer_early = int(env("VP_ADAM_OUTER_EARLY", "2"))
         self._dp_factored = env("VP_DP_FACTORED", "1") != "0"
         self._dp_enc_tail = env("VP_DP_ENC_TAIL", "1") != "0"
+        self._fin_bn_on_load = env("VP_FIN_BN_ON_LOAD", "1") != "0"
 
     def _build(self):
         B, S, C, Z, L = self.B, self.S, self.C, self.Z, self.L
@@ -165,6 +166,9 @@
         dec_in = [dn]
         dec_in_s = [dn_s]
         dec_rec = []
+        Cf = dec.conv[L - 1].conv.weight.shape[1]
+        fin_on_load = (self._fin_bn_on_load and x3 and Cf == 64 and C in (1, 3)
+                       and lib.vp_conv5_smallout_wgrad_bf16x3_workspace_bytes(B, S, S, Cf, C) != 0)
         for i in range(L):
             blk = dec.conv[i]
             Cin, Cout, Hs = dec_ch[i], dec_ch[i + 1], 8 * (2 ** i)
@@ -183,20 +187,27 @@
                 b.pack(blk.conv.weight, p0, p1, Cin, Cout, False)
                 conv = (1, "f32", dec_in[-1], p1, geom, fl)
             nxt16 = i + 1 < L and dec16[i + 1]
-            u = None if nxt16 else b.buf(f"dec{i}.u", n_out)
+            on_load = fin_on_load and i == L - 1
+            u = None if (nxt16 or on_load) else b.buf(f"dec{i}.u", n_out)
             u_s = b.sbuf(f"dec{i}.us", n_out) if nxt16 else None
-            saved = b.bn_fwd(fwd, f"dec{i}", tbuf, B * 4 * Hs * Hs, Cout, blk.bn, u, u_s, conv=conv)
+            saved = b.bn_fwd(fwd, f"dec{i}", tbuf, B * 4 * Hs * Hs, Cout, blk.bn, u, u_s, conv=conv, apply=not on_load)
+            if on_load:
+                b.derived_act(f"dec{i}.u", tbuf, B * 4 * Hs * Hs, Cout, blk.bn, saved[0], saved[1])
             dec_rec.append((blk, Cin, Cout, Hs, p0, tbuf, saved))
             dec_in.append(u)
             dec_in_s.append(u_s)
         fin = dec.conv[L][0]
-        Cf = dec_ch[-1]
+        assert Cf == dec_ch[-1]
+        fin_t, fin_bn, (fin_mean, fin_rstd, _) = dec_rec[-1][5], dec_rec[-1][0].bn, dec_rec[-1][6]
         fl_fin = 50.0 * B * S * S * Cf * C
         fp0 = b.buf("fin.p0", C * 25 * Cf)
         fp1 = b.buf("fin.p1", Cf * 25 * C)
         b.pack(fin.weight, fp0, fp1, C, Cf, False)
         xt_nhwc = b.buf("xt_nhwc", B * S * S * C)
-        if x3 and Cf == 64 and C in (1, 3):
+        if fin_on_load:
+            fwd.add("vp_conv5_smallout_bn_bf16x3", P(fin_t), P(fin_mean), P(fin_rstd), P(fin_bn.weight), P(fin_bn.bias), _ACT_RELU, P(fp0),
+                    P(fin.bias), P(xt_nhwc), B, S, S, Cf, C, _ACT_SIGMOID, flops=fl_fin, tag="fin.fwd", timed_as="vp_conv5_smallout_bf16x3")
+        elif x3 and Cf == 64 and C in (1, 3):
             fwd.add("vp_conv5_smallout_bf16x3", P(dec_in[-1]), P(fp0), P(fin.bias), P(xt_nhwc), B, S, S, Cf, C, _ACT_SIGMOID,
                     flops=fl_fin, tag="fin.fwd")
         else:
@@ -228,7 +239,12 @@
         ws_wg = b.wgrad_workspace([(B, r[3], r[1], r[2]) for r in enc_rec] + [(B, r[3], r[2], r[1]) for r in dec_rec],
                                   at_least=lib.vp_conv5_wgrad_workspace_bytes(B, S, S, Cf, C, 1))
         n_tapm = lib.vp_conv5_smallout_wgrad_bf16x3_workspace_bytes(B, S, S, Cf, C)
-        if n_tapm:
+        if fin_on_load:
+            ws_fw = b.ws("g.finwgrad.ws", n_tapm)
+            bwd.add("vp_conv5_smallout_bn_wgrad_bf16x3", P(fin_t), P(fin_mean), P(fin_rstd), P(fin_bn.weight), P(fin_bn.bias), _ACT_RELU,
+                    P(dlogit), P(grad_of(fin.weight)), B, S, S, Cf, C, P(ws_fw), ws_fw.numel() * 4, flops=fl_fin, tag="fin.wgrad",
+                    side=b.side_slot(), timed_as="vp_conv5_smallout_wgrad_bf16x3")
+        elif n_tapm:
             ws_fw = b.ws("g.finwgrad.ws", n_tapm)
             bwd.add("vp_conv5_smallout_wgrad_bf16x3" if x3 else "vp_conv5_smallout_wgrad_f32", P(dec_in[-1]), P(dlogit), P(grad_of(fin.weight)),
                     B, S, S, Cf, C, P(ws_fw), ws_fw.numel() * 4, flops=fl_fin, tag="fin.wgrad", side=b.side_slot())
@@ -348,6 +364,7 @@
 
     def forward_backward(self, x: torch.Tensor, eps: torch.Tensor, timers: Optional[dict] = None, hooks: Optional[dict] = None):
         self._bind_inputs(x, eps)
+        self._fwd_epoch = ops.PARAM_EPOCH[0]
         if self._graph is not None and timers is None and not hooks:
             self._graph.replay()
         else:
diff --git a/vae_play_amd/plan.py b/vae_play_amd/plan.py
--- a/vae_play_amd/plan.py
+++ b/vae_play_amd/plan.py
@@ -16,26 +16,27 @@
     def __init__(self):
         self.calls: List[list] = []
 
-    def add(self, name: str, *args, flops: float = 0.0, tag: str = "", side: Optional[int] = None, side_args: Optional[dict] = None):
+    def add(self, name: str, *args, flops: float = 0.0, tag: str = "", side: Optional[int] = None, side_args: Optional[dict] = None,
+            timed_as: Optional[str] = None):
         fn = getattr(_lib.load(), name)
         a = list(args) + [None]
-        self.calls.append([name, fn, a, len(a) - 1, flops, tag, side, side_args])
+        self.calls.append([name, fn, a, len(a) - 1, flops, tag, side, side_args, timed_as or name])
 
     def add_first(self, name: str, *args, side: Optional[int] = None):
         fn = getattr(_lib.load(), name)
         a = list(args) + [None]
-        self.calls.insert(0, [name, fn, a, len(a) - 1, 0.0, "", side, None])
+        self.calls.insert(0, [name, fn, a, len(a) - 1, 0.0, "", side, None, name])
 
     def wait_side(self, k: int):
-        self.calls.append(["__wait_side__", None, [k], 0, 0.0, "", None, None])
+        self.calls.append(["__wait_side__", None, [k], 0, 0.0, "", None, None, None])
 
     def hook(self, key: str, replaces_next: bool = False):
-        self.calls.append(["__hook__", None, [key, replaces_next], 0, 0.0, "", None, None])
+        self.calls.append(["__hook__", None, [key, replaces_next], 0, 0.0, "", None, None, None])
 
     def run(self, stream_ptr: int, timers: Optional[dict] = None, side: Optional["_SideCtx"] = None, hooks: Optional[dict] = None):
         s = c_void_p(stream_ptr)
         it = iter(enumerate(self.calls))
-        for ci, (name, fn, a, slot, flops, tag, sev, sargs) in it:
+        for ci, (name, fn, a, slot, flops, tag, sev, sargs, tname) in it:
             if fn is None:
                 if name == "__hook__":
                     if hooks is not None and a[0] in hooks:
@@ -54,7 +55,7 @@
                 side.launch(name, fn, a, sev)
                 continue
             a[slot] = s
-            timed = timers is not None and name in timers["names"]
+            timed = timers is not None and tname in timers["names"]
             if timed:
                 pool = timers.get("pool")
                 if pool is not None:
@@ -68,7 +69,7 @@
             rc = fn(*a)
             if timed:
                 e1.record()
-                timers["events"].append((name, tag, flops, e0, e1))
+                timers["events"].append((tname, tag, flops, e0, e1))
             if rc != 0:
                 _lib.check(rc, name)
 
@@ -96,6 +97,36 @@
 
     def join(self):
         torch.cuda.current_stream().wait_stream(self.stream)
+
+
+class DerivedBufs(dict):
+
+    def __init__(self):
+        super().__init__()
+        self._fill = {}
+
+    def derive(self, name: str, fill) -> None:
+        assert name not in self, name
+        super().__setitem__(name, None)
+        self._fill[name] = fill
+
+    def __getitem__(self, name):
+        fill = self._fill.get(name)
+        return super().__getitem__(name) if fill is None else fill()
+
+    def get(self, name, default=None):
+        return self[name] if name in self else default
+
+    def values(self):
+        return [self[k] for k in self]
+
+    def items(self):
+        return [(k, self[k]) for k in self]
+
+    def copy(self):
+        raise TypeError("DerivedBufs cannot be copied: derived entries exist only when read")
+
+    __copy__ = copy
 
 
 def _ptr(t: Optional[torch.Tensor]):
@@ -228,7 +259,7 @@
         assert ws.numel() * 4 >= nbytes, tag
         plan.add("vp_colsum_f32", _ptr(x), _ptr(out), R, C, _ptr(ws), ws.numel() * 4, side=side)
 
-    def bn_fwd(self, plan, tag, x, R, Cn, bn, y, y_s=None, count=1, conv=None):
+    def bn_fwd(self, plan, tag, x, R, Cn, bn, y, y_s=None, count=1, conv=None, apply=True):
         P = _ptr
         mean, rstd = self.buf(f"{tag}.mean", Cn), self.buf(f"{tag}.rstd", Cn)
         mom, eps = float(bn.momentum), float(bn.eps)
@@ -242,12 +273,32 @@
         if not fused:
             plan.add("vp_bn_stats_f32", P(x), R, Cn, eps, mom, P(mean), P(rstd), P(bn.running_mean), P(bn.running_var),
                      P(ws), ws.numel() * 4)
+        if not apply:
+            return mean, rstd, ws
         if self.x2 and y_s is not None:
             plan.add("vp_bn_act_fwd_split_fmt_f32", P(x), P(mean), P(rstd), P(bn.weight), P(bn.bias), P(y), P(y_s), R, Cn,
                      _ACT_RELU, 0.0, 1)
         else:
             plan.add("vp_bn_act_fwd_split_f32", P(x), P(mean), P(rstd), P(bn.weight), P(bn.bias), P(y), P(y_s), R, Cn, _ACT_RELU, 0.0)
         return mean, rstd, ws
+
+    def derived_act(self, name, x, R, Cn, bn, mean, rstd):
+        P, dev, cache = _ptr, self.dev, {}
+
+        step = self.step
+
+        def fill():
+            if dev.type == "cuda" and getattr(step, "_fwd_epoch", None) != ops.PARAM_EPOCH[0]:
+                raise _lib.VaePlayHipError(f"{name} is derived from the current BatchNorm parameters: read it after forward_backward() and "
+                                           "before the optimiser updates them (step() has already moved them)")
+            if "y" not in cache:
+                cache["y"] = torch.empty(R * Cn, dtype=torch.float32, device=dev)
+            y = cache["y"]
+            if dev.type == "cuda":
+                _lib.call("vp_bn_act_fwd_f32", P(x), P(mean), P(rstd), P(bn.weight), P(bn.bias), P(y), R, Cn, _ACT_RELU, 0.0,
+                          ops._stream())
+            return y
+        self.bufs.derive(name, fill)
 
     def _conv5_fwd(self, plan, tag, conv, x, bn, eps, mom, mean, rstd) -> bool:
         P = _ptr
```

After: 9457 images/sec, median of 6. 1.01x the previous value.
